# pkuyzy/ESC-GNN

Measured on AMD Instinct MI355X. Metric: graphs/sec + edges-aggregated/sec, NestedGIN_eff h=3 bs=128 @1/2/4/8 GPU, higher is better.
Workload: dtype f32; 1 GPU; count_cycle-shaped random regular graphs (n in 10/15/20/30), target=triangles, NestedGIN_eff h=3 layers=4 hidden=256, bs=128 per GPU (configs[1]); global_batch=128, parallelism=dp1 graph-sharded, rccl_ranks=1, ranks=1

## Files before the change

### esc-gnn_amd/_native.py

```python
import ctypes
import os
from ctypes import c_double, c_int64

from . import _abi

_HERE = os.path.dirname(os.path.abspath(__file__))
LIB_PATH = os.path.join(_HERE, "libescgnn_hip.so")


class NativeLibraryError(ImportError):
    pass


try:
    _ABI = _abi.load()
except OSError as exc:
    raise NativeLibraryError("esc_gnn_amd: cannot read the C header %s the binding is derived from (%s)" % (_abi.HEADER, exc)) from exc


def const(name):
    return _ABI.constants[name]


def struct(name):
    return _ABI.structs[name]


def callback(name):
    return _ABI.callbacks[name]


members = _abi.members
ABI_VERSION = const("ESC_ABI_VERSION")
ESC_ERANGE = const("ESC_ERANGE")
SIGNATURES = {name: args for name, (args, _) in _ABI.functions.items()}
_RET = {name: ret for name, (_, ret) in _ABI.functions.items()}
EXTENSION_HEADER = os.path.join(os.path.dirname(_abi.HEADER), "escgnn_subgraphs.h")
try:
    _EXT = _abi.load(EXTENSION_HEADER)
except OSError as exc:
    raise NativeLibraryError("esc_gnn_amd: cannot read the C header %s the binding is derived from (%s)" % (EXTENSION_HEADER, exc)) from exc
EXTENSION_SIGNATURES = {name: args for name, (args, _) in _EXT.functions.items()}
_RET.update({name: ret for name, (_, ret) in _EXT.functions.items()})
I2GNN_HEADER = os.path.join(os.path.dirname(_abi.HEADER), "escgnn_i2gnn.h")
try:
    _I2 = _abi.load(I2GNN_HEADER)
except OSError as exc:
    raise NativeLibraryError("esc_gnn_amd: cannot read the C header %s the binding is derived from (%s)" % (I2GNN_HEADER, exc)) from exc
I2GNN_SIGNATURES = {name: args for name, (args, _) in _I2.functions.items()}
_RET.update({name: ret for name, (_, ret) in _I2.functions.items()})
GINEPLUS_HEADER = os.path.join(os.path.dirname(_abi.HEADER), "escgnn_gineplus.h")
try:
    _GP = _abi.load(GINEPLUS_HEADER)
except OSError as exc:
    raise NativeLibraryError("esc_gnn_amd: cannot read the C header %s the binding is derived from (%s)" % (GINEPLUS_HEADER, exc)) from exc
GINEPLUS_SIGNATURES = {name: args for name, (args, _) in _GP.functions.items()}
_RET.update({name: ret for name, (_, ret) in _GP.functions.items()})
GPS_HEADER = os.path.join(os.path.dirname(_abi.HEADER), "escgnn_gps.h")
try:
    _GPS = _abi.load(GPS_HEADER)
except OSError as exc:
    raise NativeLibraryError("esc_gnn_amd: cannot read the C header %s the binding is derived from (%s)" % (GPS_HEADER, exc)) from exc
GPS_SIGNATURES = {name: args for name, (args, _) in _GPS.functions.items()}
_RET.update({name: ret for name, (_, ret) in _GPS.functions.items()})
LAPPE_HEADER = os.path.join(os.path.dirname(_abi.HEADER), "escgnn_lappe.h")
try:
    _LAPPE = _abi.load(LAPPE_HEADER)
except OSError as exc:
    raise NativeLibraryError("esc_gnn_amd: cannot read the C header %s the binding is derived from (%s)" % (LAPPE_HEADER, exc)) from exc
LAPPE_SIGNATURES = {name: args for name, (args, _) in _LAPPE.functions.items()}
_RET.update({name: ret for name, (_, ret) in _LAPPE.functions.items()})
RWSE_HEADER = os.path.join(os.path.dirname(_abi.HEADER), "escgnn_rwse.h")
try:
    _RWSE = _abi.load(RWSE_HEADER)
except OSError as exc:
    raise NativeLibraryError("esc_gnn_amd: cannot read the C header %s the binding is derived from (%s)" % (RWSE_HEADER, exc)) from exc
RWSE_SIGNATURES = {name: args for name, (args, _) in _RWSE.functions.items()}
_RET.update({name: ret for name, (_, ret) in _RWSE.functions.items()})
KIND = {name[len("ESC_K_"):].lower(): v for name, v in _ABI.enum.items() if name != "ESC_K_COUNT"}

CollateArgs = struct("esc_collate_args")
BnFuse = struct("esc_bn_fuse")
BnFold = struct("esc_bn_fold")
BnBwdFused = struct("esc_bn_bwd_fused")
BnBwdNext = struct("esc_bn_bwd_next")
SumJob = struct("esc_sum_job")
ReduceJob = struct("esc_reduce_job")

_lib = None


def lib():
    global _lib
    if _lib is not None:
        return _lib
    if not os.path.exists(LIB_PATH):
        raise NativeLibraryError(
            "esc_gnn_amd: %s not found. The HIP hot path has no fallback — build it with "
            "`python -c 'import __graft_entry__ as g; g.build()'` or `make -C esc-gnn_amd/csrc`." % LIB_PATH)
    h = ctypes.CDLL(LIB_PATH)
    for name, args in list(SIGNATURES.items()) + list(EXTENSION_SIGNATURES.items()) + list(I2GNN_SIGNATURES.items()) + list(GINEPLUS_SIGNATURES.items()) + list(GPS_SIGNATURES.items()) + list(LAPPE_SIGNATURES.items()) + list(RWSE_SIGNATURES.items()):
        try:
            fn = getattr(h, name)
        except AttributeError as exc:
            raise NativeLibraryError("esc_gnn_amd: %s lacks symbol %s (stale build?)" % (LIB_PATH, name)) from exc
        fn.argtypes = args
        fn.restype = _RET[name]
    if h.esc_abi_version() != ABI_VERSION:
        raise NativeLibraryError("esc_gnn_amd: ABI version mismatch (library %d, header %d) — rebuild"
                                 % (h.esc_abi_version(), ABI_VERSION))
    _lib = h
    return h


def call(name, *args):
    h = lib()
    rc = getattr(h, name)(*args)
    if rc != 0:
        raise RuntimeError("%s failed (%d): %s" % (name, rc, h.esc_last_error().decode()))


def ptr(t):
    return None if t is None else t.data_ptr()


def stream():
    import torch
    return torch.cuda.current_stream().cuda_stream


def prof_enable(kind, on=True):
    call("esc_prof_enable", KIND[kind], int(on))


def prof_reset(kind):
    call("esc_prof_reset", KIND[kind])


def prof_read(kind):
    n, ms = c_int64(0), c_double(0.0)
    call("esc_prof_read", KIND[kind], ctypes.byref(n), ctypes.byref(ms))
    return n.value, ms.value


def prof_span_arm(kind, launches):
    call("esc_prof_span_arm", KIND[kind], int(launches), stream())


def prof_span_read(kind, cap=1 << 16):
    buf = (c_double * cap)()
    n = lib().esc_prof_span_read(KIND[kind], buf, cap)
    return [buf[i] for i in range(n)]


def prof_read_all(kind, cap=1 << 16):
    buf = (c_double * cap)()
    n = lib().esc_prof_read_all(KIND[kind], buf, cap)
    return [buf[i] for i in range(n)]
```

### esc-gnn_amd/csrc/common.h

```cpp
#pragma once
#include <hip/hip_runtime.h>
#include <hip/hip_ext.h>
#include <stdint.h>
#include <stdio.h>
#include <stdarg.h>

#include "../../include/escgnn_hip.h"

namespace esc {

constexpr int WAVE = 64;

#ifndef ESC_NODE_PRIO
#define ESC_NODE_PRIO 2
#endif
#define ESC_PRIO() __builtin_amdgcn_s_setprio(ESC_NODE_PRIO)

void set_error(const char* fmt, ...);

#define ESC_REQUIRE(cond, ...)                    \
  do {                                            \
    if (!(cond)) {                                \
      esc::set_error(__VA_ARGS__);                \
      return ESC_EINVAL;                          \
    }                                             \
  } while (0)

#define ESC_CHECK_LAUNCH(name)                                              \
  do {                                                                      \
    hipError_t err__ = hipGetLastError();                                   \
    if (err__ != hipSuccess) {                                              \
      esc::set_error("%s: launch failed: %s", name, hipGetErrorString(err__)); \
      return ESC_ELAUNCH;                                                   \
    }                                                                       \
  } while (0)

inline bool aligned16(const void* p) { return (reinterpret_cast<uintptr_t>(p) & 15) == 0; }
inline int64_t cdiv(int64_t a, int64_t b) { return (a + b - 1) / b; }

bool prof_slot(int kind, hipEvent_t* start, hipEvent_t* stop);
unsigned long long* prof_span_next(int kind);
#define ESC_SPAN_WGS 2048
#define ESC_SPAN_WAVES 8192
#define ESC_SPAN_STRIDE (ESC_SPAN_WGS + ESC_SPAN_WAVES)
bool trace_launch();

void arm_launch_event(hipEvent_t ev);
hipEvent_t take_launch_event();
void arm_last_launch_event(hipEvent_t ev);
void next_launch_is_last();
hipEvent_t take_last_launch_event();

template <typename... KArgs, typename... Args>
inline void launch(int kind, void (*kernel)(KArgs...), dim3 grid, dim3 block, size_t lds, hipStream_t s,
                   Args... args) {
  hipEvent_t a = nullptr, b = nullptr;
  hipEvent_t done = take_launch_event();
  if (done != nullptr) {
    hipStreamCaptureStatus cap = hipStreamCaptureStatusNone;
    if (hipStreamIsCapturing(s, &cap) != hipSuccess || cap != hipStreamCaptureStatusNone) { arm_launch_event(done); done = nullptr; }
  }
  if (prof_slot(kind, &a, &b)) {
    hipExtLaunchKernelGGL(kernel, grid, block, (unsigned)lds, s, a, b, 0, static_cast<KArgs>(args)...);
    if (done != nullptr) (void)hipEventRecord(done, s);
  } else if (done != nullptr) {
    hipExtLaunchKernelGGL(kernel, grid, block, (unsigned)lds, s, nullptr, done, 0, static_cast<KArgs>(args)...);
  } else {
    hipLaunchKernelGGL(kernel, grid, block, (unsigned)lds, s, static_cast<KArgs>(args)...);
  }
  if (trace_launch()) {
    const char* name = hipKernelNameRefByPtr(reinterpret_cast<const void*>(kernel), s);
    fprintf(stderr, "[esc] %s grid (%u,%u,%u) block %u lds %zu stream %p ...", name ? name : "?", grid.x, grid.y, grid.z, block.x, lds, (void*)s);
    fflush(stderr);
    const hipError_t e = hipStreamSynchronize(s);
    fprintf(stderr, " %s\n", e == hipSuccess ? "done" : hipGetErrorString(e));
  }
}

struct BnCounters {
  int n = 0;
  int64_t* p[ESC_MAX_BN_COUNTERS] = {};
};
int bag_bwd_classify_counted(const int32_t* c_row, int64_t Z, int64_t H, int64_t rows, float* partials, const BnCounters& cnt,
                             void* stream);

__device__ __forceinline__ int lane_id() { return threadIdx.x & 63; }

__device__ __forceinline__ int uniform(int v) { return __builtin_amdgcn_readfirstlane(v); }

__device__ __forceinline__ float wave_sum(float v) {
#pragma unroll
  for (int o = 32; o > 0; o >>= 1) v += __shfl_xor(v, o, 64);
  return v;
}
__device__ __forceinline__ double wave_sum(double v) {
#pragma unroll
  for (int o = 32; o > 0; o >>= 1) v += __shfl_xor(v, o, 64);
  return v;
}

__device__ __forceinline__ float uniform01(unsigned long long seed, unsigned long long i) {
  unsigned long long z = seed + i * 0x9E3779B97F4A7C15ull;
  z = (z ^ (z >> 30)) * 0xBF58476D1CE4E5B9ull;
  z = (z ^ (z >> 27)) * 0x94D049BB133111EBull;
  z ^= z >> 31;
  return (float)(z >> 40) * (1.0f / 16777216.0f);
}

unsigned* tickets(int n);
int gemm_lds_floor();
void set_gemm_lds_floor(int bytes);
int edge_lds_floor();
int node_lds_floor();
void set_node_lds_floor(int bytes);
void set_edge_lds_floor(int bytes);
int norm_rowblock_cap();
void set_norm_rowblock_cap(int v);
bool bn_bwd_one_launch();
void set_bn_bwd_one_launch(int on);
bool bn_bwd_fold();
void set_bn_bwd_fold(int on);
bool last_block_finalize();
void set_last_block_finalize(int on);
void set_linear_knob(int knob, int value);
struct DualSplit { hipEvent_t dx_done = nullptr, dw_done = nullptr; int dx_lds = 0; };
void request_dual_split(const DualSplit& r);
bool take_dual_split();

__device__ __forceinline__ void store_agent(float2* p, float2 v) {
  const unsigned long long bits = ((unsigned long long)__float_as_uint(v.y) << 32) | __float_as_uint(v.x);
  __hip_atomic_store(reinterpret_cast<unsigned long long*>(p), bits, __ATOMIC_RELAXED, __HIP_MEMORY_SCOPE_AGENT);
}

__device__ __forceinline__ bool grid_last_block(unsigned* counter, unsigned nblocks) {
  __shared__ unsigned s_ticket;
  __builtin_amdgcn_s_waitcnt(0x0F70);
  __syncthreads();
  if (threadIdx.x == 0) s_ticket = __hip_atomic_fetch_add(counter, 1u, __ATOMIC_RELAXED, __HIP_MEMORY_SCOPE_AGENT);
  __syncthreads();
  const bool last = s_ticket == nblocks - 1;
  if (last) {
    __builtin_amdgcn_fence(__ATOMIC_ACQUIRE, "agent");
    if (threadIdx.x == 0) *counter = 0;
  }
  return last;
}

__device__ __forceinline__ void chan_merge(double& n, double& mu, double& m2, double nb, double mub, double m2b) {
  if (nb == 0.0) return;
  const double tot = n + nb;
  const double delta = mub - mu;
  mu += delta * nb / tot;
  m2 += m2b + delta * delta * n * nb / tot;
  n = tot;
}


struct BnFoldDev {
  const float2* partials;
  int P, block_rows, M, C;
  float eps, momentum;
  const float* gamma; const float* beta;
  float* mean; float* invstd; float* scale; float* shift; float* running_mean; float* running_var;
};
__device__ __forceinline__ void bn_fold_column(const BnFoldDev& f, int col, bool writer, float& sc, float& sh) {
  const int full = f.M / f.block_rows;
  double n = 0.0, mu = 0.0, m2 = 0.0;
  if (full > 0) {
    const double pivot = (double)f.partials[col].x;
    double S1 = 0.0, S2 = 0.0, SM = 0.0;
    constexpr int CH = 40;
    for (int p0 = 0; p0 < full; p0 += CH) {
      float2 v[CH];
#pragma unroll
      for (int u = 0; u < CH; ++u) v[u] = f.partials[(size_t)min(p0 + u, full - 1) * f.C + col];
#pragma unroll
      for (int u = 0; u < CH; ++u) {
        if (p0 + u < full) { const double d = (double)v[u].x - pivot; S1 += d; S2 += d * d; SM += (double)v[u].y; }
      }
    }
    n = (double)f.block_rows * full;
    mu = pivot + S1 / full;
    m2 = SM + (double)f.block_rows * (S2 - S1 * S1 / full);
    if (m2 < 0.0) m2 = 0.0;
  }
  if (f.M > f.block_rows * full) {
    const float2 v = f.partials[(size_t)full * f.C + col];
    chan_merge(n, mu, m2, (double)(f.M - f.block_rows * full), (double)v.x, (double)v.y);
  }
  const float is = (float)(1.0 / sqrt(m2 / (double)f.M + (double)f.eps));
  sc = (f.gamma ? f.gamma[col] : 1.f) * is;
  sh = (f.beta ? f.beta[col] : 0.f) - (float)mu * sc;
  if (writer) {
    f.mean[col] = (float)mu;
    f.invstd[col] = is;
    if (f.scale) { f.scale[col] = sc; f.shift[col] = sh; }
    if (f.running_mean) f.running_mean[col] = (1.f - f.momentum) * f.running_mean[col] + f.momentum * (float)mu;
    if (f.running_var) f.running_var[col] = (1.f - f.momentum) * f.running_var[col] + f.momentum * (float)(m2 / (double)(f.M - 1));
  }
}

struct BnbDev {
  const float* x; int ldx;
  const float* mean; const float* invstd; const float* scale; const float* shift;
  const float2* coef;
  int relu;
};
struct BnStatDev {
  float2* partial;
  const float* x; int ldx;
  const float* mean; const float* invstd; const float* scale; const float* shift;
  int relu;
};

__device__ __forceinline__ float bnb_apply(float gv, float xv, float mu, float a, float ms, float mh, float k1, float k2) {
  const float gm = fmaf(xv, ms, mh) > 0.f ? gv : 0.f;
  return a * fmaf(mu - xv, k2, gm - k1);
}
__device__ __forceinline__ float bnb_apply_elu(float gv, float xv, float mu, float a, float ms, float mh, float k1, float k2) {
  const float v = fmaf(xv, ms, mh);
  const float gm = v > 0.f ? gv : gv * expf(v);
  return a * fmaf(mu - xv, k2, gm - k1);
}
__device__ __forceinline__ float bnb_apply_act(float gv, float xv, float mu, float a, float ms, float mh, float k1, float k2, bool elu) {
  return elu ? bnb_apply_elu(gv, xv, mu, a, ms, mh, k1, k2) : bnb_apply(gv, xv, mu, a, ms, mh, k1, k2);
}

}
```

### esc-gnn_amd/csrc/engine.hip

```cpp
#include "common.h"

#include <map>
#include <vector>
#include <cstdlib>

namespace esc {

struct Arena {
  float* base;
  int64_t off;
  float* take(int64_t n) {
    float* p = base ? base + off : nullptr;
    off += (n + 63) & ~63LL;
    return p;
  }
};

struct BnWs { float *mean, *invstd, *scale, *shift, *nglob, *coef; };
struct MlpWs { float *Y0, *Y1; BnWs b0, b1; float* A1 = nullptr; };

struct Layout {
  int64_t N, E, Z, H, L, C0, W;
  float *Zb, *Yz; BnWs zb0, zb1;
  float *A0, *Zemb;
  float* e[ESC_MAX_LAYERS]; float* agg[ESC_MAX_LAYERS]; MlpWs conv[ESC_MAX_LAYERS];
  int64_t ld_e[ESC_MAX_LAYERS];
  float *e_cat, *w_cat;
  MlpWs xemb; float *cat, *Yl; BnWs bl; float *pred, *dpred;
  float *dcat, *dAl, *dT1, *dT2, *dagg, *dZemb, *dAz, *deps_part;
  float* d_e[ESC_MAX_LAYERS];
  float *bn_scratch, *bag_scratch, *slabs;
  float *col_stats;
  float *bst_part;
  float *bn_scratch_e, *col_stats_e;
  float *cat_scale, *cat_shift;
  float *X0, *dX0, *Zcat, *dZcat, *pooled, *dpool, *Al;
  int64_t G, D, Wz;
  int64_t total;
};

static BnWs take_bn(Arena& a, int64_t C) { BnWs w; w.mean = a.take(C); w.invstd = a.take(C); w.scale = a.take(C); w.shift = a.take(C); w.nglob = a.take(16); w.coef = a.take(2 * C); return w; }

static Layout plan_layout(const esc_nested_gin_t* m, int64_t N, int64_t E, int64_t Z, float* base, bool train) {
  Layout y{};
  Arena a{base, 0};
  const int64_t H = m->hidden, L = m->num_layers, C0 = m->in_dim;
  y.N = N; y.E = E; y.Z = Z; y.H = H; y.L = L; y.C0 = C0; y.W = (L + 1) * H;
  y.Zb = a.take(E * H); y.Yz = a.take(E * H); y.zb0 = take_bn(a, H); y.zb1 = take_bn(a, H);
  y.A0 = a.take(E * H); y.Zemb = a.take(E * H);
  const bool batched = L >= 3;
  if (batched) { y.e_cat = a.take(E * (L - 1) * H); y.w_cat = a.take(((L - 1) * H + (L - 1)) * H); }
  for (int l = 0; l < L; ++l) {
    const int64_t C = l == 0 ? C0 : H;
    if (batched && l >= 1) { y.e[l] = base ? y.e_cat + (int64_t)(l - 1) * H : nullptr; y.ld_e[l] = (L - 1) * H; }
    else { y.e[l] = a.take(E * C); y.ld_e[l] = C; }
    y.agg[l] = a.take(N * C);
    y.conv[l].Y0 = a.take(N * H); y.conv[l].Y1 = a.take(N * H);
    y.conv[l].b0 = take_bn(a, H); y.conv[l].b1 = take_bn(a, H);
  }
  y.xemb.Y0 = a.take(N * H); y.xemb.Y1 = a.take(N * H); y.xemb.b0 = take_bn(a, H); y.xemb.b1 = take_bn(a, H);
  y.cat = a.take(N * y.W); y.Yl = a.take(N * H); y.bl = take_bn(a, H);
  y.cat_scale = a.take(y.W); y.cat_shift = a.take(y.W);
  if (base) {
    y.xemb.b1.scale = y.cat_scale; y.xemb.b1.shift = y.cat_shift;
    for (int l = 0; l < L; ++l) { y.conv[l].b1.scale = y.cat_scale + (int64_t)(l + 1) * H; y.conv[l].b1.shift = y.cat_shift + (int64_t)(l + 1) * H; }
  }
  y.pred = a.take(N); y.dpred = a.take(N);
  y.bn_scratch = a.take(esc_bn_scratch(H));
  y.col_stats = a.take(2 * ((E > N ? E : N) / 32 + 1) * H);
  y.bn_scratch_e = a.take(esc_bn_scratch(H));
  y.col_stats_e = a.take(2 * (E / 32 + 1) * H);
  if (train) {
    y.bst_part = a.take(2 * (N / 4 + 2) * H);
    y.dcat = a.take(N * y.W); y.dAl = a.take(N * H); y.dT1 = a.take(N * H); y.dT2 = a.take(N * H);
    y.dagg = a.take(N * H); y.dZemb = a.take(E * H); y.dAz = a.take(E * H);
    for (int l = 0; l < L; ++l) y.d_e[l] = a.take(E * (l == 0 ? C0 : H));
    y.deps_part = a.take(2 * N * (L > 0 ? L : 1));
    y.bag_scratch = a.take(esc_bag_bwd_scratch(Z, H));
    int64_t sl = esc_linear_bwd_weight_scratch(E, H, H) + 64;
    for (int l = 0; l < L; ++l) {
      const int64_t C = l == 0 ? C0 : H;
      sl += esc_linear_bwd_weight_scratch(E, C, H) + esc_linear_bwd_weight_scratch(N, H, H) +
            esc_linear_bwd_weight_scratch(N, H, C) + 3 * 64;
    }
    sl += esc_linear_bwd_weight_scratch(N, H, H) + esc_linear_bwd_weight_scratch(N, H, C0) + 2 * 64;
    sl += esc_linear_bwd_weight_scratch(N, H, y.W) + esc_linear_bwd_weight_scratch(N, 1, H) + 2 * 64;
    sl += esc_linear_bwd_weight_scratch(N, H, 1) + 64;
    y.slabs = a.take(sl);
  }
  y.total = a.off;
  return y;
}

#define ESC_TRY(call)            \
  do {                           \
    int rc__ = (call);           \
    if (rc__ != ESC_OK) return rc__; \
  } while (0)

struct Ctx {
  const esc_nested_gin_t* m;
  const esc_batch_t* b;
  Layout y;
  void* s;
  bool train;
  std::vector<esc_reduce_job>* jobs = nullptr;
  float** slab_cursor = nullptr;
  bool on_edge_stream = false;
  int act = 1;
  const float* l1_target = nullptr;
  int64_t l1_denom = 0;
};

struct LdsFloorGuard {
  explicit LdsFloorGuard(bool on) : on_(on && edge_lds_floor() > 0) { if (on_) set_gemm_lds_floor(edge_lds_floor()); }
  ~LdsFloorGuard() { if (on_) set_gemm_lds_floor(0); }
  bool on_;
};

static constexpr int kNodeLdsFloorBwd = 66 * 1024;
static constexpr int kReadoutDxLds = 84 * 1024;
static_assert(2 * kReadoutDxLds > 160 * 1024 && kReadoutDxLds + kNodeLdsFloorBwd <= 160 * 1024, "one readout dX tile and one node tile per CU");
static int g_readout_one_launch = 0;
struct NodeFloorGuard {
  explicit NodeFloorGuard(int bytes) : on_(bytes > 0) { if (on_) set_node_lds_floor(bytes); }
  ~NodeFloorGuard() { if (on_) set_node_lds_floor(0); }
  bool on_;
};

static int linear_backward(const Ctx& c, const float* dY, int64_t ld_dy, const float* X, int64_t ld_x, const float* sc,
                           const float* sh, const esc_linear_t& lin, int64_t M, float* dX, int64_t ld_dx, int accumulate) {
  const LdsFloorGuard cap(c.on_edge_stream);
  const int64_t N = lin.out_dim, K = lin.in_dim;
  if (c.jobs == nullptr)
    return esc_linear_bwd_both(dY, ld_dy, X, ld_x, sc, sh, lin.w, K, M, N, K, dX, ld_dx, accumulate, lin.dw, K, lin.db,
                               c.y.slabs, c.s);
  float* slabs = *c.slab_cursor;
  *c.slab_cursor += (esc_linear_bwd_weight_scratch(M, N, K) + 63) & ~63LL;
  c.jobs->emplace_back();
  return esc_linear_bwd_both_deferred(dY, ld_dy, X, ld_x, sc, sh, lin.w, K, M, N, K, dX, ld_dx, accumulate, lin.dw, K, lin.db,
                                      slabs, &c.jobs->back(), c.s);
}

static constexpr bool kBnBwdApplyInGemm = true;
static constexpr bool kBnBwdSumsFromDx = true;
static constexpr bool kBnBwdSumsFromAgg = true;
static esc_bn_bwd_fused bn_fused(const float* x, int64_t ld_x, const BnWs& w, int relu) {
  return esc_bn_bwd_fused{x, ld_x, w.mean, w.invstd, w.scale, w.shift, w.coef, relu};
}
static int linear_backward_bn(const Ctx& c, const float* dOut, int64_t ld_dout, const esc_bn_bwd_fused& f, const float* X, int64_t ld_x,
                              const float* sc, const float* sh, const esc_linear_t& lin, int64_t M, float* dX, int64_t ld_dx,
                              int accumulate, const esc_bn_bwd_next* next) {
  const LdsFloorGuard cap(c.on_edge_stream);
  const int64_t N = lin.out_dim, K = lin.in_dim;
  if (c.jobs == nullptr)
    return esc_linear_bwd_both_bn(dOut, ld_dout, &f, X, ld_x, sc, sh, lin.w, K, M, N, K, dX, ld_dx, accumulate, lin.dw, K, lin.db, c.y.slabs,
                                  nullptr, next, c.s);
  float* slabs = *c.slab_cursor;
  *c.slab_cursor += (esc_linear_bwd_weight_scratch(M, N, K) + 63) & ~63LL;
  c.jobs->emplace_back();
  return esc_linear_bwd_both_bn(dOut, ld_dout, &f, X, ld_x, sc, sh, lin.w, K, M, N, K, dX, ld_dx, accumulate, lin.dw, K, lin.db, slabs,
                                &c.jobs->back(), next, c.s);
}

struct EdgeStream {
  hipStream_t stream = nullptr;
  hipEvent_t z_ready = nullptr, joined = nullptr, lin1_fork = nullptr, lin1_rest = nullptr, lin1_dw = nullptr, e_ready[ESC_MAX_LAYERS] = {}, de_ready[ESC_MAX_LAYERS] = {},
             agg_done[ESC_MAX_LAYERS] = {};
  bool ok = false;
};
static int g_use_edge_stream = 1;
static int current_device() {
  int dev = 0;
  (void)hipGetDevice(&dev);
  return dev;
}
static EdgeStream& edge_stream() {
  static thread_local std::map<int, EdgeStream> per_device;
  static thread_local EdgeStream off;
  if (!g_use_edge_stream) return off;
  EdgeStream& es = per_device[current_device()];
  if (!es.ok && es.stream == nullptr) {
    int least = 0, greatest = 0;
    (void)hipDeviceGetStreamPriorityRange(&least, &greatest);
    bool good = hipStreamCreateWithPriority(&es.stream, hipStreamNonBlocking, least) == hipSuccess;
    good = good && hipEventCreateWithFlags(&es.z_ready, hipEventDisableTiming) == hipSuccess;
    good = good && hipEventCreateWithFlags(&es.joined, hipEventDisableTiming) == hipSuccess;
    good = good && hipEventCreateWithFlags(&es.lin1_fork, hipEventDisableTiming) == hipSuccess;
    good = good && hipEventCreateWithFlags(&es.lin1_rest, hipEventDisableTiming) == hipSuccess;
    good = good && hipEventCreateWithFlags(&es.lin1_dw, hipEventDisableTiming) == hipSuccess;
    for (int l = 0; l < ESC_MAX_LAYERS; ++l) {
      good = good && hipEventCreateWithFlags(&es.e_ready[l], hipEventDisableTiming) == hipSuccess;
      good = good && hipEventCreateWithFlags(&es.de_ready[l], hipEventDisableTiming) == hipSuccess;
      good = good && hipEventCreateWithFlags(&es.agg_done[l], hipEventDisableTiming) == hipSuccess;
    }
    es.ok = good;
  }
  return es;
}
static int64_t g_two_stream_min_edges = 12000;
static EdgeStream& edge_stream_for(int64_t edges) {
  static thread_local EdgeStream off;
  return edges >= g_two_stream_min_edges ? edge_stream() : off;
}
static int chain(hipEvent_t ev, hipStream_t src, hipStream_t waiter) {
  if (hipEventRecord(ev, src) != hipSuccess || hipStreamWaitEvent(waiter, ev, 0) != hipSuccess) {
    set_error("esc_engine: stream event failed");
    return ESC_ELAUNCH;
  }
  return ESC_OK;
}

static int g_plain_events = 0;
struct ArmedEvent {
  ArmedEvent(hipEvent_t ev, bool on) : on_(on && !g_plain_events) { if (on_) arm_launch_event(ev); }
  ~ArmedEvent() { if (on_) (void)take_launch_event(); }
  bool on_;
};
struct ArmedLastEvent {
  ArmedLastEvent(hipEvent_t ev, bool on) : on_(on && !g_plain_events) { if (on_) arm_last_launch_event(ev); }
  ~ArmedLastEvent() { if (on_) (void)take_last_launch_event(); }
  bool bound() const { return on_ && take_last_launch_event() == nullptr; }
  bool on_;
};
static int chain_armed(hipEvent_t ev, const ArmedEvent& arm, hipStream_t src, hipStream_t waiter) {
  const bool bound = arm.on_ && take_launch_event() == nullptr;
  if ((!bound && hipEventRecord(ev, src) != hipSuccess) || (waiter != nullptr && hipStreamWaitEvent(waiter, ev, 0) != hipSuccess)) {
    set_error("esc_engine: stream event failed");
    return ESC_ELAUNCH;
  }
  return ESC_OK;
}

static Ctx edge_ctx(const Ctx& c, hipStream_t edge) {
  Ctx x = c;
  x.s = edge;
  x.on_edge_stream = true;
  x.y.bn_scratch = c.y.bn_scratch_e;
  x.y.col_stats = c.y.col_stats_e;
  return x;
}

enum { PH_START = 0, PH_EDGE_FWD_DONE, PH_NODE_FWD_DONE, PH_NODE_BWD_DONE, PH_EDGE_BWD_DONE, PH_END, PH_COUNT };
struct PhaseRing {
  static constexpr int RING = 128;
  hipEvent_t ev[RING][PH_COUNT] = {};
  int steps = 0;
  bool on = getenv("ESC_PHASE_TIMING") != nullptr;
};
static PhaseRing& phases() { static PhaseRing p; return p; }
static void mark(int which, void* stream) {
  PhaseRing& p = phases();
  if (!p.on) return;
  hipEvent_t& e = p.ev[p.steps % PhaseRing::RING][which];
  if (e == nullptr && hipEventCreate(&e) != hipSuccess) { p.on = false; return; }
  (void)hipEventRecord(e, (hipStream_t)stream);
}

static bool fuse_node_act(const Ctx& c) { return c.act == 1 && c.y.H >= 64 && c.y.H % 4 == 0 && c.y.cat_scale != nullptr; }

struct Collective {
  esc_allreduce_fn fn = nullptr; void* user = nullptr;
  int rank = 0, world = 1;
  float *buf_node = nullptr, *buf_edge = nullptr; int64_t cap = 0;
};
static Collective g_coll;
static bool sync_on(const Ctx& c) { return c.train && g_coll.fn != nullptr && g_coll.world > 1; }
static float* sync_buf(const Ctx& c) {
  EdgeStream& es = edge_stream();
  return (es.ok && c.s == (void*)es.stream) ? g_coll.buf_edge : g_coll.buf_node;
}
static int sync_allreduce(const Ctx& c, float* buf, int64_t n) {
  ESC_REQUIRE(buf != nullptr && n <= g_coll.cap, "esc_engine: SyncBN exchange buffer too small (%ld > %ld floats)", (long)n, (long)g_coll.cap);
  const int rc = g_coll.fn(buf, n, c.s, g_coll.user);
  if (rc != 0) { set_error("esc_engine: the collective provider failed (%d)", rc); return ESC_ELAUNCH; }
  return ESC_OK;
}
static int bn_sync_forward(const Ctx& c, int64_t M, const esc_bn_t& bn, const BnWs& w, int64_t C) {
  float* buf = sync_buf(c);
  ESC_TRY(esc_bn_sync_pack(w.mean, w.invstd, M, bn.eps, C, g_coll.rank, g_coll.world, buf, c.s));
  ESC_TRY(sync_allreduce(c, buf, (int64_t)g_coll.world * 3 * C));
  return esc_bn_sync_finalize(buf, g_coll.world, C, bn.eps, bn.momentum, w.mean, w.invstd, bn.running_mean, bn.running_var,
                              bn.gamma, bn.beta, w.scale, w.shift, w.nglob, c.s);
}
static int bn_backward(const Ctx& c, const float* X, int64_t ldx, const float* Y, int64_t ldy, const float* dY, int64_t lddy,
                       int64_t M, const BnWs& w, const esc_bn_t& bn, float* dX, int64_t lddx, float* scratch, int64_t width = 0) {
  const int64_t C = width > 0 ? width : c.y.H;
  if (!sync_on(c))
    return esc_bn_bwd(X, ldx, Y, ldy, dY, lddy, M, C, w.mean, w.invstd, bn.gamma, bn.beta, c.act, dX, lddx, bn.dgamma, bn.dbeta,
                      scratch, c.s);
  float* buf = sync_buf(c);
  ESC_TRY(esc_bn_bwd_sums(X, ldx, Y, ldy, dY, lddy, M, C, w.mean, w.invstd, bn.gamma, bn.beta, c.act, buf, bn.dgamma, bn.dbeta,
                          scratch, c.s));
  ESC_TRY(sync_allreduce(c, buf, 2 * C));
  ESC_TRY(esc_bn_sync_coef(buf, C, w.nglob, c.s));
  return esc_bn_bwd_apply(X, ldx, Y, ldy, dY, lddy, M, C, w.mean, w.invstd, bn.gamma, bn.beta, c.act, buf, dX, lddx, c.s);
}

static int bn_backward_drop(const Ctx& c, const float* X, int64_t ldx, const float* dY, int64_t lddy, int64_t M, const BnWs& w,
                            const esc_bn_t& bn, const uint8_t* mask, float p, int on_output, float* dX, int64_t lddx,
                            float* scratch, int64_t width = 0) {
  const int64_t C = width > 0 ? width : c.y.H;
  if (p <= 0.f) return bn_backward(c, X, ldx, nullptr, 0, dY, lddy, M, w, bn, dX, lddx, scratch, width);
  const bool fused = !sync_on(c) && c.act <= 1 && ldx == C && lddy == C && lddx == C && esc_bn_bwd_dropout_ok(C, ldx, lddy, lddx) &&
                     ((reinterpret_cast<uintptr_t>(X) | reinterpret_cast<uintptr_t>(dY) | reinterpret_cast<uintptr_t>(dX) |
                       reinterpret_cast<uintptr_t>(w.mean) | reinterpret_cast<uintptr_t>(w.invstd) | reinterpret_cast<uintptr_t>(bn.gamma) |
                       reinterpret_cast<uintptr_t>(bn.beta) | reinterpret_cast<uintptr_t>(scratch)) & 15) == 0 &&
                     (reinterpret_cast<uintptr_t>(mask) & 3) == 0;
  if (fused)
    return esc_bn_bwd_dropout(X, ldx, dY, lddy, M, C, w.mean, w.invstd, bn.gamma, bn.beta, c.act, mask, p, on_output, dX, lddx,
                              bn.dgamma, bn.dbeta, scratch, c.s);
  if (!on_output) {
    ESC_TRY(esc_dropout_bwd(dY, lddy, M, C, p, mask, nullptr, 0, dX, lddx, c.s));
    return bn_backward(c, X, ldx, nullptr, 0, dX, lddx, M, w, bn, dX, lddx, scratch, width);
  }
  ESC_TRY(bn_backward(c, X, ldx, nullptr, 0, dY, lddy, M, w, bn, dX, lddx, scratch, width));
  return esc_dropout_bwd(dX, lddx, M, C, p, mask, nullptr, 0, dX, lddx, c.s);
}

static int linear_bn(const Ctx& c, const float* X, int64_t ld_x, const esc_linear_t& lin, const float* sc, const float* sh,
                     int64_t M, float* Y, const esc_bn_t& bn, const BnWs& w, int64_t ld_y = 0) {
  const LdsFloorGuard cap(c.on_edge_stream);
  const int64_t H = lin.out_dim, K = lin.in_dim;
  if (ld_y <= 0) ld_y = H;
  const bool sync = sync_on(c);
  const bool fused = c.train && H > 32 && c.jobs != nullptr;
  if (fused && M > 1 && !sync) {
    esc_bn_fuse f{bn.eps, bn.momentum, w.mean, w.invstd, bn.running_mean, bn.running_var, bn.gamma, bn.beta, w.scale, w.shift};
    return esc_linear_bn_fwd(X, ld_x, lin.w, K, lin.b, sc, sh, M, H, K, Y, ld_y, c.y.col_stats, &f, c.s);
  }
  ESC_TRY(esc_linear_fwd(X, ld_x, lin.w, K, lin.b, sc, sh, M, H, K, Y, ld_y, fused ? c.y.col_stats : nullptr, c.s));
  if (fused) {
    ESC_TRY(esc_bn_stats_from_partials_rows(c.y.col_stats, M, H, esc_linear_stats_block_rows(X, ld_x, lin.w, K, M, H, K), bn.eps,
                                            bn.momentum, w.mean, w.invstd, sync ? nullptr : bn.running_mean,
                                            sync ? nullptr : bn.running_var, bn.gamma, bn.beta, sync ? nullptr : w.scale,
                                            sync ? nullptr : w.shift, c.s));
    return sync ? bn_sync_forward(c, M, bn, w, H) : ESC_OK;
  }
  if (c.train) {
    ESC_TRY(esc_bn_stats(Y, ld_y, M, H, bn.eps, bn.momentum, w.mean, w.invstd, sync ? nullptr : bn.running_mean,
                         sync ? nullptr : bn.running_var, bn.gamma, bn.beta, sync ? nullptr : w.scale, sync ? nullptr : w.shift,
                         c.y.bn_scratch, c.s));
    return sync ? bn_sync_forward(c, M, bn, w, H) : ESC_OK;
  }
  return esc_bn_eval_coef(bn.running_mean, bn.running_var, bn.gamma, bn.beta, bn.eps, H, w.scale, w.shift, c.s);
}

static int bn_coeffs(const Ctx& c, const float* X, int64_t ld, int64_t M, const esc_bn_t& bn, const BnWs& w, int64_t width = 0) {
  const int64_t C = width > 0 ? width : c.y.H;
  if (c.train) {
    const bool sync = sync_on(c);
    ESC_TRY(esc_bn_stats(X, ld, M, C, bn.eps, bn.momentum, w.mean, w.invstd, sync ? nullptr : bn.running_mean,
                         sync ? nullptr : bn.running_var, bn.gamma, bn.beta, sync ? nullptr : w.scale, sync ? nullptr : w.shift,
                         c.y.bn_scratch, c.s));
    return sync ? bn_sync_forward(c, M, bn, w, C) : ESC_OK;
  }
  return esc_bn_eval_coef(bn.running_mean, bn.running_var, bn.gamma, bn.beta, bn.eps, C, w.scale, w.shift, c.s);
}

static int mlp_forward(const Ctx& c, const esc_mlp_t& p, const MlpWs& w, const float* A, int64_t ld_a, int64_t M,
                       float* out, int64_t ld_out, bool pre_out = false) {
  const int64_t H = c.y.H;
  if (pre_out) {
    ESC_TRY(linear_bn(c, A, ld_a, p.lin0, nullptr, nullptr, M, w.Y0, p.bn0, w.b0));
    return linear_bn(c, w.Y0, H, p.lin1, w.b0.scale, w.b0.shift, M, out, p.bn1, w.b1, ld_out);
  }
  ESC_TRY(linear_bn(c, A, ld_a, p.lin0, nullptr, nullptr, M, w.Y0, p.bn0, w.b0));
  if (w.A1) {
    ESC_TRY(esc_affine_act(w.Y0, H, M, H, w.b0.scale, w.b0.shift, c.act, w.A1, H, c.s));
    ESC_TRY(linear_bn(c, w.A1, H, p.lin1, nullptr, nullptr, M, w.Y1, p.bn1, w.b1));
    return esc_affine_act(w.Y1, H, M, H, w.b1.scale, w.b1.shift, c.act, out, ld_out, c.s);
  }
  ESC_TRY(linear_bn(c, w.Y0, H, p.lin1, w.b0.scale, w.b0.shift, M, w.Y1, p.bn1, w.b1));
  return esc_affine_act(w.Y1, H, M, H, w.b1.scale, w.b1.shift, 1, out, ld_out, c.s);
}

struct MlpFuse { bool lin1 = false, lin0 = false; };
static MlpFuse mlp_fuse_plan(const Ctx& c, const esc_mlp_t& p, const MlpWs& w, const float* A, int64_t ld_a, int64_t M, const float* out,
                             int64_t ld_out, const float* dOut, int64_t ld_dout, const float* dA, int64_t ld_da, bool pre_out) {
  const Layout& y = c.y;
  const int64_t H = y.H;
  MlpFuse f;
  if (!(kBnBwdApplyInGemm && c.train && !sync_on(c) && y.bst_part != nullptr && p.lin1.in_dim == H && p.lin1.out_dim == H)) return f;
  if (!(c.act == 1 && w.A1 == nullptr)) return f;
  const esc_bn_bwd_fused f1 = bn_fused(pre_out ? out : w.Y1, pre_out ? ld_out : H, w.b1, c.act), f0 = bn_fused(w.Y0, H, w.b0, c.act);
  const esc_bn_bwd_next n0{y.bst_part, w.Y0, H, w.b0.mean, w.b0.invstd, w.b0.scale, w.b0.shift, c.act};
  const float* slab_probe = c.jobs ? *c.slab_cursor : y.slabs;
  f.lin1 = esc_linear_bwd_both_bn_ok(dOut, ld_dout, &f1, w.Y0, H, p.lin1.w, H, M, H, H, y.dT2, H, slab_probe, &n0) != 0;
  f.lin0 = f.lin1 && esc_linear_bwd_both_bn_ok(y.dT2, H, &f0, A, ld_a, p.lin0.w, p.lin0.in_dim, M, H, p.lin0.in_dim, dA, ld_da, slab_probe, nullptr) != 0;
  return f;
}
static bool mlp_backward_fused(const Ctx& c, const esc_mlp_t& p, const MlpWs& w, const float* A, int64_t ld_a, int64_t M, const float* out,
                               int64_t ld_out, const float* dOut, int64_t ld_dout, const float* dA, int64_t ld_da, bool pre_out) {
  return mlp_fuse_plan(c, p, w, A, ld_a, M, out, ld_out, dOut, ld_dout, dA, ld_da, pre_out).lin1;
}
static int mlp_backward(const Ctx& c, const esc_mlp_t& p, const MlpWs& w, const float* A, int64_t ld_a, int64_t M,
                        const float* out, int64_t ld_out, const float* dOut, int64_t ld_dout, float* dA,
                        int64_t ld_da, bool pre_out = false, int64_t have_slots = 0) {
  const Layout& y = c.y;
  const int64_t H = y.H;
  const MlpFuse fuse = mlp_fuse_plan(c, p, w, A, ld_a, M, out, ld_out, dOut, ld_dout, dA, ld_da, pre_out);
  if (fuse.lin1) {
    const float* x1 = pre_out ? out : w.Y1;
    const int64_t ld_x1 = pre_out ? ld_out : H;
    const esc_bn_bwd_fused f1 = bn_fused(x1, ld_x1, w.b1, c.act), f0 = bn_fused(w.Y0, H, w.b0, c.act);
    esc_bn_bwd_next n0{y.bst_part, w.Y0, H, w.b0.mean, w.b0.invstd, w.b0.scale, w.b0.shift, c.act};
    if (have_slots > 0)
      ESC_TRY(esc_bn_bwd_coef_from_partials(y.bst_part, have_slots, M, H, w.b1.coef, p.bn1.dgamma, p.bn1.dbeta, c.s));
    else
      ESC_TRY(esc_bn_bwd_coef(x1, ld_x1, nullptr, 0, dOut, ld_dout, M, H, w.b1.mean, w.b1.invstd, p.bn1.gamma, p.bn1.beta, c.act, w.b1.coef,
                              p.bn1.dgamma, p.bn1.dbeta, y.bn_scratch, c.s));
    ESC_TRY(linear_backward_bn(c, dOut, ld_dout, f1, w.Y0, H, w.b0.scale, w.b0.shift, p.lin1, M, y.dT2, H, 0, &n0));
    ESC_TRY(esc_bn_bwd_coef_from_partials(y.bst_part, cdiv(M, esc_linear_bwd_bn_block_rows(M, H, H)), M, H, w.b0.coef, p.bn0.dgamma, p.bn0.dbeta, c.s));
    if (fuse.lin0) return linear_backward_bn(c, y.dT2, H, f0, A, ld_a, nullptr, nullptr, p.lin0, M, dA, ld_da, 0, nullptr);
    ESC_TRY(esc_bn_bwd_apply(w.Y0, H, nullptr, 0, y.dT2, H, M, H, w.b0.mean, w.b0.invstd, p.bn0.gamma, p.bn0.beta, c.act, w.b0.coef, y.dT2, H, c.s));
    return linear_backward(c, y.dT2, H, A, ld_a, nullptr, nullptr, p.lin0, M, dA, ld_da, 0);
  }
  if (pre_out) ESC_TRY(bn_backward(c, out, ld_out, nullptr, 0, dOut, ld_dout, M, w.b1, p.bn1, y.dT1, H, y.bn_scratch));
  else         ESC_TRY(bn_backward(c, w.Y1, H, out, ld_out, dOut, ld_dout, M, w.b1, p.bn1, y.dT1, H, y.bn_scratch));
  if (w.A1) {
    ESC_TRY(linear_backward(c, y.dT1, H, w.A1, H, nullptr, nullptr, p.lin1, M, y.dT2, H, 0));
    ESC_TRY(bn_backward(c, w.Y0, H, w.A1, H, y.dT2, H, M, w.b0, p.bn0, y.dT2, H, y.bn_scratch));
    return linear_backward(c, y.dT2, H, A, ld_a, nullptr, nullptr, p.lin0, M, dA, ld_da, 0);
  }
  ESC_TRY(linear_backward(c, y.dT1, H, w.Y0, H, w.b0.scale, w.b0.shift, p.lin1, M, y.dT2, H, 0));
  ESC_TRY(bn_backward(c, w.Y0, H, nullptr, 0, y.dT2, H, M, w.b0, p.bn0, y.dT2, H, y.bn_scratch));
  return linear_backward(c, y.dT2, H, A, ld_a, nullptr, nullptr, p.lin0, M, dA, ld_da, 0);
}

static int forward(const Ctx& c) {
  const esc_nested_gin_t* m = c.m;
  const esc_batch_t* b = c.b;
  const Layout& y = c.y;
  const int64_t N = y.N, E = y.E, H = y.H, L = y.L, W = y.W;
  EdgeStream& es = edge_stream_for(E);
  Ctx ce = c;
  if (es.ok) {
    ESC_TRY(chain(es.z_ready, (hipStream_t)c.s, es.stream));
    ce = edge_ctx(c, es.stream);
  }
  const int64_t bag_block = (c.train && !sync_on(ce)) ? esc_bag_fwd_stats_block_rows(m->z_table, m->z_rows, H, y.Zb, H, E) : 0;
  if (bag_block > 0) {
    ESC_TRY(esc_bag_fwd_rows(m->z_table, m->z_rows, H, b->row_ptr, b->bag_idx, b->bag_val, E, y.Zb, H, 0, ce.y.col_stats, ce.s));
    ESC_TRY(esc_bn_stats_from_partials_rows(ce.y.col_stats, E, H, bag_block, m->zbn0.eps, m->zbn0.momentum, y.zb0.mean, y.zb0.invstd,
                                            m->zbn0.running_mean, m->zbn0.running_var, m->zbn0.gamma, m->zbn0.beta, y.zb0.scale, y.zb0.shift, ce.s));
  } else {
    ESC_TRY(esc_bag_fwd_rows(m->z_table, m->z_rows, H, b->row_ptr, b->bag_idx, b->bag_val, E, y.Zb, H, 0, nullptr, ce.s));
    ESC_TRY(bn_coeffs(ce, y.Zb, H, E, m->zbn0, y.zb0));
  }
  ESC_TRY(esc_affine_act(y.Zb, H, E, H, y.zb0.scale, y.zb0.shift, 1, y.A0, H, ce.s));
  ESC_TRY(linear_bn(ce, y.A0, H, m->zlin, nullptr, nullptr, E, y.Yz, m->zbn1, y.zb1));
  const bool e0_early = y.C0 <= 32 && L >= 1;
  if (e0_early) {
    const LdsFloorGuard cap(ce.on_edge_stream);
    const ArmedEvent arm(es.e_ready[0], es.ok);
    ESC_TRY(esc_linear_fwd(y.Yz, H, m->conv[0].lin.w, H, m->conv[0].lin.b, y.zb1.scale, y.zb1.shift, E, y.C0, H, y.e[0], y.ld_e[0], nullptr, ce.s));
    if (es.ok) ESC_TRY(chain_armed(es.e_ready[0], arm, es.stream, nullptr));
  }
  ESC_TRY(esc_affine_act(y.Yz, H, E, H, y.zb1.scale, y.zb1.shift, 1, y.Zemb, H, ce.s));
  auto edge_term = [&](int l) -> int {
    const LdsFloorGuard cap(ce.on_edge_stream);
    const esc_conv_t& cv = m->conv[l];
    const int64_t C = l == 0 ? y.C0 : H;
    ESC_TRY(esc_linear_fwd(y.Zemb, H, cv.lin.w, H, cv.lin.b, nullptr, nullptr, E, C, H, y.e[l], y.ld_e[l], nullptr, ce.s));
    if (es.ok && hipEventRecord(es.e_ready[l], es.stream) != hipSuccess) { set_error("esc_engine: stream event failed"); return ESC_ELAUNCH; }
    return ESC_OK;
  };
  mark(PH_START, c.s);
  const bool batched = y.e_cat != nullptr;
  if (batched) {
    if (!e0_early) ESC_TRY(edge_term(0));
    esc_table_list tl{};
    tl.count = 2 * ((int)L - 1);
    for (int l = 1; l < (int)L; ++l) {
      tl.rows[l - 1] = (int32_t)H; tl.w[l - 1] = m->conv[l].lin.w;
      tl.rows[(L - 1) + l - 1] = 1; tl.w[(L - 1) + l - 1] = m->conv[l].lin.b;
    }
    ESC_TRY(esc_table_pack(&tl, H, y.w_cat, ce.s));
    {
      const LdsFloorGuard cap(ce.on_edge_stream);
      const ArmedEvent arm(es.e_ready[1], es.ok);
      ESC_TRY(esc_linear_fwd(y.Zemb, H, y.w_cat, H, y.w_cat + (L - 1) * H * H, nullptr, nullptr, E, (L - 1) * H, H, y.e_cat, (L - 1) * H, nullptr, ce.s));
      if (es.ok) ESC_TRY(chain_armed(es.e_ready[1], arm, es.stream, nullptr));
    }
    for (int l = 2; l < (int)L; ++l)
      if (es.ok && hipEventRecord(es.e_ready[l], es.stream) != hipSuccess) { set_error("esc_engine: stream event failed"); return ESC_ELAUNCH; }
  }
  const int ahead = batched ? 0 : (es.ok ? 1 : (int)L);
  for (int l = e0_early ? 1 : 0; l < (int)L && l < ahead; ++l) ESC_TRY(edge_term(l));
  if (c.train) {
    BnCounters cnt;
    cnt.n = (int)m->n_counters;
    for (int i = 0; i < cnt.n; ++i) cnt.p[i] = m->counters[i];
    ESC_TRY(bag_bwd_classify_counted(b->col_row, y.Z, H, E, y.bag_scratch, cnt, c.s));
  }
  ESC_TRY(mlp_forward(c, m->xemb, y.xemb, b->x, y.C0, N, y.cat, W, fuse_node_act(c)));
  for (int l = 0; l < L; ++l) {
    const esc_conv_t& cv = m->conv[l];
    const int64_t C = l == 0 ? y.C0 : H;
    const float* hin = l == 0 ? b->x : y.cat + (int64_t)l * H;
    const int64_t ld_h = l == 0 ? y.C0 : W;
    if (es.ok && !(batched && l >= 2) && hipStreamWaitEvent((hipStream_t)c.s, es.e_ready[l], 0) != hipSuccess) { set_error("esc_engine: stream event failed"); return ESC_ELAUNCH; }
    if (fuse_node_act(c) && l > 0)
      ESC_TRY(esc_gine_aggregate_fwd_affine(hin, ld_h, y.cat_scale + (int64_t)l * H, y.cat_shift + (int64_t)l * H, y.e[l], y.ld_e[l], b->in_ptr,
                                            b->in_edge, b->in_src, cv.eps, N, C, y.agg[l], C, c.s));
    else
      ESC_TRY(esc_gine_aggregate_fwd(hin, ld_h, y.e[l], y.ld_e[l], b->in_ptr, b->in_edge, b->in_src, cv.eps, N, C, y.agg[l], C, c.s));
    if (!batched && es.ok && l + ahead < (int)L) {
      ESC_TRY(chain(es.agg_done[l], (hipStream_t)c.s, es.stream));
      ESC_TRY(edge_term(l + ahead));
    }
    ESC_TRY(mlp_forward(c, cv.nn, y.conv[l], y.agg[l], C, N, y.cat + (int64_t)(l + 1) * H, W, fuse_node_act(c)));
  }
  if (c.train) mark(PH_EDGE_FWD_DONE, ce.s);
  const bool fa = fuse_node_act(c);
  ESC_TRY(linear_bn(c, y.cat, W, m->lin1, fa ? y.cat_scale : nullptr, fa ? y.cat_shift : nullptr, N, y.Yl, m->bn_lin1, y.bl));
  if (c.l1_target != nullptr && esc_linear_fwd_l1_ok(y.Yl, H, m->lin2.w, H, y.bl.scale, y.bl.shift)) {
    const ArmedEvent arm(es.lin1_fork, es.ok);
    ESC_TRY(esc_linear_fwd_l1(y.Yl, H, m->lin2.w, m->lin2.b, y.bl.scale, y.bl.shift, N, H, c.l1_target, c.l1_denom, 1.0f, y.pred, y.dpred, c.s));
    return es.ok ? chain_armed(es.lin1_fork, arm, (hipStream_t)c.s, es.stream) : ESC_OK;
  }
  return esc_linear_fwd(y.Yl, H, m->lin2.w, H, m->lin2.b, y.bl.scale, y.bl.shift, N, 1, H, y.pred, 1, nullptr, c.s);
}

struct Pending {
  bool open = false;
  bool join = false;
  hipStream_t stream = nullptr;
  std::vector<esc_reduce_job> edge_jobs;
};
static Pending& pending() {
  static thread_local Pending p;
  return p;
}
static int finish_pending(Pending& p) {
  if (!p.open) return ESC_OK;
  p.open = false;
  EdgeStream& es = edge_stream();
  if (p.join && hipStreamWaitEvent(p.stream, es.joined, 0) != hipSuccess) { set_error("esc_engine: stream event failed"); return ESC_ELAUNCH; }
  if (!p.edge_jobs.empty()) ESC_TRY(esc_slab_reduce_jobs(p.edge_jobs.data(), (int)p.edge_jobs.size(), p.stream));
  p.edge_jobs.clear();
  mark(PH_END, p.stream);
  if (phases().on) ++phases().steps;
  return ESC_OK;
}

static int backward(const Ctx& c, Pending* defer) {
  EdgeStream& es = edge_stream_for(c.y.E);
  const NodeFloorGuard node_floor(es.ok ? kNodeLdsFloorBwd : 0);
  const esc_nested_gin_t* m = c.m;
  const esc_batch_t* b = c.b;
  const Layout& y = c.y;
  const int64_t N = y.N, E = y.E, H = y.H, L = y.L, W = y.W;
  ESC_TRY(linear_backward(c, y.dpred, 1, y.Yl, H, y.bl.scale, y.bl.shift, m->lin2, N, y.dAl, H, 0));
  const bool split_lin1 = es.ok && c.jobs != nullptr && L >= 1;
  const esc_bn_bwd_fused fl = bn_fused(y.Yl, H, y.bl, 1);
  const bool fa_l = fuse_node_act(c);
  const MlpWs& wl = y.conv[L > 0 ? L - 1 : 0];
  esc_bn_bwd_next nl{y.bst_part, y.cat + L * H, W, wl.b1.mean, wl.b1.invstd, wl.b1.scale, wl.b1.shift, 1};
  auto lin1_ok = [&](int64_t col0, int64_t ncols, const esc_bn_bwd_next* nx) {
    return esc_linear_bwd_both_bn_ok(y.dAl, H, &fl, y.cat + col0, W, m->lin1.w + col0, W, N, H, ncols, y.dcat + col0, W,
                                     c.jobs ? *c.slab_cursor : y.slabs, nx) != 0;
  };
  const bool fuse_l = kBnBwdApplyInGemm && c.act == 1 && !sync_on(c) && y.bst_part != nullptr &&
                      (split_lin1 ? (lin1_ok(0, L * H, nullptr) && lin1_ok(L * H, H, nullptr)) : lin1_ok(0, W, nullptr));
  int64_t last_slots = 0;
  bool k0_split = false;
  bool fork_bound = false;
  if (fuse_l) {
    const ArmedLastEvent arm(es.lin1_fork, split_lin1);
    ESC_TRY(esc_bn_bwd_coef(y.Yl, H, nullptr, 0, y.dAl, H, N, H, y.bl.mean, y.bl.invstd, m->bn_lin1.gamma, m->bn_lin1.beta, 1, y.bl.coef,
                            m->bn_lin1.dgamma, m->bn_lin1.dbeta, y.bn_scratch, c.s));
    fork_bound = arm.bound();
  } else
    ESC_TRY(bn_backward(c, y.Yl, H, nullptr, 0, y.dAl, H, N, y.bl, m->bn_lin1, y.dAl, H, y.bn_scratch));
  if (split_lin1) {
    const int64_t K0 = L * H;
    auto part = [&](void* stream, int64_t col0, int64_t ncols, float* db, const esc_bn_bwd_next* nx) -> int {
      float* slabs = *c.slab_cursor;
      *c.slab_cursor += (esc_linear_bwd_weight_scratch(N, H, ncols) + 63) & ~63LL;
      c.jobs->emplace_back();
      const bool fa = fa_l;
      if (fuse_l)
        return esc_linear_bwd_both_bn(y.dAl, H, &fl, y.cat + col0, W, fa ? y.cat_scale + col0 : nullptr, fa ? y.cat_shift + col0 : nullptr, m->lin1.w + col0, W,
                                      N, H, ncols, y.dcat + col0, W, 0, m->lin1.dw + col0, W, db, slabs, &c.jobs->back(), nx, stream);
      return esc_linear_bwd_both_deferred(y.dAl, H, y.cat + col0, W, fa ? y.cat_scale + col0 : nullptr, fa ? y.cat_shift + col0 : nullptr, m->lin1.w + col0, W, N, H, ncols,
                                          y.dcat + col0, W, 0, m->lin1.dw + col0, W, db, slabs, &c.jobs->back(), stream);
    };
    if ((!fork_bound && hipEventRecord(es.lin1_fork, (hipStream_t)c.s) != hipSuccess) || hipStreamWaitEvent(es.stream, es.lin1_fork, 0) != hipSuccess) {
      set_error("esc_engine: stream event failed");
      return ESC_ELAUNCH;
    }
    {
      const LdsFloorGuard cap(true);
      const bool ask = fuse_l && !g_readout_one_launch && !g_plain_events;
      if (ask) request_dual_split(DualSplit{es.lin1_rest, es.lin1_dw, kReadoutDxLds});
      const int rc = part(es.stream, 0, K0, nullptr, nullptr);
      k0_split = !take_dual_split() && ask;
      ESC_TRY(rc);
    }
    if (!k0_split && hipEventRecord(es.lin1_rest, es.stream) != hipSuccess) { set_error("esc_engine: stream event failed"); return ESC_ELAUNCH; }
    const bool leave = fuse_l && fa_l && kBnBwdSumsFromDx && lin1_ok(K0, H, &nl) &&
                       mlp_backward_fused(c, m->conv[L - 1].nn, y.conv[L - 1], y.agg[L - 1], L == 1 ? y.C0 : H, N, y.cat + L * H, W, y.dcat + L * H, W,
                                          y.dagg, L == 1 ? y.C0 : H, true);
    ESC_TRY(part(c.s, K0, H, m->lin1.db, leave ? &nl : nullptr));
    if (leave) last_slots = cdiv(N, esc_linear_bwd_bn_block_rows(N, H, H));
  } else if (fuse_l) {
    ESC_TRY(linear_backward_bn(c, y.dAl, H, fl, y.cat, W, fa_l ? y.cat_scale : nullptr, fa_l ? y.cat_shift : nullptr, m->lin1, N, y.dcat, W, 0, nullptr));
  } else {
    ESC_TRY(linear_backward(c, y.dAl, H, y.cat, W, fa_l ? y.cat_scale : nullptr, fa_l ? y.cat_shift : nullptr, m->lin1, N, y.dcat, W, 0));
  }
  Ctx ce = es.ok ? edge_ctx(c, es.stream) : c;
  std::vector<esc_reduce_job> edge_jobs;
  edge_jobs.reserve(ESC_MAX_REDUCE_JOBS);
  if (es.ok && c.jobs) ce.jobs = &edge_jobs;
  std::vector<esc_sum_job> eps_jobs;
  int64_t agg_slots = 0;
  for (int l = (int)L - 1; l >= 0; --l) {
    const esc_conv_t& cv = m->conv[l];
    const int64_t C = l == 0 ? y.C0 : H;
    const float* hin = l == 0 ? b->x : y.cat + (int64_t)l * H;
    const int64_t ld_h = l == 0 ? y.C0 : W;
    ESC_TRY(mlp_backward(c, cv.nn, y.conv[l], y.agg[l], C, N, y.cat + (int64_t)(l + 1) * H, W,
                         y.dcat + (int64_t)(l + 1) * H, W, y.dagg, C, fuse_node_act(c), l == (int)L - 1 ? last_slots : agg_slots));
    agg_slots = 0;
    float* dx = l == 0 ? nullptr : y.dcat + (int64_t)l * H;
    if (split_lin1 && l == (int)L - 1 &&
        hipStreamWaitEvent((hipStream_t)c.s, es.lin1_rest, 0) != hipSuccess) { set_error("esc_engine: stream event failed"); return ESC_ELAUNCH; }
    const ArmedEvent arm(es.de_ready[l], es.ok);
    const bool stats_here = fuse_node_act(c) && l > 0 && kBnBwdSumsFromAgg && esc_gine_aggregate_bwd_deps_slots(C) == 1 && C <= 2048 &&
                            mlp_backward_fused(c, m->conv[l - 1].nn, y.conv[l - 1], y.agg[l - 1], l - 1 == 0 ? y.C0 : H, N, y.cat + (int64_t)l * H, W,
                                               y.dcat + (int64_t)l * H, W, y.dagg, l - 1 == 0 ? y.C0 : H, true);
    if (stats_here) {
      ESC_TRY(esc_gine_aggregate_bwd_affine_stats(hin, ld_h, y.cat_scale + (int64_t)l * H, y.cat_shift + (int64_t)l * H, y.conv[l - 1].b1.mean,
                                                  y.conv[l - 1].b1.invstd, y.e[l], y.ld_e[l], y.dagg, C, b->out_ptr, b->out_edge, b->out_dst, cv.eps, N, C,
                                                  y.d_e[l], C, dx, W, 1, y.deps_part + (int64_t)l * 2 * N, y.bst_part, c.s));
      agg_slots = esc_gine_aggregate_bwd_stats_slots(N);
    } else if (fuse_node_act(c) && l > 0)
      ESC_TRY(esc_gine_aggregate_bwd_affine(hin, ld_h, y.cat_scale + (int64_t)l * H, y.cat_shift + (int64_t)l * H, y.e[l], y.ld_e[l], y.dagg, C,
                                            b->out_ptr, b->out_edge, b->out_dst, cv.eps, N, C, y.d_e[l], C, dx, W, 1,
                                            y.deps_part + (int64_t)l * 2 * N, c.s));
    else
      ESC_TRY(esc_gine_aggregate_bwd(hin, ld_h, y.e[l], y.ld_e[l], y.dagg, C, b->out_ptr, b->out_edge, b->out_dst, cv.eps, N, C,
                                     y.d_e[l], C, dx, W, 1, y.deps_part + (int64_t)l * 2 * N, c.s));
    eps_jobs.push_back(esc_sum_job{y.deps_part + (int64_t)l * 2 * N, N * esc_gine_aggregate_bwd_deps_slots(C), cv.deps});
    if (es.ok) ESC_TRY(chain_armed(es.de_ready[l], arm, (hipStream_t)c.s, es.stream));
    const float* zin = y.Zemb;
    if (l == 0 && es.ok && c.jobs) {
      {
        const LdsFloorGuard cap(true);
        ESC_TRY(esc_linear_bwd_input(y.d_e[l], C, cv.lin.w, H, E, C, H, y.dZemb, H, l == (int)L - 1 ? 0 : 1, es.stream));
      }
      float* slabs = *c.slab_cursor;
      *c.slab_cursor += (esc_linear_bwd_weight_scratch(E, C, H) + 63) & ~63LL;
      c.jobs->emplace_back();
      ESC_TRY(esc_linear_bwd_both_deferred(y.d_e[l], C, zin, H, nullptr, nullptr, cv.lin.w, H, E, C, H, nullptr, 0, 0, cv.lin.dw, H, cv.lin.db,
                                           slabs, &c.jobs->back(), c.s));
    } else {
      ESC_TRY(linear_backward(ce, y.d_e[l], C, zin, H, nullptr, nullptr, cv.lin, E, y.dZemb, H, l == (int)L - 1 ? 0 : 1));
    }
    if (es.ok && !edge_jobs.empty() && l > 0) {
      ESC_TRY(esc_slab_reduce_jobs(edge_jobs.data(), (int)edge_jobs.size(), es.stream));
      edge_jobs.clear();
    }
  }
  ESC_TRY(mlp_backward(c, m->xemb, y.xemb, b->x, y.C0, N, y.cat, W, y.dcat, W, nullptr, 0, fuse_node_act(c)));
  Ctx ct = ce;
  ct.on_edge_stream = false;
  ESC_TRY(bn_backward(ce, y.Yz, H, nullptr, 0, y.dZemb, H, E, y.zb1, m->zbn1, y.dZemb, H, ce.y.bn_scratch));
  ESC_TRY(linear_backward(ct, y.dZemb, H, y.A0, H, nullptr, nullptr, m->zlin, E, y.dAz, H, 0));
  ESC_TRY(bn_backward(ce, y.Zb, H, nullptr, 0, y.dAz, H, E, y.zb0, m->zbn0, y.dAz, H, ce.y.bn_scratch));
  ESC_TRY(esc_bag_bwd_table_rows(y.dAz, H, H, b->col_ptr, b->col_row, b->col_val, b->col_col, y.Z, m->z_rows, E,
                                 1, m->dz_table, y.bag_scratch, ce.s));
  mark(PH_NODE_BWD_DONE, c.s);
  mark(PH_EDGE_BWD_DONE, ce.s);
  if (!eps_jobs.empty()) ESC_TRY(esc_reduce_sum_jobs(eps_jobs.data(), (int)eps_jobs.size(), c.s));
  if (k0_split && hipStreamWaitEvent((hipStream_t)c.s, es.lin1_dw, 0) != hipSuccess) { set_error("esc_engine: stream event failed"); return ESC_ELAUNCH; }
  if (c.jobs && !c.jobs->empty()) ESC_TRY(esc_slab_reduce_jobs(c.jobs->data(), (int)c.jobs->size(), c.s));
  if (es.ok) {
    if (hipEventRecord(es.joined, es.stream) != hipSuccess) { set_error("esc_engine: stream event failed"); return ESC_ELAUNCH; }
    Pending local;
    Pending& p = defer ? *defer : local;
    p.open = true; p.join = true; p.stream = (hipStream_t)c.s;
    p.edge_jobs.swap(edge_jobs);
    if (!defer) return finish_pending(p);
  }
  return ESC_OK;
}

static Layout plan_layout_zinc(const esc_zinc_gin_t* m, int64_t N, int64_t E, int64_t Z, int64_t G, float* base, bool train) {
  Layout y{};
  Arena a{base, 0};
  const int64_t H = m->hidden, L = m->num_layers, D = m->edge_emb.dim, C0 = m->node_emb.dim;
  y.N = N; y.E = E; y.Z = Z; y.H = H; y.L = L; y.C0 = C0; y.W = L * H; y.G = G; y.D = D; y.Wz = H + D;
  y.X0 = a.take(N * C0);
  y.Zb = a.take(E * H); y.Yz = a.take(E * H); y.zb0 = take_bn(a, H); y.zb1 = take_bn(a, H);
  y.A0 = a.take(E * H); y.Zcat = a.take(E * y.Wz);
  const int64_t lb = C0 == H ? 0 : 1, nb = L - lb;
  const bool batched = nb >= 2;
  if (batched) { y.e_cat = a.take(E * nb * H); y.w_cat = a.take(nb * H * y.Wz + nb * H); }
  for (int l = 0; l < L; ++l) {
    const int64_t C = l == 0 ? C0 : H;
    if (batched && l >= lb) { y.e[l] = base ? y.e_cat + (int64_t)(l - lb) * H : nullptr; y.ld_e[l] = nb * H; }
    else { y.e[l] = a.take(E * C); y.ld_e[l] = C; }
    y.agg[l] = a.take(N * C);
    y.conv[l].Y0 = a.take(N * H); y.conv[l].Y1 = a.take(N * H); y.conv[l].A1 = a.take(N * H);
    y.conv[l].b0 = take_bn(a, H); y.conv[l].b1 = take_bn(a, H);
  }
  const bool nodes = m->node_readout != 0;
  const int64_t R = nodes ? N : G;
  y.cat = a.take(N * y.W); y.pooled = nodes ? nullptr : a.take(G * y.W); y.Yl = a.take(R * H); y.Al = a.take(R * H);
  y.bl = take_bn(a, H);
  y.pred = a.take(R); y.dpred = a.take(R);
  y.bn_scratch = a.take(esc_bn_scratch(H));
  y.col_stats = a.take(2 * ((E > N ? E : N) / 32 + 1) * H);
  y.bn_scratch_e = a.take(esc_bn_scratch(H));
  y.col_stats_e = a.take(2 * (E / 32 + 1) * H);
  if (train) {
    y.dcat = a.take(N * y.W); y.dpool = nodes ? nullptr : a.take(G * y.W); y.dAl = a.take(R * H);
    y.bst_part = a.take(2 * (N / 4 + E / 64 + 4) * H);
    y.dT1 = a.take(N * H); y.dT2 = a.take(N * H); y.dagg = a.take(N * H); y.dX0 = a.take(N * C0);
    y.dZcat = a.take(E * y.Wz); y.dZemb = a.take(E * H); y.dAz = a.take(E * H);
    for (int l = 0; l < L; ++l) y.d_e[l] = a.take(E * (l == 0 ? C0 : H));
    y.deps_part = a.take(2 * N * (L > 0 ? L : 1));
    y.bag_scratch = a.take(esc_bag_bwd_scratch(Z, H));
    int64_t sl = esc_linear_bwd_weight_scratch(E, H, H) + 64;
    for (int l = 0; l < L; ++l) {
      const int64_t C = l == 0 ? C0 : H;
      sl += esc_linear_bwd_weight_scratch(E, C, y.Wz) + esc_linear_bwd_weight_scratch(N, H, H) +
            esc_linear_bwd_weight_scratch(N, H, C) + 3 * 64;
    }
    sl += esc_linear_bwd_weight_scratch(R, H, y.W) + esc_linear_bwd_weight_scratch(R, 1, H) + 2 * 64;
    y.slabs = a.take(sl);
  }
  y.total = a.off;
  return y;
}

struct ZincCtx {
  const esc_zinc_gin_t* m;
  const esc_mol_batch_t* b;
  Ctx c;
};

static int forward_zinc(const ZincCtx& z) {
  const esc_zinc_gin_t* m = z.m;
  const esc_mol_batch_t* b = z.b;
  const Ctx& c = z.c;
  const Layout& y = c.y;
  const int64_t N = y.N, E = y.E, H = y.H, L = y.L, W = y.W, G = y.G, D = y.D, Wz = y.Wz, C0 = y.C0;
  const int act = c.act;
  EdgeStream& es = edge_stream_for(E);
  Ctx ce = c;
  if (es.ok) {
    ESC_TRY(chain(es.z_ready, (hipStream_t)c.s, es.stream));
    ce = edge_ctx(c, es.stream);
  }
  ESC_TRY(esc_bag_fwd_rows(m->z_table, m->z_rows, H, b->row_ptr, b->bag_idx, b->bag_val, E, y.Zb, H, 0, nullptr, ce.s));
  if (c.train) ESC_TRY(esc_bag_bwd_classify(b->col_row, y.Z, H, E, y.bag_scratch, ce.s));
  ESC_TRY(bn_coeffs(ce, y.Zb, H, E, m->zbn0, y.zb0));
  ESC_TRY(esc_affine_act(y.Zb, H, E, H, y.zb0.scale, y.zb0.shift, act, y.A0, H, ce.s));
  ESC_TRY(linear_bn(ce, y.A0, H, m->zlin, nullptr, nullptr, E, y.Yz, m->zbn1, y.zb1));
  ESC_TRY(esc_affine_act(y.Yz, H, E, H, y.zb1.scale, y.zb1.shift, act, y.Zcat, Wz, ce.s));
  ESC_TRY(esc_embed_fwd(m->edge_emb.w, m->edge_emb.rows, D, b->edge_type, E, y.Zcat + H, Wz, nullptr, ce.s));
  auto edge_term = [&](int l) -> int {
    const LdsFloorGuard cap(ce.on_edge_stream);
    const esc_conv_t& cv = m->conv[l];
    const int64_t C = l == 0 ? C0 : H;
    ESC_TRY(esc_linear_fwd(y.Zcat, Wz, cv.lin.w, Wz, cv.lin.b, nullptr, nullptr, E, C, Wz, y.e[l], y.ld_e[l], nullptr, ce.s));
    if (es.ok && hipEventRecord(es.e_ready[l], es.stream) != hipSuccess) { set_error("esc_zinc: stream event failed"); return ESC_ELAUNCH; }
    return ESC_OK;
  };
  const bool batched = y.e_cat != nullptr;
  if (batched) {
    const int lb = C0 == H ? 0 : 1, nb = (int)L - lb;
    if (lb == 1) ESC_TRY(edge_term(0));
    esc_table_list tw{}, tb{};
    tw.count = nb; tb.count = nb;
    for (int l = lb; l < (int)L; ++l) {
      tw.rows[l - lb] = (int32_t)H; tw.w[l - lb] = m->conv[l].lin.w;
      tb.rows[l - lb] = 1; tb.w[l - lb] = m->conv[l].lin.b;
    }
    ESC_TRY(esc_table_pack(&tw, Wz, y.w_cat, ce.s));
    ESC_TRY(esc_table_pack(&tb, H, y.w_cat + (int64_t)nb * H * Wz, ce.s));
    {
      const LdsFloorGuard cap(ce.on_edge_stream);
      ESC_TRY(esc_linear_fwd(y.Zcat, Wz, y.w_cat, Wz, y.w_cat + (int64_t)nb * H * Wz, nullptr, nullptr, E, nb * H, Wz, y.e_cat, nb * H, nullptr, ce.s));
    }
    for (int l = lb; l < (int)L; ++l)
      if (es.ok && hipEventRecord(es.e_ready[l], es.stream) != hipSuccess) { set_error("esc_zinc: stream event failed"); return ESC_ELAUNCH; }
  }
  const int ahead = batched ? 0 : (es.ok ? 1 : (int)L);
  for (int l = 0; l < (int)L && l < ahead; ++l) ESC_TRY(edge_term(l));
  ESC_TRY(esc_embed_fwd(m->node_emb.w, m->node_emb.rows, C0, b->node_type, N, y.X0, C0, nullptr, c.s));
  for (int l = 0; l < (int)L; ++l) {
    const esc_conv_t& cv = m->conv[l];
    const int64_t C = l == 0 ? C0 : H;
    const float* hin = l == 0 ? y.X0 : y.cat + (int64_t)(l - 1) * H;
    const int64_t ld_h = l == 0 ? C0 : W;
    if (es.ok && hipStreamWaitEvent((hipStream_t)c.s, es.e_ready[l], 0) != hipSuccess) { set_error("esc_zinc: stream event failed"); return ESC_ELAUNCH; }
    ESC_TRY(esc_gine_aggregate_fwd(hin, ld_h, y.e[l], y.ld_e[l], b->in_ptr, b->in_edge, b->in_src, cv.eps, N, C, y.agg[l], C, c.s));
    if (!batched && es.ok && l + ahead < (int)L) {
      ESC_TRY(chain(es.agg_done[l], (hipStream_t)c.s, es.stream));
      ESC_TRY(edge_term(l + ahead));
    }
    ESC_TRY(mlp_forward(c, cv.nn, y.conv[l], y.agg[l], C, N, y.cat + (int64_t)l * H, W));
  }
  const int64_t R = m->node_readout ? N : G;
  const float* rin = y.cat;
  if (!m->node_readout) {
    ESC_TRY(esc_segment_pool_fwd(y.cat, W, b->graph_ptr, G, W, 0, y.pooled, W, c.s));
    rin = y.pooled;
  }
  ESC_TRY(linear_bn(c, rin, W, m->lin1, nullptr, nullptr, R, y.Yl, m->bn_lin1, y.bl));
  ESC_TRY(esc_affine_act(y.Yl, H, R, H, y.bl.scale, y.bl.shift, act, y.Al, H, c.s));
  ESC_TRY(esc_linear_fwd(y.Al, H, m->lin2.w, H, m->lin2.b, nullptr, nullptr, R, 1, H, y.pred, 1, nullptr, c.s));
  if (es.ok) ESC_TRY(chain(es.joined, es.stream, (hipStream_t)c.s));
  return ESC_OK;
}

static int backward_zinc(const ZincCtx& z) {
  const esc_zinc_gin_t* m = z.m;
  const esc_mol_batch_t* b = z.b;
  const Ctx& c = z.c;
  const Layout& y = c.y;
  const int64_t N = y.N, E = y.E, H = y.H, L = y.L, W = y.W, G = y.G, D = y.D, Wz = y.Wz, C0 = y.C0;
  EdgeStream& es = edge_stream_for(E);
  Ctx ce = es.ok ? edge_ctx(c, es.stream) : c;
  std::vector<esc_reduce_job> edge_jobs;
  edge_jobs.reserve(ESC_MAX_REDUCE_JOBS);
  if (es.ok && c.jobs) ce.jobs = &edge_jobs;
  if (es.ok) ESC_TRY(chain(es.z_ready, (hipStream_t)c.s, es.stream));
  const int64_t R = m->node_readout ? N : G;
  ESC_TRY(linear_backward(c, y.dpred, 1, y.Al, H, nullptr, nullptr, m->lin2, R, y.dAl, H, 0));
  ESC_TRY(bn_backward(c, y.Yl, H, y.Al, H, y.dAl, H, R, y.bl, m->bn_lin1, y.dAl, H, y.bn_scratch));
  if (m->node_readout) {
    ESC_TRY(linear_backward(c, y.dAl, H, y.cat, W, nullptr, nullptr, m->lin1, N, y.dcat, W, 0));
  } else {
    ESC_TRY(linear_backward(c, y.dAl, H, y.pooled, W, nullptr, nullptr, m->lin1, G, y.dpool, W, 0));
    ESC_TRY(esc_segment_pool_bwd(y.dpool, W, b->graph_ptr, G, W, 0, y.dcat, W, c.s));
  }
  std::vector<esc_sum_job> eps_jobs;
  for (int l = (int)L - 1; l >= 0; --l) {
    const esc_conv_t& cv = m->conv[l];
    const int64_t C = l == 0 ? C0 : H;
    const float* hin = l == 0 ? y.X0 : y.cat + (int64_t)(l - 1) * H;
    const int64_t ld_h = l == 0 ? C0 : W;
    ESC_TRY(mlp_backward(c, cv.nn, y.conv[l], y.agg[l], C, N, y.cat + (int64_t)l * H, W, y.dcat + (int64_t)l * H, W, y.dagg, C));
    float* dx = l == 0 ? y.dX0 : y.dcat + (int64_t)(l - 1) * H;
    ESC_TRY(esc_gine_aggregate_bwd(hin, ld_h, y.e[l], y.ld_e[l], y.dagg, C, b->out_ptr, b->out_edge, b->out_dst, cv.eps, N, C,
                                   y.d_e[l], C, dx, l == 0 ? C0 : W, l == 0 ? 0 : 1, y.deps_part + (int64_t)l * 2 * N, c.s));
    eps_jobs.push_back(esc_sum_job{y.deps_part + (int64_t)l * 2 * N, N * esc_gine_aggregate_bwd_deps_slots(C), cv.deps});
    if (es.ok) ESC_TRY(chain(es.de_ready[l], (hipStream_t)c.s, es.stream));
    ESC_TRY(linear_backward(ce, y.d_e[l], C, y.Zcat, Wz, nullptr, nullptr, cv.lin, E, y.dZcat, Wz, l == (int)L - 1 ? 0 : 1));
  }
  ESC_TRY(esc_embed_bwd(y.dX0, C0, b->node_type, N, m->node_emb.rows, C0, m->node_emb.dw, c.s));
  ESC_TRY(esc_embed_bwd(y.dZcat + H, Wz, b->edge_type, E, m->edge_emb.rows, D, m->edge_emb.dw, ce.s));
  ESC_TRY(bn_backward(ce, y.Yz, H, y.Zcat, Wz, y.dZcat, Wz, E, y.zb1, m->zbn1, y.dZemb, H, ce.y.bn_scratch));
  ESC_TRY(linear_backward(ce, y.dZemb, H, y.A0, H, nullptr, nullptr, m->zlin, E, y.dAz, H, 0));
  ESC_TRY(bn_backward(ce, y.Zb, H, y.A0, H, y.dAz, H, E, y.zb0, m->zbn0, y.dAz, H, ce.y.bn_scratch));
  ESC_TRY(esc_bag_bwd_table_rows(y.dAz, H, H, b->col_ptr, b->col_row, b->col_val, b->col_col, y.Z, m->z_rows, E, 1,
                                 m->dz_table, y.bag_scratch, ce.s));
  if (es.ok && !edge_jobs.empty()) ESC_TRY(esc_slab_reduce_jobs(edge_jobs.data(), (int)edge_jobs.size(), es.stream));
  if (!eps_jobs.empty()) ESC_TRY(esc_reduce_sum_jobs(eps_jobs.data(), (int)eps_jobs.size(), c.s));
  if (c.jobs && !c.jobs->empty()) ESC_TRY(esc_slab_reduce_jobs(c.jobs->data(), (int)c.jobs->size(), c.s));
  if (es.ok) ESC_TRY(chain(es.joined, es.stream, (hipStream_t)c.s));
  return ESC_OK;
}

static int check_zinc(const esc_zinc_gin_t* m, const esc_mol_batch_t* b, const float* ws, bool train, bool need_y) {
  ESC_REQUIRE(m && b && ws, "esc_zinc: null pointer");
  ESC_REQUIRE(m->num_layers >= 1 && m->num_layers <= ESC_MAX_LAYERS, "esc_zinc: %ld layers unsupported", (long)m->num_layers);
  ESC_REQUIRE(m->hidden > 0 && m->hidden % 4 == 0, "esc_zinc: hidden must be a multiple of 4");
  ESC_REQUIRE(m->node_emb.dim > 0 && m->node_emb.dim % 4 == 0 && m->edge_emb.dim > 0 && m->edge_emb.dim % 4 == 0,
              "esc_zinc: embedding widths must be multiples of 4");
  ESC_REQUIRE(m->conv[0].lin.in_dim == m->hidden + m->edge_emb.dim && m->conv[0].lin.out_dim == m->node_emb.dim,
              "esc_zinc: conv1.lin must map hidden + edge width to the node width");
  ESC_REQUIRE(m->node_readout == 0 || m->node_readout == 1, "esc_zinc: node_readout must be 0 or 1");
  ESC_REQUIRE(b->N >= 2 && b->E >= 2 && b->Z >= 0 && b->G >= (m->node_readout ? 1 : 2),
              "esc_zinc: batch needs >= 2 nodes, edges and %s (BatchNorm statistics)", m->node_readout ? "1 graph" : "graphs");
  ESC_REQUIRE(b->node_type && b->edge_type && b->graph_ptr && b->in_ptr && b->row_ptr &&
              (!train || ((b->y || !need_y) && b->out_ptr && b->col_ptr)), "esc_zinc: null batch arrays");
  ESC_REQUIRE(aligned16(ws), "esc_zinc: workspace must be 16-byte aligned");
  return ESC_OK;
}

static ZincCtx make_zinc(const esc_zinc_gin_t* m, const esc_mol_batch_t* b, float* ws, void* stream, bool train) {
  ZincCtx z{m, b, Ctx{nullptr, nullptr, plan_layout_zinc(m, b->N, b->E, b->Z, b->G, ws, train), stream, train}};
  z.c.act = 2;
  return z;
}

struct OgbLayer {
  float *hin, *e, *agg, *Y0, *hc, *hb;
  BnWs b0, bn;
  unsigned char* mask_h;
  float *tmp, *V0, *VA, *V1, *VB, *vn;
  BnWs vb0, vb1;
  unsigned char* mask_v;
  float* d_e;
};
struct OgbLayout {
  int64_t N, E, Z, G, H, L, T;
  float *Tcat, *dTcat, *h0, *hL;
  float *Zb, *Zd, *A0, *Yz, *Yzd, *Zemb; BnWs zb0, zb1;
  unsigned char *mask_z0, *mask_z1;
  OgbLayer l[ESC_MAX_LAYERS];
  float *h[ESC_MAX_LAYERS + 1];
  float *pooled, *logits, *dlogits;
  float *dpooled, *dHa, *dHb, *dT, *dA1, *dagg, *dZemb, *dYz, *dA0, *dvn_a, *dvn_b, *dG1, *dG2, *dtmp, *poolG;
  float *deps_part, *bag_scratch, *emb_scratch, *emb_scratch_n, *slabs, *bn_scratch, *col_stats, *bn_scratch_e, *col_stats_e;
  float *bst_part;
  int64_t total;
};

static unsigned char* take_bytes(Arena& a, int64_t n) { return reinterpret_cast<unsigned char*>(a.take((n + 3) / 4)); }

static OgbLayout plan_layout_ogb(const esc_ogb_gnn_t* m, int64_t N, int64_t E, int64_t Z, int64_t G, int64_t atom_entries,
                                 int64_t bond_entries, float* base, bool train) {
  OgbLayout y{};
  Arena a{base, 0};
  const int64_t H = m->hidden, L = m->num_layers, T = m->num_tasks, H2 = 2 * H;
  const bool drop = train && m->drop_ratio > 0.f;
  y.N = N; y.E = E; y.Z = Z; y.G = G; y.H = H; y.L = L; y.T = T;
  const int64_t rows_total = m->atom_rows + L * m->bond_rows;
  y.Tcat = a.take(rows_total * H);
  y.h0 = a.take(N * H); y.h[0] = y.h0;
  y.Zb = a.take(E * H); y.Zd = drop ? a.take(E * H) : y.Zb; y.A0 = a.take(E * H);
  y.Yz = a.take(E * H); y.Yzd = drop ? a.take(E * H) : y.Yz; y.Zemb = a.take(E * H);
  y.zb0 = take_bn(a, H); y.zb1 = take_bn(a, H);
  if (drop) { y.mask_z0 = take_bytes(a, E * H); y.mask_z1 = take_bytes(a, E * H); }
  for (int l = 0; l < L; ++l) {
    OgbLayer& q = y.l[l];
    q.vn = a.take(G * H);
    q.hin = a.take(N * H);
    q.e = a.take(E * H);
    q.agg = a.take(N * H);
    q.Y0 = a.take(N * H2); q.hc = a.take(N * H); q.hb = nullptr;
    q.b0 = take_bn(a, H2); q.bn = take_bn(a, H);
    y.h[l + 1] = a.take(N * H);
    if (drop) q.mask_h = take_bytes(a, N * H);
    if (l < L - 1) {
      q.tmp = a.take(G * H); q.V0 = a.take(G * H2); q.VA = a.take(G * H2); q.V1 = a.take(G * H); q.VB = nullptr;
      q.vb0 = take_bn(a, H2); q.vb1 = take_bn(a, H);
      if (drop) q.mask_v = take_bytes(a, G * H);
    }
  }
  y.hL = y.h[L];
  y.pooled = a.take(G * H); y.logits = a.take(G * T); y.dlogits = a.take(G * T);
  y.bn_scratch = a.take(esc_bn_scratch(H2));
  y.col_stats = a.take(2 * ((E > N ? E : N) / 32 + 1) * H2);
  y.bn_scratch_e = a.take(esc_bn_scratch(H2));
  y.col_stats_e = a.take(2 * (E / 32 + 1) * H2);
  if (train) {
    y.dTcat = a.take(rows_total * H);
    y.bst_part = a.take(2 * (N / 64 + 2) * H2);
    y.dpooled = a.take(G * H); y.dHa = a.take(N * H); y.dHb = a.take(N * H); y.dT = a.take(N * H);
    y.dA1 = a.take(N * H2); y.dagg = a.take(N * H);
    y.dZemb = a.take(E * H); y.dYz = a.take(E * H); y.dA0 = a.take(E * H);
    y.dvn_a = a.take(G * H); y.dvn_b = a.take(G * H); y.dG1 = a.take(G * H2); y.dG2 = a.take(G * H); y.dtmp = a.take(G * H);
    y.poolG = a.take(G * H);
    for (int l = 0; l < L; ++l) y.l[l].d_e = a.take(E * H);
    y.deps_part = a.take(2 * N * (L > 0 ? L : 1));
    y.bag_scratch = a.take(esc_bag_bwd_scratch(Z, H));
    const int64_t ent = atom_entries > bond_entries ? atom_entries : bond_entries;
    y.emb_scratch = a.take(esc_bag_bwd_scratch(ent, H));
    y.emb_scratch_n = a.take(esc_bag_bwd_scratch(ent, H));
    int64_t sl = esc_linear_bwd_weight_scratch(E, H, H) + 64;
    for (int l = 0; l < L; ++l) {
      sl += esc_linear_bwd_weight_scratch(E, H, H) + esc_linear_bwd_weight_scratch(N, H2, H) +
            esc_linear_bwd_weight_scratch(N, H, H2) + 3 * 64;
      if (l < L - 1) sl += esc_linear_bwd_weight_scratch(G, H2, H) + esc_linear_bwd_weight_scratch(G, H, H2) + 2 * 64;
    }
    sl += esc_linear_bwd_weight_scratch(G, T, H) + 64;
    y.slabs = a.take(sl);
  }
  y.total = a.off;
  return y;
}

struct OgbCtx {
  const esc_ogb_gnn_t* m;
  const esc_ogb_batch_t* b;
  OgbLayout o;
  Ctx c;
  float p;
};

static uint64_t drop_seed(const OgbCtx& z, int which) { return z.b->seed * 0x2545F4914F6CDD1Dull + (uint64_t)(which + 1) * 0xD1342543DE82EF95ull; }

static int forward_ogb(const OgbCtx& z) {
  const esc_ogb_gnn_t* m = z.m;
  const esc_ogb_batch_t* b = z.b;
  const OgbLayout& y = z.o;
  const Ctx& c = z.c;
  const int64_t N = y.N, E = y.E, H = y.H, L = y.L, G = y.G, T = y.T, H2 = 2 * H;
  const float p = z.p;
  ESC_TRY(esc_table_pack(&m->tables, H, y.Tcat, c.s));
  EdgeStream& es = edge_stream_for(E);
  Ctx ce = c;
  if (es.ok) {
    ESC_TRY(chain(es.z_ready, (hipStream_t)c.s, es.stream));
    ce = edge_ctx(c, es.stream);
  }
  ESC_TRY(esc_bag_fwd_rows(m->z_table, m->z_rows, H, b->row_ptr, b->bag_idx, b->bag_val, E, y.Zb, H, 0, nullptr, ce.s));
  if (c.train) ESC_TRY(esc_bag_bwd_classify(b->col_row, y.Z, H, E, y.bag_scratch, ce.s));
  if (p > 0.f) ESC_TRY(esc_dropout_fwd(y.Zb, H, E, H, p, drop_seed(z, 0), nullptr, 0, y.Zd, H, y.mask_z0, ce.s));
  ESC_TRY(bn_coeffs(ce, y.Zd, H, E, m->zbn0, y.zb0));
  ESC_TRY(esc_affine_act(y.Zd, H, E, H, y.zb0.scale, y.zb0.shift, 1, y.A0, H, ce.s));
  if (p > 0.f) {
    ESC_TRY(esc_linear_fwd(y.A0, H, m->zlin.w, H, m->zlin.b, nullptr, nullptr, E, H, H, y.Yz, H, nullptr, ce.s));
    ESC_TRY(esc_dropout_fwd(y.Yz, H, E, H, p, drop_seed(z, 1), nullptr, 0, y.Yzd, H, y.mask_z1, ce.s));
    ESC_TRY(bn_coeffs(ce, y.Yzd, H, E, m->zbn1, y.zb1));
  } else {
    ESC_TRY(linear_bn(ce, y.A0, H, m->zlin, nullptr, nullptr, E, y.Yz, m->zbn1, y.zb1));
  }
  ESC_TRY(esc_affine_act(y.Yzd, H, E, H, y.zb1.scale, y.zb1.shift, 1, y.Zemb, H, ce.s));
  auto edge_term = [&](int l) -> int {
    const LdsFloorGuard cap(ce.on_edge_stream);
    const esc_ogb_layer_t& q = m->layer[l];
    ESC_TRY(esc_linear_fwd(y.Zemb, H, q.pos.w, H, q.pos.b, nullptr, nullptr, E, H, H, y.l[l].e, H, nullptr, ce.s));
    ESC_TRY(esc_bag_fwd_rows(y.Tcat + q.bond_row0 * H, m->bond_rows, H, b->bonds.row_ptr, b->bonds.idx, b->bonds.ones, E, y.l[l].e, H, 1, nullptr, ce.s));
    if (es.ok && hipEventRecord(es.e_ready[l], es.stream) != hipSuccess) { set_error("esc_ogb: stream event failed"); return ESC_ELAUNCH; }
    return ESC_OK;
  };
  const int ahead = es.ok ? 1 : (int)L;
  for (int l = 0; l < (int)L && l < ahead; ++l) ESC_TRY(edge_term(l));
  ESC_TRY(esc_bag_fwd_rows(y.Tcat, m->atom_rows, H, b->atoms.row_ptr, b->atoms.idx, b->atoms.ones, N, y.h0, H, 0, nullptr, c.s));
  ESC_TRY(esc_embed_fwd(m->vn_w, 1, H, b->zero_idx, G, y.l[0].vn, H, nullptr, c.s));
  for (int l = 0; l < (int)L; ++l) {
    const esc_ogb_layer_t& q = m->layer[l];
    const OgbLayer& w = y.l[l];
    ESC_TRY(esc_segment_broadcast_add(y.h[l], H, w.vn, H, b->graph_ptr, G, N, H, w.hin, H, c.s));
    if (es.ok && hipStreamWaitEvent((hipStream_t)c.s, es.e_ready[l], 0) != hipSuccess) { set_error("esc_ogb: stream event failed"); return ESC_ELAUNCH; }
    ESC_TRY(esc_gine_aggregate_fwd(w.hin, H, w.e, H, b->in_ptr, b->in_edge, b->in_src, q.eps, N, H, w.agg, H, c.s));
    if (es.ok && l + ahead < (int)L) {
      ESC_TRY(chain(es.agg_done[l], (hipStream_t)c.s, es.stream));
      ESC_TRY(edge_term(l + ahead));
    }
    ESC_TRY(linear_bn(c, w.agg, H, q.lin0, nullptr, nullptr, N, w.Y0, q.bn0, w.b0));
    ESC_TRY(linear_bn(c, w.Y0, H2, q.lin1, w.b0.scale, w.b0.shift, N, w.hc, q.bn, w.bn));
    ESC_TRY(esc_affine_act_dropout_fwd(w.hc, H, N, H, w.bn.scale, w.bn.shift, l == (int)L - 1 ? 0 : 1, p, drop_seed(z, 2 + 2 * l),
                                       m->residual ? w.hin : nullptr, H, y.h[l + 1], H, w.mask_h, c.s));
    if (l < (int)L - 1) {
      ESC_TRY(esc_segment_pool_fwd(w.hin, H, b->graph_ptr, G, H, 0, w.tmp, H, c.s));
      ESC_TRY(esc_dropout_fwd(w.tmp, H, G, H, 0.f, 0, w.vn, H, w.tmp, H, nullptr, c.s));
      ESC_TRY(linear_bn(c, w.tmp, H, q.vlin0, nullptr, nullptr, G, w.V0, q.vbn0, w.vb0));
      ESC_TRY(esc_affine_act(w.V0, H2, G, H2, w.vb0.scale, w.vb0.shift, 1, w.VA, H2, c.s));
      ESC_TRY(linear_bn(c, w.VA, H2, q.vlin1, nullptr, nullptr, G, w.V1, q.vbn1, w.vb1));
      ESC_TRY(esc_affine_act_dropout_fwd(w.V1, H, G, H, w.vb1.scale, w.vb1.shift, 1, p, drop_seed(z, 3 + 2 * l),
                                         m->residual ? w.vn : nullptr, H, y.l[l + 1].vn, H, w.mask_v, c.s));
    }
  }
  ESC_TRY(esc_segment_pool_fwd(y.hL, H, b->graph_ptr, G, H, m->mean_pool, y.pooled, H, c.s));
  ESC_TRY(esc_linear_fwd(y.pooled, H, m->head.w, H, m->head.b, nullptr, nullptr, G, T, H, y.logits, T, nullptr, c.s));
  if (es.ok) ESC_TRY(chain(es.joined, es.stream, (hipStream_t)c.s));
  return ESC_OK;
}

static int backward_ogb(const OgbCtx& z) {
  const esc_ogb_gnn_t* m = z.m;
  const esc_ogb_batch_t* b = z.b;
  const OgbLayout& y = z.o;
  const Ctx& c = z.c;
  Ctx c0 = c; c0.act = 0;
  const int64_t N = y.N, E = y.E, H = y.H, L = y.L, G = y.G, T = y.T, H2 = 2 * H;
  const float p = z.p;
  ESC_TRY(linear_backward(c, y.dlogits, T, y.pooled, H, nullptr, nullptr, m->head, G, y.dpooled, H, 0));
  float* dH = y.dHa;
  float* dHin = y.dHb;
  ESC_TRY(esc_segment_pool_bwd(y.dpooled, H, b->graph_ptr, G, H, m->mean_pool, dH, H, c.s));
  float* dvn_next = nullptr;
  float* dvn_cur = y.dvn_a;
  std::vector<esc_sum_job> eps_jobs;
  EdgeStream& es = edge_stream_for(E);
  Ctx ce = es.ok ? edge_ctx(c, es.stream) : c;
  std::vector<esc_reduce_job> edge_jobs;
  edge_jobs.reserve(ESC_MAX_REDUCE_JOBS);
  if (es.ok && c.jobs) ce.jobs = &edge_jobs;
  if (es.ok) ESC_TRY(chain(es.z_ready, (hipStream_t)c.s, es.stream));
  for (int l = (int)L - 1; l >= 0; --l) {
    const esc_ogb_layer_t& q = m->layer[l];
    const OgbLayer& w = y.l[l];
    const bool last = l == (int)L - 1;
    ESC_TRY(bn_backward_drop(last ? c0 : c, w.hc, H, dH, H, N, w.bn, q.bn, w.mask_h, p, 0, y.dT, H, y.bn_scratch));
    bool hidden_done = false;
    if (kBnBwdSumsFromDx && !sync_on(c) && y.bst_part != nullptr) {
      const esc_bn_bwd_next n0{y.bst_part, w.Y0, H2, w.b0.mean, w.b0.invstd, w.b0.scale, w.b0.shift, 1};
      const float* slab_probe = c.jobs ? *c.slab_cursor : c.y.slabs;
      if (esc_linear_bwd_both_bn_ok(y.dT, H, nullptr, w.Y0, H2, q.lin1.w, H2, N, H, H2, y.dA1, H2, slab_probe, &n0)) {
        float* slabs = c.y.slabs;
        esc_reduce_job* job = nullptr;
        if (c.jobs) {
          slabs = *c.slab_cursor;
          *c.slab_cursor += (esc_linear_bwd_weight_scratch(N, H, H2) + 63) & ~63LL;
          c.jobs->emplace_back();
          job = &c.jobs->back();
        }
        ESC_TRY(esc_linear_bwd_both_bn(y.dT, H, nullptr, w.Y0, H2, w.b0.scale, w.b0.shift, q.lin1.w, H2, N, H, H2, y.dA1, H2, 0, q.lin1.dw, H2,
                                       q.lin1.db, slabs, job, &n0, c.s));
        ESC_TRY(esc_bn_bwd_coef_from_partials(y.bst_part, cdiv(N, esc_linear_bwd_bn_block_rows(N, H, H2)), N, H2, w.b0.coef, q.bn0.dgamma,
                                              q.bn0.dbeta, c.s));
        ESC_TRY(esc_bn_bwd_apply(w.Y0, H2, nullptr, 0, y.dA1, H2, N, H2, w.b0.mean, w.b0.invstd, q.bn0.gamma, q.bn0.beta, 1, w.b0.coef, y.dA1, H2, c.s));
        hidden_done = true;
      }
    }
    if (!hidden_done) {
      ESC_TRY(linear_backward(c, y.dT, H, w.Y0, H2, w.b0.scale, w.b0.shift, q.lin1, N, y.dA1, H2, 0));
      ESC_TRY(bn_backward(c, w.Y0, H2, nullptr, 0, y.dA1, H2, N, w.b0, q.bn0, y.dA1, H2, y.bn_scratch, H2));
    }
    ESC_TRY(linear_backward(c, y.dA1, H2, w.agg, H, nullptr, nullptr, q.lin0, N, y.dagg, H, 0));
    bool have_dhin = false;
    if (!last) {
      ESC_TRY(bn_backward_drop(c, w.V1, H, dvn_next, H, G, w.vb1, q.vbn1, w.mask_v, p, 0, y.dG2, H, y.bn_scratch));
      ESC_TRY(linear_backward(c, y.dG2, H, w.VA, H2, nullptr, nullptr, q.vlin1, G, y.dG1, H2, 0));
      ESC_TRY(bn_backward(c, w.V0, H2, nullptr, 0, y.dG1, H2, G, w.vb0, q.vbn0, y.dG1, H2, y.bn_scratch, H2));
      ESC_TRY(linear_backward(c, y.dG1, H2, w.tmp, H, nullptr, nullptr, q.vlin0, G, y.dtmp, H, 0));
      ESC_TRY(esc_dropout_bwd(y.dtmp, H, G, H, 0.f, nullptr, m->residual ? dvn_next : nullptr, H, dvn_cur, H, c.s));
      ESC_TRY(esc_segment_broadcast_add(m->residual ? dH : nullptr, H, y.dtmp, H, b->graph_ptr, G, N, H, dHin, H, c.s));
      have_dhin = true;
    } else if (m->residual) {
      float* t = dH; dH = dHin; dHin = t;
      have_dhin = true;
    }
    ESC_TRY(esc_gine_aggregate_bwd(w.hin, H, w.e, H, y.dagg, H, b->out_ptr, b->out_edge, b->out_dst, q.eps, N, H, w.d_e, H,
                                   dHin, H, have_dhin ? 1 : 0, y.deps_part + (int64_t)l * 2 * N, c.s));
    eps_jobs.push_back(esc_sum_job{y.deps_part + (int64_t)l * 2 * N, N * esc_gine_aggregate_bwd_deps_slots(H), q.deps});
    if (es.ok) ESC_TRY(chain(es.de_ready[l], (hipStream_t)c.s, es.stream));
    const bool bonds_on_node = l == 0 && es.ok;
    ESC_TRY(esc_bag_bwd_table(w.d_e, H, H, b->bonds.col_ptr, b->bonds.c_row, b->bonds.ones, b->bonds.c_col, b->bonds.n_entries,
                              m->bond_rows, y.dTcat + q.bond_row0 * H, bonds_on_node ? y.emb_scratch_n : y.emb_scratch,
                              bonds_on_node ? c.s : ce.s));
    ESC_TRY(linear_backward(ce, w.d_e, H, y.Zemb, H, nullptr, nullptr, q.pos, E, y.dZemb, H, last ? 0 : 1));
    ESC_TRY(esc_segment_pool_fwd(dHin, H, b->graph_ptr, G, H, 0, y.poolG, H, c.s));
    ESC_TRY(esc_dropout_bwd(y.poolG, H, G, H, 0.f, nullptr, last ? nullptr : dvn_cur, H, dvn_cur, H, c.s));
    dvn_next = dvn_cur;
    dvn_cur = dvn_cur == y.dvn_a ? y.dvn_b : y.dvn_a;
    { float* t = dH; dH = dHin; dHin = t; }
  }
  ESC_TRY(esc_bag_bwd_table(dH, H, H, b->atoms.col_ptr, b->atoms.c_row, b->atoms.ones, b->atoms.c_col, b->atoms.n_entries,
                            m->atom_rows, y.dTcat, y.emb_scratch_n, c.s));
  ESC_TRY(esc_embed_bwd(dvn_next, H, b->zero_idx, G, 1, H, m->vn_dw, c.s));
  ESC_TRY(bn_backward_drop(ce, y.Yzd, H, y.dZemb, H, E, y.zb1, m->zbn1, y.mask_z1, p, 1, y.dYz, H, ce.y.bn_scratch));
  ESC_TRY(linear_backward(ce, y.dYz, H, y.A0, H, nullptr, nullptr, m->zlin, E, y.dA0, H, 0));
  ESC_TRY(bn_backward_drop(ce, y.Zd, H, y.dA0, H, E, y.zb0, m->zbn0, y.mask_z0, p, 1, y.dA0, H, ce.y.bn_scratch));
  ESC_TRY(esc_bag_bwd_table_rows(y.dA0, H, H, b->col_ptr, b->col_row, b->col_val, b->col_col, y.Z, m->z_rows, E, 1,
                                 m->dz_table, y.bag_scratch, ce.s));
  if (es.ok && !edge_jobs.empty()) ESC_TRY(esc_slab_reduce_jobs(edge_jobs.data(), (int)edge_jobs.size(), es.stream));
  if (!eps_jobs.empty()) ESC_TRY(esc_reduce_sum_jobs(eps_jobs.data(), (int)eps_jobs.size(), c.s));
  if (c.jobs && !c.jobs->empty()) ESC_TRY(esc_slab_reduce_jobs(c.jobs->data(), (int)c.jobs->size(), c.s));
  if (es.ok) ESC_TRY(chain(es.joined, es.stream, (hipStream_t)c.s));
  return esc_table_unpack_grad(&m->tables, H, y.dTcat, c.s);
}

static int check_ogb(const esc_ogb_gnn_t* m, const esc_ogb_batch_t* b, const float* ws, bool train, bool need_y) {
  ESC_REQUIRE(m && b && ws, "esc_ogb: null pointer");
  ESC_REQUIRE(m->num_layers >= 1 && m->num_layers <= ESC_MAX_LAYERS, "esc_ogb: %ld layers unsupported", (long)m->num_layers);
  ESC_REQUIRE(m->hidden > 0 && m->hidden % 4 == 0 && m->num_tasks >= 1, "esc_ogb: hidden must be a multiple of 4");
  ESC_REQUIRE(m->drop_ratio >= 0.f && m->drop_ratio < 1.f, "esc_ogb: drop_ratio %g outside [0,1)", (double)m->drop_ratio);
  ESC_REQUIRE(m->tables.count > 0 && m->tables.count <= ESC_MAX_TABLES && m->atom_rows > 0 && m->bond_rows > 0 && m->vn_w,
              "esc_ogb: encoder tables missing");
  ESC_REQUIRE(b->N >= 2 && b->E >= 2 && b->Z >= 0 && b->G >= 2, "esc_ogb: batch needs >= 2 nodes, edges and graphs (BatchNorm statistics)");
  ESC_REQUIRE(b->graph_ptr && b->zero_idx && b->in_ptr && b->row_ptr && b->atoms.row_ptr && b->atoms.idx && b->atoms.ones &&
              b->bonds.row_ptr && b->bonds.idx && b->bonds.ones, "esc_ogb: null batch arrays");
  ESC_REQUIRE(!train || ((b->y || !need_y) && b->out_ptr && b->col_ptr && b->atoms.col_ptr && b->atoms.c_row && b->atoms.c_col &&
                         b->bonds.col_ptr && b->bonds.c_row && b->bonds.c_col && m->vn_dw), "esc_ogb: null training arrays");
  ESC_REQUIRE(aligned16(ws), "esc_ogb: workspace must be 16-byte aligned");
  return ESC_OK;
}

static OgbCtx make_ogb(const esc_ogb_gnn_t* m, const esc_ogb_batch_t* b, float* ws, void* stream, bool train) {
  OgbCtx z{m, b, plan_layout_ogb(m, b->N, b->E, b->Z, b->G, b->atoms.n_entries, b->bonds.n_entries, ws, train),
           Ctx{nullptr, nullptr, Layout{}, stream, train}, train ? m->drop_ratio : 0.f};
  z.c.y.H = m->hidden; z.c.y.N = b->N; z.c.y.E = b->E;
  z.c.y.col_stats = z.o.col_stats; z.c.y.bn_scratch = z.o.bn_scratch; z.c.y.slabs = z.o.slabs;
  z.c.y.col_stats_e = z.o.col_stats_e; z.c.y.bn_scratch_e = z.o.bn_scratch_e;
  z.c.act = 1;
  return z;
}

static int check(const esc_nested_gin_t* m, const esc_batch_t* b, const float* ws, bool train, bool need_y = true) {
  ESC_REQUIRE(m && b && ws, "esc_engine: null pointer");
  ESC_REQUIRE(m->num_layers >= 1 && m->num_layers <= ESC_MAX_LAYERS, "esc_engine: %ld layers unsupported", (long)m->num_layers);
  ESC_REQUIRE(m->hidden > 0 && m->hidden % 4 == 0 && m->in_dim > 0, "esc_engine: hidden must be a multiple of 4");
  ESC_REQUIRE(b->N >= 2 && b->E >= 2 && b->Z >= 0, "esc_engine: batch needs >= 2 nodes and edges (BatchNorm statistics)");
  ESC_REQUIRE(b->x && b->in_ptr && b->row_ptr && (!train || ((b->y || !need_y) && b->out_ptr && b->col_ptr)), "esc_engine: null batch arrays");
  ESC_REQUIRE(aligned16(ws), "esc_engine: workspace must be 16-byte aligned");
  ESC_REQUIRE(m->n_counters >= 0 && m->n_counters <= ESC_MAX_BN_COUNTERS, "esc_engine: bad BatchNorm counter list");
  for (int64_t i = 0; i < m->n_counters; ++i) ESC_REQUIRE(m->counters[i] != nullptr, "esc_engine: null BatchNorm counter");
  return ESC_OK;
}

static int copy_floats(float* dst, const float* src, int64_t n, void* stream, const char* what) {
  if (hipMemcpyAsync(dst, src, sizeof(float) * (size_t)n, hipMemcpyDeviceToDevice, (hipStream_t)stream) != hipSuccess) {
    set_error("%s: copy failed", what);
    return ESC_ELAUNCH;
  }
  return ESC_OK;
}

struct JobList {
  std::vector<esc_reduce_job> jobs;
  float* cursor = nullptr;
};

static void arm_jobs(Ctx& c, JobList& l, float* slabs, int64_t budget, bool always = false) {
  if (!always) l.jobs.reserve(ESC_MAX_REDUCE_JOBS);
  l.cursor = slabs;
  if (always || budget <= ESC_MAX_REDUCE_JOBS) { c.jobs = &l.jobs; c.slab_cursor = &l.cursor; }
}

}

using namespace esc;

extern "C" {

int esc_engine_set_two_stream_min_edges(int64_t edges) {
  g_two_stream_min_edges = edges < 0 ? 0 : edges;
  return ESC_OK;
}

int esc_engine_set_side_stream(int on) {
  g_use_edge_stream = (on & 2) != 0;
  g_plain_events = (on & 64) != 0;
  g_readout_one_launch = (on & 128) != 0;
  return ESC_OK;
}

int esc_engine_phase_times(double* out, int skip) {
  PhaseRing& p = phases();
  for (int i = 0; i < 6; ++i) out[i] = 0.0;
  if (!p.on || p.steps < 2) return 0;
  const int first = p.steps > PhaseRing::RING ? p.steps - PhaseRing::RING + 1 : 0;
  int n = 0;
  for (int sidx = first + skip; sidx < p.steps; ++sidx) {
    hipEvent_t* e = p.ev[sidx % PhaseRing::RING];
    bool ok = true;
    for (int k = 0; k < PH_COUNT; ++k) ok = ok && e[k] != nullptr;
    if (!ok) continue;
    float t[6] = {};
    if (hipEventElapsedTime(&t[0], e[PH_START], e[PH_EDGE_FWD_DONE]) != hipSuccess) continue;
    (void)hipEventElapsedTime(&t[1], e[PH_START], e[PH_NODE_FWD_DONE]);
    (void)hipEventElapsedTime(&t[2], e[PH_NODE_FWD_DONE], e[PH_NODE_BWD_DONE]);
    if (hipEventElapsedTime(&t[3], e[PH_NODE_BWD_DONE], e[PH_EDGE_BWD_DONE]) != hipSuccess) {
      (void)hipEventElapsedTime(&t[3], e[PH_EDGE_BWD_DONE], e[PH_NODE_BWD_DONE]); t[3] = -t[3];
    }
    (void)hipEventElapsedTime(&t[4], e[PH_START], e[PH_END]);
    if (sidx + 1 < p.steps) (void)hipEventElapsedTime(&t[5], e[PH_END], p.ev[(sidx + 1) % PhaseRing::RING][PH_START]);
    for (int i = 0; i < 6; ++i) out[i] += t[i];
    ++n;
  }
  for (int i = 0; i < 6; ++i) out[i] /= n > 0 ? n : 1;
  return n;
}

int esc_engine_set_collective(esc_allreduce_fn fn, void* user, int rank, int world, float* buf_node, float* buf_edge,
                              int64_t cap) {
  ESC_REQUIRE(fn == nullptr || (world >= 1 && rank >= 0 && rank < world && buf_node && buf_edge && cap > 0),
              "esc_engine_set_collective: bad argument");
  g_coll = Collective{fn, user, rank, world < 1 ? 1 : world, buf_node, buf_edge, cap};
  return ESC_OK;
}

int64_t esc_engine_workspace_floats(const esc_nested_gin_t* m, int64_t N, int64_t E, int64_t Z) {
  if (!m || N < 0 || E < 0 || Z < 0) return -1;
  return plan_layout(m, N, E, Z, nullptr, true).total;
}

static int train_step_impl(const esc_nested_gin_t* m, const esc_batch_t* b, float* workspace,
                           int64_t loss_denom, float* loss, float* pred, void* stream, Pending* defer);

int esc_engine_train_step(const esc_nested_gin_t* m, const esc_batch_t* b, float* workspace,
                          int64_t loss_denom, float* loss, float* pred, void* stream) {
  ESC_TRY(finish_pending(pending()));
  return train_step_impl(m, b, workspace, loss_denom, loss, pred, stream, nullptr);
}

int esc_engine_train_step_begin(const esc_nested_gin_t* m, const esc_batch_t* b, float* workspace,
                                int64_t loss_denom, float* loss, float* pred, void* stream) {
  ESC_TRY(finish_pending(pending()));
  return train_step_impl(m, b, workspace, loss_denom, loss, pred, stream, &pending());
}

int esc_engine_train_step_end(void) { return finish_pending(pending()); }

static int train_step_impl(const esc_nested_gin_t* m, const esc_batch_t* b, float* workspace,
                           int64_t loss_denom, float* loss, float* pred, void* stream, Pending* defer) {
  int rc = check(m, b, workspace, true);
  if (rc) return rc;
  ESC_REQUIRE(loss, "esc_engine_train_step: null loss pointer");
  Ctx c{m, b, plan_layout(m, b->N, b->E, b->Z, workspace, true), stream, true};
  JobList jobs;
  arm_jobs(c, jobs, c.y.slabs, 3 * m->num_layers + 7);
  const int64_t denom = loss_denom > 0 ? loss_denom : b->N;
  EdgeStream& es = edge_stream_for(b->E);
  const bool head_l1 = es.ok && m->hidden <= 1024 &&
                       esc_linear_fwd_l1_ok(c.y.Yl, m->hidden, m->lin2.w, m->hidden, c.y.bl.scale, c.y.bl.shift) != 0;
  if (head_l1) { c.l1_target = b->y; c.l1_denom = denom; }
  ESC_TRY(forward(c));
  if (head_l1) {
    ESC_TRY(esc_l1_loss(c.y.pred, b->y, b->N, denom, 1.0f, loss, nullptr, es.stream));
  } else {
    ESC_TRY(esc_l1_loss(c.y.pred, b->y, b->N, denom, 1.0f, loss, c.y.dpred, stream));
  }
  mark(PH_NODE_FWD_DONE, stream);
  if (pred) ESC_TRY(copy_floats(pred, c.y.pred, b->N, stream, "esc_engine_train_step"));
  return backward(c, defer);
}

int esc_engine_forward_train(const esc_nested_gin_t* m, const esc_batch_t* b, float* workspace, float* pred,
                             void* stream) {
  ESC_TRY(finish_pending(pending()));
  int rc = check(m, b, workspace, true, false);
  if (rc) return rc;
  ESC_REQUIRE(pred, "esc_engine_forward_train: null output");
  Ctx c{m, b, plan_layout(m, b->N, b->E, b->Z, workspace, true), stream, true};
  JobList jobs;
  arm_jobs(c, jobs, c.y.slabs, 0, true);
  ESC_TRY(forward(c));
  return copy_floats(pred, c.y.pred, b->N, stream, "esc_engine_forward_train");
}

int esc_engine_backward(const esc_nested_gin_t* m, const esc_batch_t* b, float* workspace, const float* dpred,
                        void* stream) {
  ESC_TRY(finish_pending(pending()));
  int rc = check(m, b, workspace, true, false);
  if (rc) return rc;
  ESC_REQUIRE(dpred, "esc_engine_backward: null gradient");
  Ctx c{m, b, plan_layout(m, b->N, b->E, b->Z, workspace, true), stream, true};
  JobList jobs;
  arm_jobs(c, jobs, c.y.slabs, 3 * m->num_layers + 7);
  ESC_TRY(copy_floats(c.y.dpred, dpred, b->N, stream, "esc_engine_backward"));
  return backward(c, nullptr);
}

int esc_engine_predict(const esc_nested_gin_t* m, const esc_batch_t* b, float* workspace, float* pred,
                       void* stream) {
  ESC_TRY(finish_pending(pending()));
  int rc = check(m, b, workspace, false);
  if (rc) return rc;
  ESC_REQUIRE(pred, "esc_engine_predict: null output");
  Ctx c{m, b, plan_layout(m, b->N, b->E, b->Z, workspace, false), stream, false};
  ESC_TRY(forward(c));
  return copy_floats(pred, c.y.pred, b->N, stream, "esc_engine_predict");
}

int64_t esc_zinc_workspace_floats(const esc_zinc_gin_t* m, int64_t N, int64_t E, int64_t Z, int64_t G) {
  if (!m || N < 0 || E < 0 || Z < 0 || G < 0) return -1;
  return plan_layout_zinc(m, N, E, Z, G, nullptr, true).total + 64;
}

static int64_t zinc_rows(const esc_zinc_gin_t* m, const esc_mol_batch_t* b) { return m->node_readout ? b->N : b->G; }

int esc_zinc_train_step(const esc_zinc_gin_t* m, const esc_mol_batch_t* b, float* workspace, int64_t loss_denom,
                        float* loss, float* pred, void* stream) {
  ESC_TRY(finish_pending(pending()));
  int rc = check_zinc(m, b, workspace, true, true);
  if (rc) return rc;
  ESC_REQUIRE(loss, "esc_zinc_train_step: null loss pointer");
  ZincCtx z = make_zinc(m, b, workspace, stream, true);
  JobList jobs;
  arm_jobs(z.c, jobs, z.c.y.slabs, 3 * m->num_layers + 3);
  const int64_t R = zinc_rows(m, b);
  ESC_TRY(forward_zinc(z));
  ESC_TRY(esc_l1_loss(z.c.y.pred, b->y, R, loss_denom > 0 ? loss_denom : R, 1.0f, loss, z.c.y.dpred, stream));
  if (pred) ESC_TRY(copy_floats(pred, z.c.y.pred, R, stream, "esc_zinc_train_step"));
  return backward_zinc(z);
}

int esc_zinc_forward_train(const esc_zinc_gin_t* m, const esc_mol_batch_t* b, float* workspace, float* pred, void* stream) {
  ESC_TRY(finish_pending(pending()));
  int rc = check_zinc(m, b, workspace, true, false);
  if (rc) return rc;
  ESC_REQUIRE(pred, "esc_zinc_forward_train: null output");
  ZincCtx z = make_zinc(m, b, workspace, stream, true);
  JobList jobs;
  arm_jobs(z.c, jobs, z.c.y.slabs, 0, true);
  ESC_TRY(forward_zinc(z));
  return copy_floats(pred, z.c.y.pred, zinc_rows(m, b), stream, "esc_zinc_forward_train");
}

int esc_zinc_backward(const esc_zinc_gin_t* m, const esc_mol_batch_t* b, float* workspace, const float* dpred, void* stream) {
  ESC_TRY(finish_pending(pending()));
  int rc = check_zinc(m, b, workspace, true, false);
  if (rc) return rc;
  ESC_REQUIRE(dpred, "esc_zinc_backward: null gradient");
  ZincCtx z = make_zinc(m, b, workspace, stream, true);
  JobList jobs;
  arm_jobs(z.c, jobs, z.c.y.slabs, 3 * m->num_layers + 3);
  ESC_TRY(copy_floats(z.c.y.dpred, dpred, zinc_rows(m, b), stream, "esc_zinc_backward"));
  return backward_zinc(z);
}

int esc_zinc_predict(const esc_zinc_gin_t* m, const esc_mol_batch_t* b, float* workspace, float* pred, void* stream) {
  ESC_TRY(finish_pending(pending()));
  int rc = check_zinc(m, b, workspace, false, false);
  if (rc) return rc;
  ESC_REQUIRE(pred, "esc_zinc_predict: null output");
  ZincCtx z = make_zinc(m, b, workspace, stream, false);
  ESC_TRY(forward_zinc(z));
  return copy_floats(pred, z.c.y.pred, zinc_rows(m, b), stream, "esc_zinc_predict");
}

int64_t esc_ogb_workspace_floats(const esc_ogb_gnn_t* m, int64_t N, int64_t E, int64_t Z, int64_t G, int64_t atom_entries,
                                 int64_t bond_entries) {
  if (!m || N < 0 || E < 0 || Z < 0 || G < 0 || atom_entries < 0 || bond_entries < 0) return -1;
  return plan_layout_ogb(m, N, E, Z, G, atom_entries, bond_entries, nullptr, true).total + 64;
}

int esc_ogb_train_step(const esc_ogb_gnn_t* m, const esc_ogb_batch_t* b, float* workspace, int64_t loss_denom, float* loss,
                       float* logits, void* stream) {
  ESC_TRY(finish_pending(pending()));
  int rc = check_ogb(m, b, workspace, true, true);
  if (rc) return rc;
  ESC_REQUIRE(loss, "esc_ogb_train_step: null loss pointer");
  OgbCtx z = make_ogb(m, b, workspace, stream, true);
  JobList jobs;
  arm_jobs(z.c, jobs, z.o.slabs, 5 * m->num_layers + 2);
  ESC_TRY(forward_ogb(z));
  ESC_TRY(esc_bce_logits_loss(z.o.logits, b->y, b->G * m->num_tasks, loss_denom, loss, z.o.dlogits, stream));
  if (logits) ESC_TRY(copy_floats(logits, z.o.logits, b->G * m->num_tasks, stream, "esc_ogb_train_step"));
  return backward_ogb(z);
}

int esc_ogb_forward_train(const esc_ogb_gnn_t* m, const esc_ogb_batch_t* b, float* workspace, float* logits, void* stream) {
  ESC_TRY(finish_pending(pending()));
  int rc = check_ogb(m, b, workspace, true, false);
  if (rc) return rc;
  ESC_REQUIRE(logits, "esc_ogb_forward_train: null output");
  OgbCtx z = make_ogb(m, b, workspace, stream, true);
  JobList jobs;
  arm_jobs(z.c, jobs, z.o.slabs, 0, true);
  ESC_TRY(forward_ogb(z));
  return copy_floats(logits, z.o.logits, b->G * m->num_tasks, stream, "esc_ogb_forward_train");
}

int esc_ogb_backward(const esc_ogb_gnn_t* m, const esc_ogb_batch_t* b, float* workspace, const float* dlogits, void* stream) {
  ESC_TRY(finish_pending(pending()));
  int rc = check_ogb(m, b, workspace, true, false);
  if (rc) return rc;
  ESC_REQUIRE(dlogits, "esc_ogb_backward: null gradient");
  OgbCtx z = make_ogb(m, b, workspace, stream, true);
  JobList jobs;
  arm_jobs(z.c, jobs, z.o.slabs, 5 * m->num_layers + 2);
  ESC_TRY(copy_floats(z.o.dlogits, dlogits, b->G * m->num_tasks, stream, "esc_ogb_backward"));
  return backward_ogb(z);
}

int esc_ogb_predict(const esc_ogb_gnn_t* m, const esc_ogb_batch_t* b, float* workspace, float* logits, void* stream) {
  ESC_TRY(finish_pending(pending()));
  int rc = check_ogb(m, b, workspace, false, false);
  if (rc) return rc;
  ESC_REQUIRE(logits, "esc_ogb_predict: null output");
  OgbCtx z = make_ogb(m, b, workspace, stream, false);
  ESC_TRY(forward_ogb(z));
  return copy_floats(logits, z.o.logits, b->G * m->num_tasks, stream, "esc_ogb_predict");
}

}
```

### esc-gnn_amd/csrc/optim.hip

```cpp
#include "common.h"

namespace esc {

__global__ __launch_bounds__(1024) void l1_loss_kernel(const float* __restrict__ pred, const float* __restrict__ y,
                                                       int64_t M, double denom, float grad_scale,
                                                       float* __restrict__ loss, float* __restrict__ dpred) {
  ESC_PRIO();
  __shared__ double sh[16];
  double acc = 0.0;
  const float gs = (float)((double)grad_scale / denom);
  for (int64_t i = threadIdx.x; i < M; i += blockDim.x) {
    const float d = pred[i] - y[i];
    acc += (double)fabsf(d);
    if (dpred) dpred[i] = d > 0.f ? gs : (d < 0.f ? -gs : 0.f);
  }
  acc = wave_sum(acc);
  if ((threadIdx.x & 63) == 0) sh[threadIdx.x >> 6] = acc;
  __syncthreads();
  if (threadIdx.x == 0) {
    double t = 0.0;
    for (int w = 0; w < 16; ++w) t += sh[w];
    loss[0] = (float)(t / denom);
  }
}

__global__ __launch_bounds__(1024) void bce_logits_kernel(const float* __restrict__ pred, const float* __restrict__ y,
                                                          int64_t M, double denom_in, float* __restrict__ loss,
                                                          float* __restrict__ dpred) {
  ESC_PRIO();
  __shared__ double sh[16];
  __shared__ double shc[16];
  double acc = 0.0, cnt = 0.0;
  for (int64_t i = threadIdx.x; i < M; i += blockDim.x) {
    const float t = y[i], x = pred[i];
    if (t == t) {
      acc += (double)(fmaxf(x, 0.f) - x * t + log1pf(expf(-fabsf(x))));
      cnt += 1.0;
    }
  }
  acc = wave_sum(acc);
  cnt = wave_sum(cnt);
  if ((threadIdx.x & 63) == 0) { sh[threadIdx.x >> 6] = acc; shc[threadIdx.x >> 6] = cnt; }
  __syncthreads();
  double t = 0.0, c = 0.0;
  for (int w = 0; w < 16; ++w) { t += sh[w]; c += shc[w]; }
  const double denom = denom_in > 0.0 ? denom_in : c;
  if (threadIdx.x == 0) loss[0] = denom > 0.0 ? (float)(t / denom) : 0.f;
  if (dpred) {
    const float inv = denom > 0.0 ? (float)(1.0 / denom) : 0.f;
    for (int64_t i = threadIdx.x; i < M; i += blockDim.x) {
      const float tt = y[i], x = pred[i];
      const float sg = 1.f / (1.f + expf(-x));
      dpred[i] = (tt == tt) ? (sg - tt) * inv : 0.f;
    }
  }
}

__global__ __launch_bounds__(256) void adam_kernel(float* __restrict__ p, const float* __restrict__ g,
                                                   float* __restrict__ m, float* __restrict__ v, int64_t n,
                                                   float one_minus_b1, float b2, float one_minus_b2,
                                                   float bc2_sqrt, float eps, float neg_step,
                                                   const float* __restrict__ grad_denom) {
  ESC_PRIO();
  const float den = grad_denom ? grad_denom[0] : 1.f;
  for (int64_t i = (int64_t)blockIdx.x * blockDim.x + threadIdx.x; i < n; i += (int64_t)gridDim.x * blockDim.x) {
    const float gi = grad_denom ? g[i] / den : g[i];
    const float mi = m[i] + one_minus_b1 * (gi - m[i]);
    const float vi = v[i] * b2 + one_minus_b2 * gi * gi;
    m[i] = mi;
    v[i] = vi;
    const float denom = sqrtf(vi) / bc2_sqrt + eps;
    p[i] = p[i] + neg_step * (mi / denom);
  }
}

}

using namespace esc;

extern "C" {

int esc_l1_loss(const float* pred, const float* y, int64_t M, int64_t denom, float grad_scale, float* loss,
                float* dpred, void* stream) {
  ESC_REQUIRE(pred && y && loss, "esc_l1_loss: null pointer");
  ESC_REQUIRE(M > 0 && denom > 0, "esc_l1_loss: empty batch");
  esc::launch(-1, l1_loss_kernel, dim3(1), dim3(1024), 0, (hipStream_t)stream, pred, y, M, (double)denom, grad_scale, loss, dpred);
  ESC_CHECK_LAUNCH("esc_l1_loss");
  return ESC_OK;
}

int esc_bce_logits_loss(const float* pred, const float* y, int64_t M, int64_t denom, float* loss, float* dpred,
                        void* stream) {
  ESC_REQUIRE(pred && y && loss, "esc_bce_logits_loss: null pointer");
  ESC_REQUIRE(M > 0, "esc_bce_logits_loss: empty batch");
  esc::launch(-1, bce_logits_kernel, dim3(1), dim3(1024), 0, (hipStream_t)stream, pred, y, M, (double)denom, loss, dpred);
  ESC_CHECK_LAUNCH("esc_bce_logits_loss");
  return ESC_OK;
}

int esc_adam_step(float* param, const float* grad, float* exp_avg, float* exp_avg_sq, int64_t n,
                  double lr, double beta1, double beta2, double eps, int64_t step, void* stream) {
  return esc_adam_step_scaled(param, grad, exp_avg, exp_avg_sq, n, lr, beta1, beta2, eps, step, nullptr, stream);
}

int esc_adam_step_scaled(float* param, const float* grad, float* exp_avg, float* exp_avg_sq, int64_t n,
                         double lr, double beta1, double beta2, double eps, int64_t step,
                         const float* grad_denom, void* stream) {
  ESC_REQUIRE(param && grad && exp_avg && exp_avg_sq, "esc_adam_step: null pointer");
  ESC_REQUIRE(n >= 0 && step >= 1, "esc_adam_step: bad n/step");
  if (n == 0) return ESC_OK;
  const double bc1 = 1.0 - pow(beta1, (double)step);
  const double bc2 = 1.0 - pow(beta2, (double)step);
  const unsigned blocks = (unsigned)(cdiv(n, 256) < 2048 ? cdiv(n, 256) : 2048);
  esc::launch(-1, adam_kernel, dim3(blocks), dim3(256), 0, (hipStream_t)stream, param, grad, exp_avg, exp_avg_sq, n,
                     (float)(1.0 - beta1), (float)beta2, (float)(1.0 - beta2), (float)sqrt(bc2), (float)eps,
                     (float)(-lr / bc1), grad_denom);
  ESC_CHECK_LAUNCH("esc_adam_step");
  return ESC_OK;
}

}
```

### esc-gnn_amd/engine.py

```python
import collections
import ctypes
import functools
from ctypes import c_void_p

import torch

from . import _native as nv
from .nested import Z_TABLE_ROWS
from .plan import plan_of

MAX_LAYERS, MAX_BN_COUNTERS, MAX_TABLES = (nv.const(n) for n in ("ESC_MAX_LAYERS", "ESC_MAX_BN_COUNTERS", "ESC_MAX_TABLES"))

_Linear, _BN, _MLP, _Conv = (nv.struct(n) for n in ("esc_linear_t", "esc_bn_t", "esc_mlp_t", "esc_conv_t"))
_Model, _Batch = nv.struct("esc_nested_gin_t"), nv.struct("esc_batch_t")
_Embed, _ZincModel, _MolBatch = nv.struct("esc_embed_t"), nv.struct("esc_zinc_gin_t"), nv.struct("esc_mol_batch_t")
_TableList, _OgbLayer, _OgbModel = nv.struct("esc_table_list"), nv.struct("esc_ogb_layer_t"), nv.struct("esc_ogb_gnn_t")
_BagPlan, _OgbBatch = nv.struct("esc_bag_plan_t"), nv.struct("esc_ogb_batch_t")


def _names(cls):
    return [m[0] for m in nv.members(cls)]


_PLAN_FIELDS = tuple(_names(_Batch)[_names(_Batch).index("in_ptr"):])
assert all(set(_PLAN_FIELDS) <= set(_names(b)) for b in (_MolBatch, _OgbBatch)), "batch structs without the plan's index arrays"


def _bind_plan(b, plan):
    for f in _PLAN_FIELDS:
        setattr(b, f, getattr(plan, f).data_ptr())


def _f32c(t):
    return t if (t.dtype == torch.float32 and t.is_contiguous()) else t.float().contiguous()


def _grad_ptr(p):
    if p.grad is None:
        p.grad = torch.zeros_like(p.data)
    return p.grad.data_ptr()


def _lin(mod, gp=_grad_ptr):
    s = _Linear()
    s.w, s.dw = mod.weight.data_ptr(), gp(mod.weight)
    s.b, s.db = (mod.bias.data_ptr(), gp(mod.bias)) if mod.bias is not None else (None, None)
    s.in_dim, s.out_dim = mod.in_features, mod.out_features
    return s


def _bn(mod, gp=_grad_ptr):
    s = _BN()
    s.gamma, s.beta = mod.weight.data_ptr(), mod.bias.data_ptr()
    s.dgamma, s.dbeta = gp(mod.weight), gp(mod.bias)
    s.running_mean, s.running_var = mod.running_mean.data_ptr(), mod.running_var.data_ptr()
    s.eps, s.momentum = mod.eps, mod.momentum
    return s


def _mlp(seq, gp=_grad_ptr):
    s = _MLP()
    s.lin0, s.bn0, s.lin1, s.bn1 = _lin(seq[0], gp), _bn(seq[2], gp), _lin(seq[4], gp), _bn(seq[6], gp)
    return s


def describe(m, gp=_grad_ptr):
    d = _Model()
    convs = [m.conv1] + list(m.convs)
    if len(convs) > MAX_LAYERS:
        raise ValueError("at most %d layers" % MAX_LAYERS)
    d.num_layers, d.hidden = len(convs), m.lin2.in_features
    d.in_dim, d.z_rows = m.x_embedding[0].in_features, m.z_initial.num_embeddings
    d.z_table, d.dz_table = m.z_initial.weight.data_ptr(), gp(m.z_initial.weight)
    d.zbn0, d.zlin, d.zbn1 = _bn(m.z_embedding[1], gp), _lin(m.z_embedding[3], gp), _bn(m.z_embedding[5], gp)
    d.xemb = _mlp(m.x_embedding, gp)
    for i, cv in enumerate(convs):
        c = _Conv()
        c.eps, c.deps = cv.eps.data_ptr(), gp(cv.eps)
        c.nn, c.lin = _mlp(cv.nn, gp), _lin(cv.lin, gp)
        d.conv[i] = c
    d.lin1, d.bn_lin1, d.lin2 = _lin(m.lin1, gp), _bn(m.bn_lin1, gp), _lin(m.lin2, gp)
    counters = _bn_counters(m)
    if len(counters) > MAX_BN_COUNTERS:
        raise ValueError("at most %d BatchNorm step counters" % MAX_BN_COUNTERS)
    d.n_counters = len(counters)
    for i, t in enumerate(counters):
        if t.dtype != torch.int64 or t.device != m.lin1.weight.device:
            raise RuntimeError("step engine: num_batches_tracked must be an int64 tensor on the model's device")
        d.counters[i] = t.data_ptr()
    return d


def _bn_counters(m):
    return [mod.num_batches_tracked for mod in m.modules()
            if isinstance(mod, torch.nn.BatchNorm1d) and mod.num_batches_tracked is not None]


def _bns(m, cache=None):
    if cache is None:
        cache = m.__dict__.get("_esc_node_cache")
        if cache is not None and not cache.valid():
            cache = None
    if cache is not None:
        return cache.bns
    return [mod for mod in m.modules() if hasattr(mod, "sync_group")]


def _sync_groups(m, cache=None):
    return [mod.sync_group for mod in _bns(m, cache) if mod.sync_group is not False]


def engine_supports(m, cache=None):
    if m.graph_pred or m.dropout != 0 or not m.use_cycle or m.lin1.weight.device.type != "cuda":
        return False
    if m.lin2.out_features != 1 or m.lin2.in_features % 4 != 0:
        return False
    return _one_sync_group(m, cache)


def _one_sync_group(m, cache=None):
    bns = _bns(m, cache)
    groups = [mod.sync_group for mod in bns if mod.sync_group is not False]
    return not groups or (len(groups) == len(bns) and all(g is groups[0] for g in groups))


def _bn_width(m, cache=None):
    mods = _bns(m, cache)
    return max([mod.num_features for mod in mods if isinstance(mod, torch.nn.BatchNorm1d)] or [1])


def _arm_collective(model, device, cache=None):
    groups = _sync_groups(model, cache)
    if not groups:
        return
    if not _one_sync_group(model, cache):
        raise NotImplementedError("step engine: all BatchNorm layers must share one sync group")
    width = _bn_width(model, cache)
    if _collective.get("group", False) is not groups[0] or _collective.get("width", 0) < width:
        install_collective(width, device, groups[0])


_ALLREDUCE_T = nv.callback("esc_allreduce_fn")
_collective = {}


def install_collective(hidden, device, group=None):
    import torch.distributed as dist
    if not (dist.is_available() and dist.is_initialized()) or dist.get_world_size(group) <= 1:
        nv.call("esc_engine_set_collective", None, None, 0, 1, None, None, 0)
        _collective.clear()
        return False
    world, rank = dist.get_world_size(group), dist.get_rank(group)
    cap = world * 3 * hidden
    bufs = [torch.zeros(cap, dtype=torch.float32, device=device) for _ in range(2)]
    by_ptr = {b.data_ptr(): b for b in bufs}

    def allreduce(buf, n, stream, user):
        try:
            t = by_ptr[buf][:n]
            cur = torch.cuda.current_stream(device)
            if stream is None or stream == cur.cuda_stream:
                dist.all_reduce(t, op=dist.ReduceOp.SUM, group=group)
            else:
                with torch.cuda.stream(torch.cuda.ExternalStream(stream, device=device)):
                    dist.all_reduce(t, op=dist.ReduceOp.SUM, group=group)
            return 0
        except Exception as exc:
            print("esc_gnn_amd: collective provider failed: %r" % (exc,))
            return 1

    cb = _ALLREDUCE_T(allreduce)
    nv.call("esc_engine_set_collective", ctypes.cast(cb, c_void_p), None, rank, world, bufs[0].data_ptr(), bufs[1].data_ptr(), cap)
    _collective.update(cb=cb, bufs=bufs, group=group, world=world, width=hidden)
    return True


class _AddressGuard(object):

    def _sentinels(self):
        ps = self._guard_params
        first, last = ps[0], ps[-1]
        g0, g1 = first.grad, last.grad
        bufs = self._guard_buffers
        return (first.data_ptr(), last.data_ptr(), g0.data_ptr() if g0 is not None else 0,
                g1.data_ptr() if g1 is not None else 0, bufs[0].data_ptr() if bufs else 0)

    def _guard_arm(self):
        self._guard_params = list(self.model.parameters())
        self._guard_buffers = [b for b in self.model.buffers() if b.is_floating_point()]
        self._guard_sig = self._sentinels()

    def _guard_check(self):
        if self._sentinels() != self._guard_sig:
            self.refresh()

    def _mark_bucket_written(self):
        bucket = _bucket_of(self._guard_params[0])
        if bucket is not None:
            bucket._clean_version = None


def _bucket_of(param):
    from .parallel import _BUCKETS
    g = param.grad
    base = getattr(g, "_base", None) if g is not None else None
    return _BUCKETS.get(base.data_ptr()) if base is not None else None


def _count_batch(model, data, need_y):
    dev = model.lin1.weight.device
    if data.x.device != dev:
        data.to(dev)
    plan = plan_of(data)
    if plan.in_ptr.device != dev:
        raise RuntimeError("StepEngine: batch plan lives on %s, model on %s" % (plan.in_ptr.device, dev))
    b = _Batch()
    b.N, b.E, b.Z = plan.num_nodes, plan.num_edges, plan.nnz
    x = data.x if data.x.is_contiguous() else data.x.contiguous()
    b.x = x.data_ptr()
    y = None
    if need_y:
        y = _f32c(data.y.reshape(-1))
        if y.numel() != plan.num_nodes:
            raise ValueError("StepEngine: expected one target per node")
        b.y = y.data_ptr()
    _bind_plan(b, plan)
    return b, (x, y, plan)


def _embed(mod, gp=_grad_ptr):
    s = _Embed()
    s.w, s.dw = mod.weight.data_ptr(), gp(mod.weight)
    s.rows, s.dim = mod.num_embeddings, mod.embedding_dim
    return s


def describe_zinc(m, gp=_grad_ptr):
    d = _ZincModel()
    convs = [m.conv1] + list(m.convs)
    if len(convs) > MAX_LAYERS:
        raise ValueError("at most %d layers" % MAX_LAYERS)
    d.num_layers, d.hidden, d.z_rows = len(convs), m.lin2.in_features, m.z_initial.num_embeddings
    d.z_table, d.dz_table = m.z_initial.weight.data_ptr(), gp(m.z_initial.weight)
    d.zbn0, d.zlin, d.zbn1 = _bn(m.z_embedding[1], gp), _lin(m.z_embedding[3], gp), _bn(m.z_embedding[5], gp)
    d.node_emb, d.edge_emb = _embed(m.node_type_embedding, gp), _embed(m.edge_type_embedding, gp)
    for i, cv in enumerate(convs):
        c = _Conv()
        c.eps, c.deps = cv.eps.data_ptr(), gp(cv.eps)
        c.nn, c.lin = _mlp(cv.nn, gp), _lin(cv.lin, gp)
        d.conv[i] = c
    d.lin1, d.bn_lin1, d.lin2 = _lin(m.lin1, gp), _bn(m.bn_lin1, gp), _lin(m.lin2, gp)
    d.node_readout = int(bool(getattr(m, "node_readout", False)))
    return d


def _zinc_rows(m, b):
    return b.N if getattr(m, "node_readout", False) else b.G


def zinc_engine_supports(m, data=None):
    from .zinc_models import NestedGIN_eff
    if not isinstance(m, NestedGIN_eff):
        return False
    if m.dropout != 0 or m.lin1.weight.device.type != "cuda" or m.lin2.out_features != 1 or not _one_sync_group(m):
        return False
    if data is not None:
        if "edge_pos" in data or "pos_batch" not in data or data.edge_index.size(1) < 2 or data["edge_attr"] is None:
            return False
    return True


def zinc_engine_ready(m, data):
    if not zinc_engine_supports(m, data):
        return False
    from .plan import graph_ptr_of
    plan = plan_of(data, Z_TABLE_ROWS)
    if getattr(m, "node_readout", False):
        return plan.num_nodes >= 2
    return graph_ptr_of(data, plan)[1] >= 2


def _zinc_batch(model, data, need_y, y=None):
    from .plan import graph_ptr_of
    dev = model.lin1.weight.device
    if data.edge_index.device != dev:
        data.to(dev)
    plan = plan_of(data, Z_TABLE_ROWS)
    gptr, G = graph_ptr_of(data, plan)
    b = _MolBatch()
    b.N, b.E, b.Z, b.G = plan.num_nodes, plan.num_edges, plan.nnz, G
    nt = data.x.reshape(-1)
    et = data.edge_attr.reshape(-1)
    nt = nt if (nt.dtype == torch.int64 and nt.is_contiguous()) else nt.to(torch.int64).contiguous()
    et = et if (et.dtype == torch.int64 and et.is_contiguous()) else et.to(torch.int64).contiguous()
    if nt.numel() != b.N or et.numel() != b.E:
        raise ValueError("ZINC engine: expected one type id per node and per edge")
    rng, sig = data.__dict__.get("_esc_int_ranges") or ({}, {})
    for key, src, ids, rows in (("x", data.x, nt, model.node_type_embedding.num_embeddings),
                                ("edge_attr", data.edge_attr, et, model.edge_type_embedding.num_embeddings)):
        r = rng.get(key) if sig.get(key) == (src.data_ptr(), src._version) else None
        if r is not None and min(r[0]) >= 0 and max(r[1]) < rows:
            continue
        seen = getattr(src, "_esc_zinc_checked", None)
        if seen == (src._version, rows):
            continue
        if ids.numel() and (int(ids.min()) < 0 or int(ids.max()) >= rows):
            raise IndexError("ZINC engine: %s holds a type id outside the %d-row embedding table" % (key, rows))
        src._esc_zinc_checked = (src._version, rows)
    b.node_type, b.edge_type, b.graph_ptr = nt.data_ptr(), et.data_ptr(), gptr.data_ptr()
    if need_y:
        y = _f32c((data.y if y is None else y).reshape(-1))
        if y.numel() != _zinc_rows(model, b):
            raise ValueError("ZINC engine: expected one target per %s" % ("node" if getattr(model, "node_readout", False) else "graph"))
        if y.device != dev:
            y = y.to(dev)
        b.y = y.data_ptr()
    _bind_plan(b, plan)
    return b, (nt, et, y, plan, gptr)


def ogb_engine_supports(m, data=None):
    from .ogb_mol_gnn import AtomEncoder, BondEncoder
    g = m.gnn_node
    if g.JK != "last" or not g.virtual_node or g.skip_node_encoder or m.graph_pooling not in ("sum", "mean") or not _one_sync_group(m):
        return False
    if m.graph_pred_linear.weight.device.type != "cuda" or m.emb_dim % 4 != 0 or not isinstance(g.node_encoder, AtomEncoder):
        return False
    if not all(isinstance(cv.edge_encoder, BondEncoder) for cv in g.convs):
        return False
    if data is not None:
        if "edge_pos" in data or "pos_batch" not in data or data.edge_index.size(1) < 2 or data["edge_attr"] is None:
            return False
        if data.x.dim() != 2 or data.x.size(1) != 9 or data.edge_attr.dim() != 2 or data.edge_attr.size(1) != 3:
            return False
    return True


def describe_ogb(m, gp=_grad_ptr):
    g = m.gnn_node
    L = g.num_layer
    if L > MAX_LAYERS:
        raise ValueError("at most %d layers" % MAX_LAYERS)
    d = _OgbModel()
    d.num_layers, d.hidden, d.z_rows, d.num_tasks = L, m.emb_dim, g.z_initial.num_embeddings, m.num_tasks
    d.residual, d.mean_pool, d.drop_ratio = int(bool(g.residual)), int(m.graph_pooling == "mean"), float(g.drop_ratio)
    d.z_table, d.dz_table = g.z_initial.weight.data_ptr(), gp(g.z_initial.weight)
    d.zbn0, d.zlin, d.zbn1 = _bn(g.z_embedding[1], gp), _lin(g.z_embedding[3], gp), _bn(g.z_embedding[5], gp)
    tabs = list(g.node_encoder.atom_embedding_list)
    d.atom_rows = sum(t.num_embeddings for t in tabs)
    bond_rows = sum(t.num_embeddings for t in g.convs[0].edge_encoder.bond_embedding_list)
    d.bond_rows = bond_rows
    for l, cv in enumerate(g.convs):
        tabs += list(cv.edge_encoder.bond_embedding_list)
    if len(tabs) > MAX_TABLES:
        raise ValueError("too many embedding tables for the OGB engine")
    d.tables.count = len(tabs)
    for j, t in enumerate(tabs):
        d.tables.rows[j], d.tables.w[j], d.tables.dw[j] = t.num_embeddings, t.weight.data_ptr(), gp(t.weight)
    d.vn_w, d.vn_dw = g.virtualnode_embedding.weight.data_ptr(), gp(g.virtualnode_embedding.weight)
    for l, cv in enumerate(g.convs):
        q = _OgbLayer()
        q.eps, q.deps = cv.eps.data_ptr(), gp(cv.eps)
        q.pos = _lin(cv.edge_encoder_pos, gp)
        q.lin0, q.bn0, q.lin1 = _lin(cv.mlp[0], gp), _bn(cv.mlp[1], gp), _lin(cv.mlp[3], gp)
        q.bn = _bn(g.batch_norms[l], gp)
        if l < L - 1:
            v = g.mlp_virtualnode_list[l]
            q.vlin0, q.vbn0, q.vlin1, q.vbn1 = _lin(v[0], gp), _bn(v[1], gp), _lin(v[3], gp), _bn(v[4], gp)
        q.bond_row0 = d.atom_rows + l * bond_rows
        d.layer[l] = q
    d.head = _lin(m.graph_pred_linear, gp)
    return d


def _bag_plan(plan):
    b = _BagPlan()
    b.n_entries = plan["entries"]
    b.row_ptr, b.idx, b.ones = plan["row_ptr"].data_ptr(), plan["idx32"].data_ptr(), plan["ones"].data_ptr()
    b.col_ptr, b.c_row, b.c_col = plan["col_ptr"].data_ptr(), plan["c_row"].data_ptr(), plan["c_col"].data_ptr()
    return b


_zero_idx = {}


def _ogb_batch(model, data, need_y, seed=0):
    from .ogb_mol_gnn import ATOM_FEATURE_DIMS, BOND_FEATURE_DIMS
    from .ops import embed_plan
    from .plan import graph_ptr_of
    dev = model.graph_pred_linear.weight.device
    if data.edge_index.device != dev:
        data.to(dev)
    plan = plan_of(data, Z_TABLE_ROWS)
    gptr, G = graph_ptr_of(data, plan)
    rng, sig = data.__dict__.get("_esc_int_ranges") or ({}, {})

    def known(key):
        t = data[key]
        return rng.get(key) if sig.get(key) == (t.data_ptr(), t._version) else None
    pa = embed_plan(data.x, ATOM_FEATURE_DIMS, known("x"))
    pb = embed_plan(data.edge_attr, BOND_FEATURE_DIMS, known("edge_attr"))
    b = _OgbBatch()
    b.N, b.E, b.Z, b.G = plan.num_nodes, plan.num_edges, plan.nnz, G
    if data.x.size(0) != b.N or data.edge_attr.size(0) != b.E:
        raise ValueError("OGB engine: expected one feature row per node and per edge")
    b.atoms, b.bonds = _bag_plan(pa), _bag_plan(pb)
    zero = _zero_idx.get(dev)
    if zero is None or zero.numel() < G:
        zero = _zero_idx[dev] = torch.zeros(max(G, 1024), dtype=torch.int64, device=dev)
    b.graph_ptr, b.zero_idx, b.seed = gptr.data_ptr(), zero.data_ptr(), int(seed) & ((1 << 64) - 1)
    y = None
    if need_y:
        y = _f32c(data.y.reshape(G, -1))
        if y.size(1) != model.num_tasks:
            raise ValueError("OGB engine: expected [num_graphs, num_tasks] targets")
        b.y = y.data_ptr()
    _bind_plan(b, plan)
    return b, (y, plan, gptr, pa, pb, zero)


def ogb_engine_ready(m, data):
    if not ogb_engine_supports(m, data):
        return False
    from .plan import graph_ptr_of
    return graph_ptr_of(data, plan_of(data, Z_TABLE_ROWS))[1] >= 2


def _drop_seed(model):
    n = model.__dict__.get("_esc_drop_step", 0)
    model.__dict__["_esc_drop_step"] = n + 1
    return (torch.initial_seed() * 0x9E3779B97F4A7C15 + n) & ((1 << 64) - 1)


_Family = collections.namedtuple("_Family", "prefix describe struct device batch sizes pred_shape py_counters dropout")

COUNTING = _Family("esc_engine_", describe, _Model, lambda m: m.lin1.weight.device, _count_batch,
                   lambda b: (b.N, b.E, b.Z), lambda m, b: (b.N, 1), py_counters=False, dropout=False)
ZINC = _Family("esc_zinc_", describe_zinc, _ZincModel, lambda m: m.lin1.weight.device, _zinc_batch,
               lambda b: (b.N, b.E, b.Z, b.G), lambda m, b: (_zinc_rows(m, b), 1), py_counters=True, dropout=False)
OGB = _Family("esc_ogb_", describe_ogb, _OgbModel, lambda m: m.graph_pred_linear.weight.device, _ogb_batch,
              lambda b: (b.N, b.E, b.Z, b.G, b.atoms.n_entries, b.bonds.n_entries), lambda m, b: (b.G, m.num_tasks),
              py_counters=True, dropout=True)


def _training_args(family, model):
    return {"seed": _drop_seed(model)} if family.dropout else {}


def _workspace_floats(family, desc, b):
    return getattr(nv.lib(), family.prefix + "workspace_floats")(ctypes.byref(desc), *family.sizes(b))


class _NodeCache(object):

    MARK = 0x5E5C00000000

    def __init__(self, model, family):
        import numpy as np
        self.family = family
        self.params = list(model.parameters())
        self.buffers = [b for b in model.buffers() if b.is_floating_point()]
        self.counters = _bn_counters(model)
        self.key = tuple(t.data_ptr() for t in self.params + self.buffers + self.counters)
        self.bns = [m for m in model.modules() if hasattr(m, "sync_group")]
        with torch.enable_grad():
            p0 = self.params[0]
            self.acc0 = p0.view_as(p0).grad_fn.next_functions[0][0] if p0.requires_grad else None
        index = {id(p): i for i, p in enumerate(self.params)}
        self.template = family.describe(model, lambda p: self.MARK + index[id(p)])
        words = np.frombuffer(self.template, dtype=np.uint64)
        hits = np.nonzero((words >= self.MARK) & (words < self.MARK + len(self.params)))[0]
        self.slots = hits
        self.slot_param = (words[hits] - self.MARK).astype(np.int64)
        offs, total = [], 0
        for p in self.params:
            offs.append(total)
            total += -(-p.numel() // 16) * 16
        self.offsets, self.total = offs, total
        self.byte_offsets = np.asarray(offs, dtype=np.uint64)[self.slot_param] * np.uint64(4)

    def valid(self):
        return self.key == tuple(t.data_ptr() for t in self.params + self.buffers + self.counters)

    def descriptor(self, grad_base):
        import numpy as np
        d = self.family.struct.from_buffer_copy(self.template)
        np.frombuffer(d, dtype=np.uint64)[self.slots] = np.uint64(grad_base) + self.byte_offsets
        return d

    def descriptor_at(self, addresses):
        import numpy as np
        d = self.family.struct.from_buffer_copy(self.template)
        np.frombuffer(d, dtype=np.uint64)[self.slots] = np.asarray(addresses, dtype=np.uint64)[self.slot_param]
        return d

    def owning_bucket(self):
        bucket = _bucket_of(self.params[0])
        if bucket is None or not bucket.engine_direct:
            return None
        for p in self.params:
            if not p.requires_grad or p._backward_hooks or getattr(p, "_post_accumulate_grad_hooks", None):
                return None
        return bucket

    def direct_bucket(self):
        bucket = self.owning_bucket()
        return bucket.direct_grad_addresses(self.params) if bucket is not None else None

    def node_inputs(self):
        return (self.params[0],) if self.owning_bucket() is not None else tuple(self.params)


def _under_autograd_grad(cache):
    if cache.acc0 is None:
        return False
    try:
        torch._C._will_engine_execute_node(cache.acc0)
        return False
    except RuntimeError as exc:
        return "autograd.grad" in str(exc)
    except Exception:
        return False


def _node_backward(ctx, dpred, entry):
    cache = ctx.cache
    if ctx.ws is None:
        raise RuntimeError("esc_gnn_amd: this engine node's workspace was released by its first backward; a second "
                           "backward through the same forward (retain_graph=True) needs the per-op path")
    g = _f32c(dpred.reshape(-1))
    slim = ctx.n_in < len(cache.params)
    none = (None, None, None) + (None,) * ctx.n_in

    def run(desc):
        nv.call(entry, ctypes.byref(desc), ctypes.byref(ctx.b), ctx.ws.data_ptr(), g.data_ptr(), nv.stream())
        ctx.ws = ctx.keep = None

    if _under_autograd_grad(cache):
        flat = torch.empty(cache.total, dtype=torch.float32, device=dpred.device)
        run(cache.descriptor(flat.data_ptr()))
        grads = tuple(flat[o:o + p.numel()].view(p.shape) if p.requires_grad else None
                      for p, o in zip(cache.params[:ctx.n_in], cache.offsets[:ctx.n_in]))
        return (None, None, None) + grads

    bucket = cache.owning_bucket()
    direct = bucket.direct_grad_addresses(cache.params) if bucket is not None else None
    if direct is not None:
        run(cache.descriptor_at(direct))
        return none
    if slim:
        offs = bucket.grad_offsets(cache.params) if bucket is not None else None
        if offs is not None:
            tmp = torch.zeros_like(bucket.flat_grad)
            run(cache.descriptor_at([tmp.data_ptr() + 4 * o for o in offs]))
            bucket.flat_grad.add_(tmp)
            return none
        flat = torch.zeros(cache.total, dtype=torch.float32, device=dpred.device)
        run(cache.descriptor(flat.data_ptr()))
        for p, o in zip(cache.params, cache.offsets):
            gp = flat[o:o + p.numel()].view(p.shape)
            if p.grad is None:
                p.grad = gp
            else:
                p.grad.add_(gp)
        return none
    flat = torch.empty(cache.total, dtype=torch.float32, device=dpred.device)
    run(cache.descriptor(flat.data_ptr()))
    grads = tuple(flat[o:o + p.numel()].view(p.shape) if p.requires_grad else None
                  for p, o in zip(cache.params, cache.offsets))
    return (None, None, None) + grads


def _node_cache(model, family):
    c = model.__dict__.get("_esc_node_cache")
    if c is None or not c.valid():
        c = model.__dict__["_esc_node_cache"] = _NodeCache(model, family)
    return c


def _private_workspace(family, desc, b, dev):
    return torch.empty(int(_workspace_floats(family, desc, b)), dtype=torch.float32, device=dev)


class _EngineNode(torch.autograd.Function):

    @staticmethod
    def forward(ctx, model, data, cache, *params):
        fam = cache.family
        dev = fam.device(model)
        b, keep = fam.batch(model, data, False, **_training_args(fam, model))
        desc = cache.descriptor(0)
        ws = _private_workspace(fam, desc, b, dev)
        pred = torch.empty(fam.pred_shape(model, b), dtype=torch.float32, device=dev)
        nv.call(fam.prefix + "forward_train", ctypes.byref(desc), ctypes.byref(b), ws.data_ptr(), pred.data_ptr(), nv.stream())
        if fam.py_counters and cache.counters:
            torch._foreach_add_(cache.counters, 1)
        ctx.cache, ctx.b, ctx.keep, ctx.ws, ctx.n_in = cache, b, keep, ws, len(params)
        return pred

    @staticmethod
    @torch.autograd.function.once_differentiable
    def backward(ctx, dpred):
        return _node_backward(ctx, dpred, ctx.cache.family.prefix + "backward")


def _engine_forward(family, model, data, cache=None):
    cache = cache if cache is not None else _node_cache(model, family)
    _arm_collective(model, family.device(model), cache)
    return _EngineNode.apply(model, data, cache, *cache.node_inputs())


@torch.no_grad()
def _predict(family, model, data, desc, workspace):
    b, keep = family.batch(model, data, False)
    ws = workspace(b)
    pred = torch.empty(family.pred_shape(model, b), dtype=torch.float32, device=ws.device)
    nv.call(family.prefix + "predict", ctypes.byref(desc), ctypes.byref(b), ws.data_ptr(), pred.data_ptr(), nv.stream())
    return pred


def _engine_predict(family, model, data):
    desc = _node_cache(model, family).descriptor(0)
    return _predict(family, model, data, desc, lambda b: _private_workspace(family, desc, b, family.device(model)))


engine_forward, engine_predict = functools.partial(_engine_forward, COUNTING), functools.partial(_engine_predict, COUNTING)
zinc_engine_forward, zinc_engine_predict = functools.partial(_engine_forward, ZINC), functools.partial(_engine_predict, ZINC)
ogb_engine_forward, ogb_engine_predict = functools.partial(_engine_forward, OGB), functools.partial(_engine_predict, OGB)


class _FamilyEngine(_AddressGuard):
    family = None

    def __init__(self, model):
        self.model = model
        self._ws = None
        _arm_collective(model, self.family.device(model))
        self.refresh()

    def refresh(self):
        fam, m = self.family, self.model
        self._desc = fam.describe(m)
        self._dev = fam.device(m)
        self._counters = _bn_counters(m) if fam.py_counters else []
        self._open = None
        self._guard_arm()

    def _workspace(self, b):
        need = _workspace_floats(self.family, self._desc, b)
        if self._ws is None or self._ws.numel() < need:
            self._ws = torch.empty(int(need * 1.25), dtype=torch.float32, device=self._dev)
        return self._ws

    def prepare(self, data):
        self.family.batch(self.model, data, False)
        return data

    def _step(self, entry, data, loss_denom, return_pred, **target):
        fam, m = self.family, self.model
        self._guard_check()
        b, keep = fam.batch(m, data, True, **target, **_training_args(fam, m))
        ws = self._workspace(b)
        loss = torch.empty(1, dtype=torch.float32, device=self._dev)
        pred = torch.empty(fam.pred_shape(m, b), dtype=torch.float32, device=self._dev) if return_pred else None
        nv.call(fam.prefix + entry, ctypes.byref(self._desc), ctypes.byref(b), ws.data_ptr(), int(loss_denom or 0),
                loss.data_ptr(), nv.ptr(pred), nv.stream())
        self._mark_bucket_written()
        if self._counters:
            torch._foreach_add_(self._counters, 1)
        self._open = (keep, ws) if entry.endswith("_begin") else None
        return (loss.view(()), pred) if return_pred else loss.view(())

    def train_step(self, data, loss_denom=None, return_pred=False):
        return self._step("train_step", data, loss_denom, return_pred)

    def predict(self, data):
        self._guard_check()
        return _predict(self.family, self.model, data, self._desc, self._workspace)


class StepEngine(_FamilyEngine):
    family = COUNTING

    def __init__(self, model):
        if model.graph_pred or model.dropout != 0 or not model.use_cycle:
            raise NotImplementedError("StepEngine covers the run_graphcount configuration "
                                      "(graph_pred=False, dropout=0, use_cycle=True); use model(batch) otherwise")
        if model.lin1.weight.device.type != "cuda":
            raise RuntimeError("StepEngine runs on the HIP device only; there is no CPU fallback")
        super().__init__(model)

    def begin_step(self, data, loss_denom=None, return_pred=False):
        return self._step("train_step_begin", data, loss_denom, return_pred)

    def end_step(self):
        nv.call("esc_engine_train_step_end")
        self._open = None


class ZincStepEngine(_FamilyEngine):
    family = ZINC

    def __init__(self, model):
        if not zinc_engine_supports(model):
            raise NotImplementedError("ZincStepEngine covers dropout 0, lin2 -> 1 output, BatchNorm on one sync group, on the HIP device")
        super().__init__(model)

    def train_step(self, data, loss_denom=None, return_pred=False, y=None):
        return self._step("train_step", data, loss_denom, return_pred, y=y)


class OgbStepEngine(_FamilyEngine):
    family = OGB

    def __init__(self, model):
        if not ogb_engine_supports(model):
            raise NotImplementedError("OgbStepEngine covers ogbg-mol* gin_eff with a virtual node, JK=last, sum/mean pooling")
        super().__init__(model)
```

### esc-gnn_amd/optim.py

```python
import math

import torch

from . import _native as nv
from .parallel import FlatBucket


class FlatAdam(FlatBucket):
    def __init__(self, params, lr=1e-3, betas=(0.9, 0.999), eps=1e-8, late=None, weight_decay=0.0):
        params = [p for p in params]
        if params and params[0].device.type != "cuda":
            raise RuntimeError("FlatAdam runs on the HIP device only; there is no CPU fallback")
        super().__init__(params, late=late)
        self.exp_avg = torch.zeros_like(self.flat_param)
        self.exp_avg_sq = torch.zeros_like(self.flat_param)
        self.param_groups = [dict(lr=lr, betas=betas, eps=eps, params=self.params)]
        if weight_decay:
            self.param_groups[0]["weight_decay"] = weight_decay
        self.step_count = 0

    def step(self, grad_denom=None):
        g = self.param_groups[0]
        self.step_count += 1
        if g.get("weight_decay"):
            self.flat_param.mul_(1.0 - float(g["lr"]) * float(g["weight_decay"]))
        nv.call("esc_adam_step_scaled", nv.ptr(self.flat_param), nv.ptr(self.flat_grad), nv.ptr(self.exp_avg),
                nv.ptr(self.exp_avg_sq), self.flat_param.numel(), float(g["lr"]), float(g["betas"][0]),
                float(g["betas"][1]), float(g["eps"]), self.step_count, nv.ptr(grad_denom), nv.stream())

    def clip_scale(self, max_norm):
        norm = torch.linalg.vector_norm(self.flat_grad)
        return ((norm + 1e-6) / float(max_norm)).clamp_(min=1.0).reshape(1)

    def state_dict(self):
        return dict(step=self.step_count, exp_avg=self.exp_avg, exp_avg_sq=self.exp_avg_sq,
                    param_groups=[{k: v for k, v in g.items() if k != "params"} for g in self.param_groups])

    def load_state_dict(self, sd):
        self.step_count = int(sd["step"])
        self.exp_avg.copy_(sd["exp_avg"])
        self.exp_avg_sq.copy_(sd["exp_avg_sq"])
        for g, s in zip(self.param_groups, sd["param_groups"]):
            g.update(s)


class ReduceLROnPlateau(object):

    def __init__(self, optimizer, mode="min", factor=0.1, patience=10, min_lr=0.0, threshold=1e-4):
        assert mode == "min"
        self.optimizer, self.factor, self.patience, self.min_lr, self.threshold = optimizer, factor, patience, min_lr, threshold
        self.best, self.num_bad = float("inf"), 0

    def step(self, metric):
        m = float(metric)
        if m < self.best * (1.0 - self.threshold):
            self.best, self.num_bad = m, 0
        else:
            self.num_bad += 1
        if self.num_bad > self.patience:
            for g in self.optimizer.param_groups:
                new = max(g["lr"] * self.factor, self.min_lr)
                if g["lr"] - new > 1e-8:
                    g["lr"] = new
            self.num_bad = 0


class CosineWithWarmup(object):

    def __init__(self, optimizer, num_warmup_epochs, max_epoch):
        self.optimizer, self.num_warmup_epochs, self.max_epoch = optimizer, int(num_warmup_epochs), int(max_epoch)
        self.base_lrs = [g["lr"] for g in optimizer.param_groups]
        self.last_epoch = -1
        self.step()

    def factor(self, epoch):
        if epoch < self.num_warmup_epochs:
            return max(1e-6, float(epoch) / float(max(1, self.num_warmup_epochs)))
        progress = float(epoch - self.num_warmup_epochs) / float(max(1, self.max_epoch - self.num_warmup_epochs))
        return max(0.0, 0.5 * (1.0 + math.cos(math.pi * 0.5 * 2.0 * progress)))

    def step(self, metric=None):
        self.last_epoch += 1
        for g, base in zip(self.optimizer.param_groups, self.base_lrs):
            g["lr"] = base * self.factor(self.last_epoch)
```

### esc-gnn_amd/store.py

```python
import ctypes

import numpy as np
import torch

from . import _native as nv
from .batch import Batch
from .plan import BatchPlan, plan_key, _sig

N_COLS = 1800


def _stable_group(key, n_keys):
    perm = torch.sort(key, stable=True)[1]
    ptr = torch.zeros(n_keys + 1, dtype=torch.int64, device=key.device)
    ptr[1:] = torch.cumsum(torch.bincount(key, minlength=n_keys), 0)
    return ptr, perm


class DeviceGraphStore(object):
    def __init__(self, data_list, device):
        if len(data_list) == 0:
            raise ValueError("DeviceGraphStore: empty dataset")
        dev = torch.device(device)
        if dev.type != "cuda":
            raise RuntimeError("DeviceGraphStore lives in HBM; there is no CPU fallback")
        self.device = dev
        G = len(data_list)
        n = torch.tensor([d.x.size(0) for d in data_list], dtype=torch.int64)
        e = torch.tensor([d.edge_index.size(1) for d in data_list], dtype=torch.int64)
        z = torch.tensor([d.pos_enc.numel() for d in data_list], dtype=torch.int64)
        ys = [d.y.reshape(d.y.size(0), -1) if d.y.dim() > 0 else d.y.reshape(1, 1) for d in data_list]
        yr = torch.tensor([t.size(0) for t in ys], dtype=torch.int64)

        def ptr(c):
            p = torch.zeros(G + 1, dtype=torch.int64)
            p[1:] = torch.cumsum(c, 0)
            return p
        self.h_node_ptr, self.h_edge_ptr, self.h_nnz_ptr, self.h_y_ptr = ptr(n), ptr(e), ptr(z), ptr(yr)
        self.node_ptr, self.edge_ptr = self.h_node_ptr.to(dev), self.h_edge_ptr.to(dev)
        self.nnz_ptr, self.y_ptr = self.h_nnz_ptr.to(dev), self.h_y_ptr.to(dev)
        self.num_graphs = G
        self.x_is_int = not data_list[0].x.is_floating_point()
        self.x_was_1d = data_list[0].x.dim() == 1
        self.geo_dim, self.names, self.node_type_range = None, None, None
        if data_list[0]["pos"] is not None and data_list[0]["node_type"] is not None:
            self.geo_dim = int(data_list[0].x.reshape(data_list[0].x.size(0), -1).size(1))
            nt = torch.cat([d.node_type.reshape(-1) for d in data_list])
            if nt.numel() and (int(nt.min()) < -(1 << 24) or int(nt.max()) > (1 << 24)):
                raise ValueError("DeviceGraphStore: node_type does not survive the fp32 packing")
            self.node_type_range = (int(nt.min()), int(nt.max())) if nt.numel() else (0, 0)
            self.x_all = torch.cat([torch.cat([d.x.reshape(d.x.size(0), -1).float(), d.pos.reshape(-1, 3).float(),
                                               d.node_type.reshape(-1, 1).float()], dim=1) for d in data_list]).contiguous().to(dev)
            if data_list[0]["name"] is not None:
                self.names = [d.name for d in data_list]
        else:
            self.x_all = torch.cat([d.x.reshape(d.x.size(0), -1).float() for d in data_list]).contiguous().to(dev)
        ea = [d.edge_attr for d in data_list]
        self.edge_attr_all = None if any(a is None for a in ea) else torch.cat(ea, dim=0).contiguous().to(dev)
        self._compute_int_ranges()
        self.y_all = torch.cat(ys).float().contiguous().to(dev)
        self.x_dim, self.y_dim = self.x_all.size(1), self.y_all.size(1)
        self.y_is_vector = all(d.y.dim() <= 1 for d in data_list)
        ei = torch.cat([d.edge_index for d in data_list], dim=1).to(torch.int64)
        self.esrc_all, self.edst_all = ei[0].contiguous().to(dev), ei[1].contiguous().to(dev)
        self.pos_enc_all = torch.cat([d.pos_enc for d in data_list]).to(torch.int64).to(dev)
        self.pos_index_all = torch.cat([d.pos_index for d in data_list]).to(torch.int64).to(dev)
        self.pos_batch_all = torch.cat([d.pos_batch for d in data_list]).to(torch.int64).to(dev)
        if int(self.pos_index_all.max()) >= N_COLS or int(self.pos_index_all.min()) < 0:
            raise IndexError("pos_index outside the %d-row z_initial table" % N_COLS)

        Nn, Ee, Zz = int(self.h_node_ptr[-1]), int(self.h_edge_ptr[-1]), int(self.h_nnz_ptr[-1])
        gid_e = torch.repeat_interleave(torch.arange(G, device=dev), e.to(dev))
        node_off_e = self.node_ptr[gid_e]
        self.in_ptr_all, self.in_edge_all = _stable_group(self.edst_all + node_off_e, Nn)
        self.out_ptr_all, self.out_edge_all = _stable_group(self.esrc_all + node_off_e, Nn)
        gid_z = torch.repeat_interleave(torch.arange(G, device=dev), z.to(dev))
        edge_glob = self.pos_batch_all + self.edge_ptr[gid_z]
        if Zz and not bool((edge_glob[1:] >= edge_glob[:-1]).all()):
            raise ValueError("pos_batch must be non-decreasing inside every graph")
        self.row_ptr_all = torch.zeros(Ee + 1, dtype=torch.int64, device=dev)
        self.row_ptr_all[1:] = torch.cumsum(torch.bincount(edge_glob, minlength=Ee), 0)
        gc_key = gid_z * N_COLS + self.pos_index_all
        gc_ptr, self.c_perm_all = _stable_group(gc_key, G * N_COLS)
        self.c_rank_all = (torch.arange(Zz, device=dev) - gc_ptr[gc_key[self.c_perm_all]]).to(torch.int32)
        self.col_cnt_all = (gc_ptr[1:] - gc_ptr[:-1]).to(torch.int32).view(G, N_COLS).contiguous()
        self._build_views()

    _VIEWS = ("in_ptr32", "out_ptr32", "in_edge32", "in_src32", "out_edge32", "out_dst32", "row_ptr32",
              "c_col32", "c_row32", "c_val32")
    _NARROW = (("esrc32", "esrc_all"), ("edst32", "edst_all"), ("pos_enc32", "pos_enc_all"),
               ("pos_index32", "pos_index_all"), ("pos_batch32", "pos_batch_all"))

    def _build_views(self):
        dev, G = self.device, self.num_graphs

        def low32(t):
            return (((t & 0xFFFFFFFF) ^ 0x80000000) - 0x80000000).to(torch.int32).contiguous()

        def per(hptr):
            return torch.repeat_interleave(torch.arange(G, device=dev), (hptr[1:] - hptr[:-1]).to(dev))
        gid_n, gid_e = per(self.h_node_ptr), per(self.h_edge_ptr)
        e0_n, e0_e, z0_e = self.edge_ptr[gid_n], self.edge_ptr[gid_e], self.nnz_ptr[gid_e]
        self.in_ptr32, self.out_ptr32 = low32(self.in_ptr_all[:-1] - e0_n), low32(self.out_ptr_all[:-1] - e0_n)
        self.in_edge32, self.out_edge32 = low32(self.in_edge_all - e0_e), low32(self.out_edge_all - e0_e)
        self.in_src32, self.out_dst32 = low32(self.esrc_all[self.in_edge_all]), low32(self.edst_all[self.out_edge_all])
        self.row_ptr32 = low32(self.row_ptr_all[:-1] - z0_e)
        perm = self.c_perm_all
        self.c_col32, self.c_row32 = low32(self.pos_index_all[perm]), low32(self.pos_batch_all[perm])
        self.c_val32 = low32(self.pos_enc_all[perm])
        for name, src in self._NARROW:
            t = getattr(self, src)
            fits = t.numel() == 0 or (int(t.min()) >= -2 ** 31 and int(t.max()) < 2 ** 31)
            setattr(self, name, t.to(torch.int32).contiguous() if fits else None)
        self.__dict__.pop("_args_tpl", None)

    def _compute_int_ranges(self):
        self.int_ranges = {}
        if self.x_is_int and self.x_all.numel():
            xi = self.x_all.long()
            self.int_ranges["x"] = (xi.min(0)[0].tolist(), xi.max(0)[0].tolist())
        ea = self.edge_attr_all
        if ea is not None and not ea.is_floating_point() and ea.numel():
            ea2 = ea.reshape(ea.size(0), -1)
            self.int_ranges["edge_attr"] = (ea2.min(0)[0].tolist(), ea2.max(0)[0].tolist())

    def __len__(self):
        return self.num_graphs

    _HOST = ("h_node_ptr", "h_edge_ptr", "h_nnz_ptr", "h_y_ptr")
    _META = ("num_graphs", "x_dim", "y_dim", "y_is_vector", "x_is_int", "x_was_1d", "geo_dim", "names", "node_type_range")

    def save(self, path):
        blob = {k: (v.cpu() if torch.is_tensor(v) else v) for k, v in self.__dict__.items()
                if torch.is_tensor(v) or k in self._META}
        torch.save(blob, path)

    def to_data_slices(self):
        x = self.x_all.cpu()
        x = (x.long().view(-1) if self.x_was_1d else x.long()) if self.x_is_int else x
        geo = getattr(self, "geo_dim", None)
        packed, x = x, (x[:, :geo].contiguous() if geo is not None else x)
        y = self.y_all.cpu()
        data = dict(x=x, edge_index=torch.stack([self.esrc_all, self.edst_all]).cpu(),
                    y=y.view(-1) if (self.y_is_vector and self.y_dim == 1) else y,
                    pos_enc=self.pos_enc_all.cpu(), pos_index=self.pos_index_all.cpu(), pos_batch=self.pos_batch_all.cpu())
        slices = dict(x=self.h_node_ptr.clone(), edge_index=self.h_edge_ptr.clone(), y=self.h_y_ptr.clone(),
                      pos_enc=self.h_nnz_ptr.clone(), pos_index=self.h_nnz_ptr.clone(), pos_batch=self.h_nnz_ptr.clone())
        if self.edge_attr_all is not None:
            data["edge_attr"], slices["edge_attr"] = self.edge_attr_all.cpu(), self.h_edge_ptr.clone()
        if geo is not None:
            data["pos"], slices["pos"] = packed[:, geo:geo + 3].contiguous(), self.h_node_ptr.clone()
            data["node_type"], slices["node_type"] = packed[:, geo + 3].long(), self.h_node_ptr.clone()
        return data, slices

    @classmethod
    def from_data_slices(cls, data, slices, device):
        from .data import Data
        get = (lambda k: data[k] if k in data else None) if isinstance(data, dict) else (lambda k: getattr(data, k, None))
        keys = [k for k in ("x", "edge_index", "edge_attr", "y", "pos_enc", "pos_index", "pos_batch") if get(k) is not None]
        if "pos" in slices and "node_type" in slices and get("pos") is not None and get("node_type") is not None:
            keys += ["pos", "node_type"]
        for k in ("x", "edge_index", "y", "pos_enc", "pos_index", "pos_batch"):
            if k not in keys or k not in slices:
                raise KeyError("from_data_slices: key %r missing from data / slices" % k)
        G = int(slices["x"].numel()) - 1
        graphs = []
        for g in range(G):
            kw = {}
            for k in keys:
                t, a, b = get(k), int(slices[k][g]), int(slices[k][g + 1])
                kw[k] = t[:, a:b] if k == "edge_index" else t[a:b]
            graphs.append(Data(**kw))
        return cls(graphs, device)

    @classmethod
    def load(cls, path, device):
        dev = torch.device(device)
        if dev.type != "cuda":
            raise RuntimeError("DeviceGraphStore lives in HBM; there is no CPU fallback")
        blob = torch.load(path, map_location="cpu", weights_only=True)
        self = cls.__new__(cls)
        self.device = dev
        self.edge_attr_all = None
        self.geo_dim, self.names, self.node_type_range = None, None, None
        for k, v in blob.items():
            setattr(self, k, v if (k in cls._HOST or k in cls._META) else v.to(dev))
        self._compute_int_ranges()
        if all(k in blob for k in cls._VIEWS):
            for name, _ in cls._NARROW:
                self.__dict__.setdefault(name, None)
        else:
            self._build_views()
        return self

    def nbytes(self):
        return sum(v.numel() * v.element_size() for v in self.__dict__.values() if torch.is_tensor(v) and v.is_cuda)

    def collate(self, graph_ids):
        if torch.is_tensor(graph_ids) and graph_ids.is_cuda:
            ids_h = graph_ids.to(torch.int64).reshape(-1).cpu()
        else:
            ids_h = torch.as_tensor(graph_ids, dtype=torch.int64).reshape(-1)
        B = ids_h.numel()
        if B == 0:
            raise ValueError("collate: empty batch")
        if int(ids_h.min()) < 0 or int(ids_h.max()) >= self.num_graphs:
            raise IndexError("collate: graph id out of range")
        ptrs = self.__dict__.get("_np_ptrs")
        if ptrs is None:
            ptrs = np.stack([t.numpy() for t in (self.h_node_ptr, self.h_edge_ptr, self.h_nnz_ptr, self.h_y_ptr)])
            self.__dict__["_np_ptrs"] = ptrs
        stage = torch.empty(13 * B + 4, dtype=torch.int64, pin_memory=True)
        st = stage.numpy()
        idn = ids_h.numpy()
        st[:B] = idn
        start, count = st[B:5 * B].reshape(4, B), st[5 * B:9 * B].reshape(4, B)
        offs_np = st[9 * B:].reshape(4, B + 1)
        np.take(ptrs, idn, axis=1, out=start)
        np.subtract(ptrs[:, idn + 1], start, out=count)
        offs_np[:, 0] = 0
        np.cumsum(count, axis=1, out=offs_np[:, 1:])
        N, E, Z, Y = (int(v) for v in offs_np[:, B])
        stage_d = stage.to(self.device, non_blocking=True)
        ids_d, offs_d = stage_d[:B], stage_d[9 * B:].view(4, B + 1)
        offs = stage[9 * B:].view(4, B + 1)
        dev, i64, i32, f32 = self.device, torch.int64, torch.int32, torch.float32
        x = torch.empty((N, self.x_dim), dtype=i64 if self.x_is_int else f32, device=dev)
        ea_all = self.edge_attr_all
        ea_row = 1
        for d_ in (ea_all.shape[1:] if ea_all is not None else ()):
            ea_row *= int(d_)
        ea_fused = ea_all is not None and ea_all.is_contiguous() and ea_row > 0 and (ea_all.element_size() * ea_row) % 4 == 0
        edge_attr = torch.empty((E,) + tuple(ea_all.shape[1:]), dtype=ea_all.dtype, device=dev) if ea_fused else None
        graph_ptr = torch.empty(B + 1, dtype=i32, device=dev)
        y = torch.empty((Y, self.y_dim), dtype=f32, device=dev)
        edge_index = torch.empty((2, E), dtype=i64, device=dev)
        batch = torch.empty(N, dtype=i64, device=dev)
        pos_enc = torch.empty(Z, dtype=i64, device=dev)
        pos_index = torch.empty(Z, dtype=i64, device=dev)
        pos_batch = torch.empty(Z, dtype=i64, device=dev)
        sizes = [N + 1, E, E, N + 1, E, E, E + 1, Z, Z, Z, Z, Z, N_COLS + 1, N_COLS, B * N_COLS]
        slab = torch.empty(sum(sizes), dtype=i32, device=dev)
        parts, o = [], 0
        for s_ in sizes:
            parts.append(slab[o:o + s_])
            o += s_
        (in_ptr, in_edge, in_src, out_ptr, out_edge, out_dst, row_ptr, bag_idx, bag_val, col_row, col_val, col_col,
         col_ptr, col_total, col_prefix) = parts
        s = nv.stream()
        nv.call("esc_collate_cols", nv.ptr(self.col_cnt_all), N_COLS, nv.ptr(ids_d), B, nv.ptr(col_prefix),
                nv.ptr(col_total), s)
        tpl = self.__dict__.get("_args_tpl")
        if tpl is None:
            t0 = nv.CollateArgs()
            t0.x_dim, t0.y_dim, t0.n_cols = self.x_dim, self.y_dim, N_COLS
            for name in ("x_all", "y_all", "esrc_all", "edst_all", "pos_enc_all", "pos_index_all", "pos_batch_all",
                         "c_rank_all") + self._VIEWS + tuple(n for n, _ in self._NARROW):
                setattr(t0, name, nv.ptr(getattr(self, name)))
            tpl = bytes(t0)
            self.__dict__["_args_tpl"] = tpl
        a = nv.CollateArgs.from_buffer_copy(tpl)
        a.B, a.N, a.E, a.Z = B, N, E, Z
        a.stage, a.col_total, a.col_prefix = stage_d.data_ptr(), col_total.data_ptr(), col_prefix.data_ptr()
        a.x, a.y, a.edge_index, a.batch = x.data_ptr(), y.data_ptr(), edge_index.data_ptr(), batch.data_ptr()
        a.pos_enc, a.pos_index, a.pos_batch = pos_enc.data_ptr(), pos_index.data_ptr(), pos_batch.data_ptr()
        base32 = slab.data_ptr()
        o = 0
        for name, s_ in zip(("in_ptr", "in_edge", "in_src", "out_ptr", "out_edge", "out_dst", "row_ptr", "bag_idx", "bag_val",
                             "col_row", "col_val", "col_col", "col_ptr"), sizes):
            setattr(a, name, base32 + 4 * o)
            o += s_
        if self.x_is_int:
            a.x, a.x_long = None, x.data_ptr()
        if ea_fused:
            a.edge_attr_all, a.edge_attr = ea_all.data_ptr(), edge_attr.data_ptr()
            a.ea_words = ea_all.element_size() * ea_row // 4
        a.graph_ptr = graph_ptr.data_ptr()
        nv.call("esc_collate_fill", ctypes.byref(a), s)
        out = Batch()
        if self.x_is_int:
            x = x.view(-1) if self.x_was_1d else x
        geo = getattr(self, "geo_dim", None)
        if geo is not None:
            packed, x = x, x[:, :geo]
            out.pos = packed[:, geo:geo + 3]
            out.node_type = packed[:, geo + 3].long()
            out.node_type._esc_known_range = (self.node_type_range, out.node_type._version)
            if self.names is not None:
                out.name = [self.names[i] for i in ids_h.tolist()]
        out.x, out.edge_index = x, edge_index
        if ea_fused:
            out.edge_attr = edge_attr
        elif self.edge_attr_all is not None:
            cnt = (offs_d[1, 1:] - offs_d[1, :-1])
            src0 = self.edge_ptr[ids_d]
            gather = torch.arange(E, device=dev) + torch.repeat_interleave(src0 - offs_d[1, :-1], cnt, output_size=E)
            out.edge_attr = self.edge_attr_all[gather]
        out.y = y.view(-1) if (self.y_is_vector and self.y_dim == 1) else y
        out.pos_enc, out.pos_index, out.pos_batch, out.batch = pos_enc, pos_index, pos_batch, batch
        plan = BatchPlan(in_ptr=in_ptr, in_edge=in_edge, in_src=in_src, out_ptr=out_ptr, out_edge=out_edge,
                         out_dst=out_dst, row_ptr=row_ptr, bag_idx=bag_idx, bag_val=bag_val, col_ptr=col_ptr,
                         col_row=col_row, col_val=col_val, col_col=col_col, num_nodes=N, num_edges=E, nnz=Z,
                         n_cols=N_COLS)
        plan._keepalive = (slab, stage_d)
        plan.graph_ptr, plan.num_graphs = graph_ptr, B
        plan._batch_sig = _sig(batch)
        object.__setattr__(out, "_num_graphs", B)
        batch._esc_seg = {(batch._version, None): plan.graph_ptr, (batch._version, B): plan.graph_ptr}
        sig = {k: (out[k].data_ptr(), out[k]._version) for k in ("x", "edge_attr") if out[k] is not None}
        object.__setattr__(out, "_esc_int_ranges", (getattr(self, "int_ranges", None) or {}, sig))
        for k, rng in (getattr(self, "int_ranges", None) or {}).items():
            if out[k] is not None:
                out[k]._esc_known_range = (rng, out[k]._version)
        plan._key = plan_key(out, N_COLS)
        object.__setattr__(out, "_esc_plan", plan)
        has_attr = self.edge_attr_all is not None

        def lazy_slices():
            node, edge, nnz, yy = (offs[r].tolist() for r in range(4))
            zero = [0] * B
            slices = dict(x=node, edge_index=edge, y=yy, pos_enc=nnz, pos_index=nnz, pos_batch=nnz)
            shifts = dict(x=zero, edge_index=node[:-1], y=zero, pos_enc=zero, pos_index=zero, pos_batch=edge[:-1])
            if has_attr:
                slices["edge_attr"], shifts["edge_attr"] = edge, zero
            if geo is not None:
                slices["pos"], shifts["pos"], slices["node_type"], shifts["node_type"] = node, zero, node, zero
                if self.names is not None:
                    slices["name"], shifts["name"] = list(range(B + 1)), zero
            return slices, shifts
        object.__setattr__(out, "_lazy_slices", lazy_slices)
        return out


class DeviceLoader(object):

    def __init__(self, store, batch_size=1, shuffle=False, generator=None):
        self.store, self.batch_size, self.shuffle, self.generator = store, batch_size, shuffle, generator

    def __len__(self):
        return (len(self.store) + self.batch_size - 1) // self.batch_size

    def __iter__(self):
        G = len(self.store)
        order = torch.randperm(G, generator=self.generator) if self.shuffle else torch.arange(G)
        for i in range(0, G, self.batch_size):
            yield self.store.collate(order[i:i + self.batch_size])
```

Baseline: 135,500 graphs/s.

## Split Adam step across streams and overlap next forward's bag gather with late update

Adds a "seam" between optimizer and the next training step. The Adam update is split into an early slice on the caller stream and a late slice (containing the z_table) on the edge stream. The next step's forward can then start its bag gather before waiting on z_ready, and the edge-side reduce jobs are moved onto the edge stream before the join. The aim is to remove serialization between the optimizer tail and the next forward. In exchange it adds complex version/stamp bookkeeping, which risks ordering bugs if the guards miss a write to the z_table.

```diff
diff --git a/esc-gnn_amd/_native.py b/esc-gnn_amd/_native.py
--- a/esc-gnn_amd/_native.py
+++ b/esc-gnn_amd/_native.py
@@ -77,6 +77,13 @@
     raise NativeLibraryError("esc_gnn_amd: cannot read the C header %s the binding is derived from (%s)" % (RWSE_HEADER, exc)) from exc
 RWSE_SIGNATURES = {name: args for name, (args, _) in _RWSE.functions.items()}
 _RET.update({name: ret for name, (_, ret) in _RWSE.functions.items()})
+STEP_HEADER = os.path.join(os.path.dirname(_abi.HEADER), "escgnn_step.h")
+try:
+    _STEP = _abi.load(STEP_HEADER)
+except OSError as exc:
+    raise NativeLibraryError("esc_gnn_amd: cannot read the C header %s the binding is derived from (%s)" % (STEP_HEADER, exc)) from exc
+STEP_SIGNATURES = {name: args for name, (args, _) in _STEP.functions.items()}
+_RET.update({name: ret for name, (_, ret) in _STEP.functions.items()})
 KIND = {name[len("ESC_K_"):].lower(): v for name, v in _ABI.enum.items() if name != "ESC_K_COUNT"}
 
 CollateArgs = struct("esc_collate_args")
@@ -99,7 +106,7 @@
             "esc_gnn_amd: %s not found. The HIP hot path has no fallback — build it with "
             "`python -c 'import __graft_entry__ as g; g.build()'` or `make -C esc-gnn_amd/csrc`." % LIB_PATH)
     h = ctypes.CDLL(LIB_PATH)
-    for name, args in list(SIGNATURES.items()) + list(EXTENSION_SIGNATURES.items()) + list(I2GNN_SIGNATURES.items()) + list(GINEPLUS_SIGNATURES.items()) + list(GPS_SIGNATURES.items()) + list(LAPPE_SIGNATURES.items()) + list(RWSE_SIGNATURES.items()):
+    for name, args in list(SIGNATURES.items()) + list(EXTENSION_SIGNATURES.items()) + list(I2GNN_SIGNATURES.items()) + list(GINEPLUS_SIGNATURES.items()) + list(GPS_SIGNATURES.items()) + list(LAPPE_SIGNATURES.items()) + list(RWSE_SIGNATURES.items()) + list(STEP_SIGNATURES.items()):
         try:
             fn = getattr(h, name)
         except AttributeError as exc:
diff --git a/esc-gnn_amd/csrc/common.h b/esc-gnn_amd/csrc/common.h
--- a/esc-gnn_amd/csrc/common.h
+++ b/esc-gnn_amd/csrc/common.h
@@ -50,6 +50,10 @@
 void arm_last_launch_event(hipEvent_t ev);
 void next_launch_is_last();
 hipEvent_t take_last_launch_event();
+
+int adam_launch(float* param, const float* grad, float* exp_avg, float* exp_avg_sq, int64_t n, double lr, double beta1, double beta2,
+                double eps, int64_t step, const float* grad_denom, void* stream);
+void seam_reset();
 
 template <typename... KArgs, typename... Args>
 inline void launch(int kind, void (*kernel)(KArgs...), dim3 grid, dim3 block, size_t lds, hipStream_t s,
diff --git a/esc-gnn_amd/csrc/engine.hip b/esc-gnn_amd/csrc/engine.hip
--- a/esc-gnn_amd/csrc/engine.hip
+++ b/esc-gnn_amd/csrc/engine.hip
@@ -1,4 +1,5 @@
 #include "common.h"
+#include "../../include/escgnn_step.h"
 
 #include <map>
 #include <vector>
@@ -110,6 +111,7 @@
   int act = 1;
   const float* l1_target = nullptr;
   int64_t l1_denom = 0;
+  bool fast_seam = false;
 };
 
 struct LdsFloorGuard {
@@ -167,6 +169,7 @@
   hipStream_t stream = nullptr;
   hipEvent_t z_ready = nullptr, joined = nullptr, lin1_fork = nullptr, lin1_rest = nullptr, lin1_dw = nullptr, e_ready[ESC_MAX_LAYERS] = {}, de_ready[ESC_MAX_LAYERS] = {},
              agg_done[ESC_MAX_LAYERS] = {};
+  hipEvent_t caller_done = nullptr, late_done = nullptr;
   bool ok = false;
 };
 static int g_use_edge_stream = 1;
@@ -189,6 +192,8 @@
     good = good && hipEventCreateWithFlags(&es.lin1_fork, hipEventDisableTiming) == hipSuccess;
     good = good && hipEventCreateWithFlags(&es.lin1_rest, hipEventDisableTiming) == hipSuccess;
     good = good && hipEventCreateWithFlags(&es.lin1_dw, hipEventDisableTiming) == hipSuccess;
+    good = good && hipEventCreateWithFlags(&es.caller_done, hipEventDisableTiming) == hipSuccess;
+    good = good && hipEventCreateWithFlags(&es.late_done, hipEventDisableTiming) == hipSuccess;
     for (int l = 0; l < ESC_MAX_LAYERS; ++l) {
       good = good && hipEventCreateWithFlags(&es.e_ready[l], hipEventDisableTiming) == hipSuccess;
       good = good && hipEventCreateWithFlags(&es.de_ready[l], hipEventDisableTiming) == hipSuccess;
@@ -436,16 +441,18 @@
   EdgeStream& es = edge_stream_for(E);
   Ctx ce = c;
   if (es.ok) {
-    ESC_TRY(chain(es.z_ready, (hipStream_t)c.s, es.stream));
+    if (!c.fast_seam) ESC_TRY(chain(es.z_ready, (hipStream_t)c.s, es.stream));
     ce = edge_ctx(c, es.stream);
   }
   const int64_t bag_block = (c.train && !sync_on(ce)) ? esc_bag_fwd_stats_block_rows(m->z_table, m->z_rows, H, y.Zb, H, E) : 0;
   if (bag_block > 0) {
     ESC_TRY(esc_bag_fwd_rows(m->z_table, m->z_rows, H, b->row_ptr, b->bag_idx, b->bag_val, E, y.Zb, H, 0, ce.y.col_stats, ce.s));
+    if (c.fast_seam) ESC_TRY(chain(es.z_ready, (hipStream_t)c.s, es.stream));
     ESC_TRY(esc_bn_stats_from_partials_rows(ce.y.col_stats, E, H, bag_block, m->zbn0.eps, m->zbn0.momentum, y.zb0.mean, y.zb0.invstd,
                                             m->zbn0.running_mean, m->zbn0.running_var, m->zbn0.gamma, m->zbn0.beta, y.zb0.scale, y.zb0.shift, ce.s));
   } else {
     ESC_TRY(esc_bag_fwd_rows(m->z_table, m->z_rows, H, b->row_ptr, b->bag_idx, b->bag_val, E, y.Zb, H, 0, nullptr, ce.s));
+    if (c.fast_seam) ESC_TRY(chain(es.z_ready, (hipStream_t)c.s, es.stream));
     ESC_TRY(bn_coeffs(ce, y.Zb, H, E, m->zbn0, y.zb0));
   }
   ESC_TRY(esc_affine_act(y.Zb, H, E, H, y.zb0.scale, y.zb0.shift, 1, y.A0, H, ce.s));
@@ -526,23 +533,56 @@
 struct Pending {
   bool open = false;
   bool join = false;
+  bool halves = false;
   hipStream_t stream = nullptr;
+  const float* workspace = nullptr;
+  const float *z_table = nullptr, *dz_table = nullptr;
   std::vector<esc_reduce_job> edge_jobs;
 };
 static Pending& pending() {
   static thread_local Pending p;
   return p;
 }
+
+static int g_legacy_seam = 0;
+struct Seam {
+  int stage = 0;
+  bool claimed = false;
+  hipStream_t stream = nullptr;
+  const float* workspace = nullptr;
+  const float *z_table = nullptr, *dz_table = nullptr;
+  const float *late_lo = nullptr, *late_hi = nullptr;
+  int64_t taken = 0, split_steps = 0;
+};
+static Seam& seam() {
+  static thread_local Seam s;
+  return s;
+}
+void seam_reset() { seam().stage = 0; seam().claimed = false; }
+
 static int finish_pending(Pending& p) {
   if (!p.open) return ESC_OK;
   p.open = false;
   EdgeStream& es = edge_stream();
+  const bool edge_reduced = p.join && p.edge_jobs.empty();
+  if (p.join && p.halves && !g_legacy_seam && hipEventRecord(es.caller_done, p.stream) != hipSuccess) { set_error("esc_engine: stream event failed"); return ESC_ELAUNCH; }
   if (p.join && hipStreamWaitEvent(p.stream, es.joined, 0) != hipSuccess) { set_error("esc_engine: stream event failed"); return ESC_ELAUNCH; }
   if (!p.edge_jobs.empty()) ESC_TRY(esc_slab_reduce_jobs(p.edge_jobs.data(), (int)p.edge_jobs.size(), p.stream));
   p.edge_jobs.clear();
   mark(PH_END, p.stream);
   if (phases().on) ++phases().steps;
-  return ESC_OK;
+  Seam& sm = seam();
+  seam_reset();
+  if (p.halves && edge_reduced && !g_legacy_seam) {
+    sm.stage = 1;
+    sm.stream = p.stream; sm.workspace = p.workspace; sm.z_table = p.z_table; sm.dz_table = p.dz_table;
+  }
+  return ESC_OK;
+}
+static int enter_engine() {
+  const int rc = finish_pending(pending());
+  seam_reset();
+  return rc;
 }
 
 static int backward(const Ctx& c, Pending* defer) {
@@ -678,10 +718,16 @@
   if (k0_split && hipStreamWaitEvent((hipStream_t)c.s, es.lin1_dw, 0) != hipSuccess) { set_error("esc_engine: stream event failed"); return ESC_ELAUNCH; }
   if (c.jobs && !c.jobs->empty()) ESC_TRY(esc_slab_reduce_jobs(c.jobs->data(), (int)c.jobs->size(), c.s));
   if (es.ok) {
-    if (hipEventRecord(es.joined, es.stream) != hipSuccess) { set_error("esc_engine: stream event failed"); return ESC_ELAUNCH; }
+    if (!g_legacy_seam) {
+      const ArmedEvent arm(es.joined, !edge_jobs.empty());
+      if (!edge_jobs.empty()) ESC_TRY(esc_slab_reduce_jobs(edge_jobs.data(), (int)edge_jobs.size(), es.stream));
+      edge_jobs.clear();
+      ESC_TRY(chain_armed(es.joined, arm, es.stream, nullptr));
+    } else if (hipEventRecord(es.joined, es.stream) != hipSuccess) { set_error("esc_engine: stream event failed"); return ESC_ELAUNCH; }
     Pending local;
     Pending& p = defer ? *defer : local;
-    p.open = true; p.join = true; p.stream = (hipStream_t)c.s;
+    p.open = true; p.join = true; p.halves = defer != nullptr; p.stream = (hipStream_t)c.s;
+    p.workspace = nullptr; p.z_table = m->z_table; p.dz_table = m->dz_table;
     p.edge_jobs.swap(edge_jobs);
     if (!defer) return finish_pending(p);
   }
@@ -1225,8 +1271,49 @@
   g_use_edge_stream = (on & 2) != 0;
   g_plain_events = (on & 64) != 0;
   g_readout_one_launch = (on & 128) != 0;
-  return ESC_OK;
-}
+  g_legacy_seam = (on & 256) != 0;
+  seam_reset();
+  return ESC_OK;
+}
+
+int esc_engine_adam_step(float* param, const float* grad, float* exp_avg, float* exp_avg_sq, int64_t n, int64_t n_early,
+                         double lr, double beta1, double beta2, double eps, int64_t step, void* stream) {
+  ESC_REQUIRE(param && grad && exp_avg && exp_avg_sq, "esc_engine_adam_step: null pointer");
+  ESC_REQUIRE(n >= 0 && n_early >= 0 && n_early <= n && step >= 1, "esc_engine_adam_step: bad n/n_early/step");
+  Seam& sm = seam();
+  const bool split = sm.stage == 1 && !g_legacy_seam && sm.stream == (hipStream_t)stream && n_early < n &&
+                     sm.z_table >= param + n_early && sm.z_table < param + n && sm.dz_table >= grad + n_early && sm.dz_table < grad + n;
+  seam_reset();
+  if (!split) return adam_launch(param, grad, exp_avg, exp_avg_sq, n, lr, beta1, beta2, eps, step, nullptr, stream);
+  EdgeStream& es = edge_stream();
+  if (!es.ok) return adam_launch(param, grad, exp_avg, exp_avg_sq, n, lr, beta1, beta2, eps, step, nullptr, stream);
+  if (hipStreamWaitEvent(es.stream, es.caller_done, 0) != hipSuccess) { set_error("esc_engine: stream event failed"); return ESC_ELAUNCH; }
+  {
+    const ArmedEvent arm(es.late_done, true);
+    ESC_TRY(adam_launch(param + n_early, grad + n_early, exp_avg + n_early, exp_avg_sq + n_early, n - n_early, lr, beta1, beta2, eps, step,
+                        nullptr, es.stream));
+    ESC_TRY(chain_armed(es.late_done, arm, es.stream, nullptr));
+  }
+  ESC_TRY(adam_launch(param, grad, exp_avg, exp_avg_sq, n_early, lr, beta1, beta2, eps, step, nullptr, stream));
+  if (hipStreamWaitEvent((hipStream_t)stream, es.late_done, 0) != hipSuccess) { set_error("esc_engine: stream event failed"); return ESC_ELAUNCH; }
+  sm.stage = 2;
+  sm.late_lo = param + n_early; sm.late_hi = param + n;
+  ++sm.split_steps;
+  return ESC_OK;
+}
+
+int esc_engine_claim_fast_seam(void) {
+  Seam& sm = seam();
+  sm.claimed = sm.stage == 2;
+  return ESC_OK;
+}
+
+int esc_engine_drop_fast_seam(void) {
+  seam_reset();
+  return ESC_OK;
+}
+
+int64_t esc_engine_seam_count(int which) { return which == 0 ? seam().taken : which == 1 ? seam().split_steps : -1; }
 
 int esc_engine_phase_times(double* out, int skip) {
   PhaseRing& p = phases();
@@ -1273,7 +1360,7 @@
 
 int esc_engine_train_step(const esc_nested_gin_t* m, const esc_batch_t* b, float* workspace,
                           int64_t loss_denom, float* loss, float* pred, void* stream) {
-  ESC_TRY(finish_pending(pending()));
+  ESC_TRY(enter_engine());
   return train_step_impl(m, b, workspace, loss_denom, loss, pred, stream, nullptr);
 }
 
@@ -1283,10 +1370,14 @@
   return train_step_impl(m, b, workspace, loss_denom, loss, pred, stream, &pending());
 }
 
+
 int esc_engine_train_step_end(void) { return finish_pending(pending()); }
 
 static int train_step_impl(const esc_nested_gin_t* m, const esc_batch_t* b, float* workspace,
                            int64_t loss_denom, float* loss, float* pred, void* stream, Pending* defer) {
+  Seam& sm = seam();
+  const bool seam_offered = defer != nullptr && sm.stage == 2 && sm.claimed && !g_legacy_seam;
+  seam_reset();
   int rc = check(m, b, workspace, true);
   if (rc) return rc;
   ESC_REQUIRE(loss, "esc_engine_train_step: null loss pointer");
@@ -1298,6 +1389,9 @@
   const bool head_l1 = es.ok && m->hidden <= 1024 &&
                        esc_linear_fwd_l1_ok(c.y.Yl, m->hidden, m->lin2.w, m->hidden, c.y.bl.scale, c.y.bl.shift) != 0;
   if (head_l1) { c.l1_target = b->y; c.l1_denom = denom; }
+  c.fast_seam = seam_offered && es.ok && !sync_on(c) && sm.stream == (hipStream_t)stream && sm.workspace == workspace &&
+                m->z_table >= sm.late_lo && m->z_table < sm.late_hi;
+  if (c.fast_seam) ++sm.taken;
   ESC_TRY(forward(c));
   if (head_l1) {
     ESC_TRY(esc_l1_loss(c.y.pred, b->y, b->N, denom, 1.0f, loss, nullptr, es.stream));
@@ -1306,12 +1400,14 @@
   }
   mark(PH_NODE_FWD_DONE, stream);
   if (pred) ESC_TRY(copy_floats(pred, c.y.pred, b->N, stream, "esc_engine_train_step"));
-  return backward(c, defer);
+  rc = backward(c, defer);
+  if (defer != nullptr) defer->workspace = workspace;
+  return rc;
 }
 
 int esc_engine_forward_train(const esc_nested_gin_t* m, const esc_batch_t* b, float* workspace, float* pred,
                              void* stream) {
-  ESC_TRY(finish_pending(pending()));
+  ESC_TRY(enter_engine());
   int rc = check(m, b, workspace, true, false);
   if (rc) return rc;
   ESC_REQUIRE(pred, "esc_engine_forward_train: null output");
@@ -1324,7 +1420,7 @@
 
 int esc_engine_backward(const esc_nested_gin_t* m, const esc_batch_t* b, float* workspace, const float* dpred,
                         void* stream) {
-  ESC_TRY(finish_pending(pending()));
+  ESC_TRY(enter_engine());
   int rc = check(m, b, workspace, true, false);
   if (rc) return rc;
   ESC_REQUIRE(dpred, "esc_engine_backward: null gradient");
@@ -1337,7 +1433,7 @@
 
 int esc_engine_predict(const esc_nested_gin_t* m, const esc_batch_t* b, float* workspace, float* pred,
                        void* stream) {
-  ESC_TRY(finish_pending(pending()));
+  ESC_TRY(enter_engine());
   int rc = check(m, b, workspace, false);
   if (rc) return rc;
   ESC_REQUIRE(pred, "esc_engine_predict: null output");
@@ -1355,7 +1451,7 @@
 
 int esc_zinc_train_step(const esc_zinc_gin_t* m, const esc_mol_batch_t* b, float* workspace, int64_t loss_denom,
                         float* loss, float* pred, void* stream) {
-  ESC_TRY(finish_pending(pending()));
+  ESC_TRY(enter_engine());
   int rc = check_zinc(m, b, workspace, true, true);
   if (rc) return rc;
   ESC_REQUIRE(loss, "esc_zinc_train_step: null loss pointer");
@@ -1370,7 +1466,7 @@
 }
 
 int esc_zinc_forward_train(const esc_zinc_gin_t* m, const esc_mol_batch_t* b, float* workspace, float* pred, void* stream) {
-  ESC_TRY(finish_pending(pending()));
+  ESC_TRY(enter_engine());
   int rc = check_zinc(m, b, workspace, true, false);
   if (rc) return rc;
   ESC_REQUIRE(pred, "esc_zinc_forward_train: null output");
@@ -1382,7 +1478,7 @@
 }
 
 int esc_zinc_backward(const esc_zinc_gin_t* m, const esc_mol_batch_t* b, float* workspace, const float* dpred, void* stream) {
-  ESC_TRY(finish_pending(pending()));
+  ESC_TRY(enter_engine());
   int rc = check_zinc(m, b, workspace, true, false);
   if (rc) return rc;
   ESC_REQUIRE(dpred, "esc_zinc_backward: null gradient");
@@ -1394,7 +1490,7 @@
 }
 
 int esc_zinc_predict(const esc_zinc_gin_t* m, const esc_mol_batch_t* b, float* workspace, float* pred, void* stream) {
-  ESC_TRY(finish_pending(pending()));
+  ESC_TRY(enter_engine());
   int rc = check_zinc(m, b, workspace, false, false);
   if (rc) return rc;
   ESC_REQUIRE(pred, "esc_zinc_predict: null output");
@@ -1411,7 +1507,7 @@
 
 int esc_ogb_train_step(const esc_ogb_gnn_t* m, const esc_ogb_batch_t* b, float* workspace, int64_t loss_denom, float* loss,
                        float* logits, void* stream) {
-  ESC_TRY(finish_pending(pending()));
+  ESC_TRY(enter_engine());
   int rc = check_ogb(m, b, workspace, true, true);
   if (rc) return rc;
   ESC_REQUIRE(loss, "esc_ogb_train_step: null loss pointer");
@@ -1425,7 +1521,7 @@
 }
 
 int esc_ogb_forward_train(const esc_ogb_gnn_t* m, const esc_ogb_batch_t* b, float* workspace, float* logits, void* stream) {
-  ESC_TRY(finish_pending(pending()));
+  ESC_TRY(enter_engine());
   int rc = check_ogb(m, b, workspace, true, false);
   if (rc) return rc;
   ESC_REQUIRE(logits, "esc_ogb_forward_train: null output");
@@ -1437,7 +1533,7 @@
 }
 
 int esc_ogb_backward(const esc_ogb_gnn_t* m, const esc_ogb_batch_t* b, float* workspace, const float* dlogits, void* stream) {
-  ESC_TRY(finish_pending(pending()));
+  ESC_TRY(enter_engine());
   int rc = check_ogb(m, b, workspace, true, false);
   if (rc) return rc;
   ESC_REQUIRE(dlogits, "esc_ogb_backward: null gradient");
@@ -1449,7 +1545,7 @@
 }
 
 int esc_ogb_predict(const esc_ogb_gnn_t* m, const esc_ogb_batch_t* b, float* workspace, float* logits, void* stream) {
-  ESC_TRY(finish_pending(pending()));
+  ESC_TRY(enter_engine());
   int rc = check_ogb(m, b, workspace, false, false);
   if (rc) return rc;
   ESC_REQUIRE(logits, "esc_ogb_predict: null output");
diff --git a/esc-gnn_amd/csrc/optim.hip b/esc-gnn_amd/csrc/optim.hip
--- a/esc-gnn_amd/csrc/optim.hip
+++ b/esc-gnn_amd/csrc/optim.hip
@@ -74,6 +74,21 @@
   }
 }
 
+int adam_launch(float* param, const float* grad, float* exp_avg, float* exp_avg_sq, int64_t n, double lr, double beta1, double beta2,
+                double eps, int64_t step, const float* grad_denom, void* stream) {
+  ESC_REQUIRE(param && grad && exp_avg && exp_avg_sq, "esc_adam_step: null pointer");
+  ESC_REQUIRE(n >= 0 && step >= 1, "esc_adam_step: bad n/step");
+  if (n == 0) return ESC_OK;
+  const double bc1 = 1.0 - pow(beta1, (double)step);
+  const double bc2 = 1.0 - pow(beta2, (double)step);
+  const unsigned blocks = (unsigned)(cdiv(n, 256) < 2048 ? cdiv(n, 256) : 2048);
+  esc::launch(-1, adam_kernel, dim3(blocks), dim3(256), 0, (hipStream_t)stream, param, grad, exp_avg, exp_avg_sq, n,
+                     (float)(1.0 - beta1), (float)beta2, (float)(1.0 - beta2), (float)sqrt(bc2), (float)eps,
+                     (float)(-lr / bc1), grad_denom);
+  ESC_CHECK_LAUNCH("esc_adam_step");
+  return ESC_OK;
+}
+
 }
 
 using namespace esc;
@@ -106,17 +121,8 @@
 int esc_adam_step_scaled(float* param, const float* grad, float* exp_avg, float* exp_avg_sq, int64_t n,
                          double lr, double beta1, double beta2, double eps, int64_t step,
                          const float* grad_denom, void* stream) {
-  ESC_REQUIRE(param && grad && exp_avg && exp_avg_sq, "esc_adam_step: null pointer");
-  ESC_REQUIRE(n >= 0 && step >= 1, "esc_adam_step: bad n/step");
-  if (n == 0) return ESC_OK;
-  const double bc1 = 1.0 - pow(beta1, (double)step);
-  const double bc2 = 1.0 - pow(beta2, (double)step);
-  const unsigned blocks = (unsigned)(cdiv(n, 256) < 2048 ? cdiv(n, 256) : 2048);
-  esc::launch(-1, adam_kernel, dim3(blocks), dim3(256), 0, (hipStream_t)stream, param, grad, exp_avg, exp_avg_sq, n,
-                     (float)(1.0 - beta1), (float)beta2, (float)(1.0 - beta2), (float)sqrt(bc2), (float)eps,
-                     (float)(-lr / bc1), grad_denom);
-  ESC_CHECK_LAUNCH("esc_adam_step");
-  return ESC_OK;
+  esc::seam_reset();
+  return esc::adam_launch(param, grad, exp_avg, exp_avg_sq, n, lr, beta1, beta2, eps, step, grad_denom, stream);
 }
 
 }
diff --git a/esc-gnn_amd/engine.py b/esc-gnn_amd/engine.py
--- a/esc-gnn_amd/engine.py
+++ b/esc-gnn_amd/engine.py
@@ -644,6 +644,7 @@
         self._dev = fam.device(m)
         self._counters = _bn_counters(m) if fam.py_counters else []
         self._open = None
+        self._seam_mark = None
         self._guard_arm()
 
     def _workspace(self, b):
@@ -663,6 +664,8 @@
         ws = self._workspace(b)
         loss = torch.empty(1, dtype=torch.float32, device=self._dev)
         pred = torch.empty(fam.pred_shape(m, b), dtype=torch.float32, device=self._dev) if return_pred else None
+        if entry.endswith("_begin") and self._claims_fast_seam(keep):
+            nv.call("esc_engine_claim_fast_seam")
         nv.call(fam.prefix + entry, ctypes.byref(self._desc), ctypes.byref(b), ws.data_ptr(), int(loss_denom or 0),
                 loss.data_ptr(), nv.ptr(pred), nv.stream())
         self._mark_bucket_written()
@@ -694,8 +697,28 @@
         return self._step("train_step_begin", data, loss_denom, return_pred)
 
     def end_step(self):
+        from .store import collate_seq
         nv.call("esc_engine_train_step_end")
         self._open = None
+        self._seam_mark = collate_seq()
+        bucket = _bucket_of(self._guard_params[0])
+        if hasattr(bucket, "write_versions"):
+            bucket._seam_versions = bucket.write_versions()
+
+    def _claims_fast_seam(self, keep):
+        x, y, plan = keep
+        stamp, mark = getattr(plan, "_collate_stamp", None), getattr(self, "_seam_mark", None)
+        if stamp is None or mark is None:
+            return False
+        bucket = _bucket_of(self._guard_params[0])
+        if not hasattr(bucket, "write_versions") or bucket._seam_versions != bucket.write_versions():
+            return False
+        seq, sig_x, sig_y, stream = stamp
+        return (seq <= mark and stream == nv.stream() and sig_x[0] == x.data_ptr() and sig_x[2] == x._version and
+                sig_y[0] == y.data_ptr() and sig_y[2] == y._version)
+
+    def drop_fast_seam(self):
+        nv.call("esc_engine_drop_fast_seam")
 
 
 class ZincStepEngine(_FamilyEngine):
diff --git a/esc-gnn_amd/optim.py b/esc-gnn_amd/optim.py
--- a/esc-gnn_amd/optim.py
+++ b/esc-gnn_amd/optim.py
@@ -4,6 +4,11 @@
 
 from . import _native as nv
 from .parallel import FlatBucket
+
+
+def _several_ranks():
+    import torch.distributed as dist
+    return dist.is_available() and dist.is_initialized() and dist.get_world_size() > 1
 
 
 class FlatAdam(FlatBucket):
@@ -18,12 +23,23 @@
         if weight_decay:
             self.param_groups[0]["weight_decay"] = weight_decay
         self.step_count = 0
+        self._seam_versions = None
+
+    def write_versions(self):
+        return (self._grad_store._version, self.flat_param._version, self.exp_avg._version, self.exp_avg_sq._version,
+                tuple(p._version for p in self.params))
 
     def step(self, grad_denom=None):
         g = self.param_groups[0]
         self.step_count += 1
         if g.get("weight_decay"):
             self.flat_param.mul_(1.0 - float(g["lr"]) * float(g["weight_decay"]))
+        elif (grad_denom is None and self.early_numel < self.numel and self._seam_versions is not None and
+              self._seam_versions == self.write_versions() and not _several_ranks()):
+            nv.call("esc_engine_adam_step", nv.ptr(self.flat_param), nv.ptr(self.flat_grad), nv.ptr(self.exp_avg),
+                    nv.ptr(self.exp_avg_sq), self.flat_param.numel(), self.early_numel, float(g["lr"]), float(g["betas"][0]),
+                    float(g["betas"][1]), float(g["eps"]), self.step_count, nv.stream())
+            return
         nv.call("esc_adam_step_scaled", nv.ptr(self.flat_param), nv.ptr(self.flat_grad), nv.ptr(self.exp_avg),
                 nv.ptr(self.exp_avg_sq), self.flat_param.numel(), float(g["lr"]), float(g["betas"][0]),
                 float(g["betas"][1]), float(g["eps"]), self.step_count, nv.ptr(grad_denom), nv.stream())
diff --git a/esc-gnn_amd/store.py b/esc-gnn_amd/store.py
--- a/esc-gnn_amd/store.py
+++ b/esc-gnn_amd/store.py
@@ -8,6 +8,12 @@
 from .plan import BatchPlan, plan_key, _sig
 
 N_COLS = 1800
+
+_collate_seq = [0]
+
+
+def collate_seq():
+    return _collate_seq[0]
 
 
 def _stable_group(key, n_keys):
@@ -314,6 +320,8 @@
                 out[k]._esc_known_range = (rng, out[k]._version)
         plan._key = plan_key(out, N_COLS)
         object.__setattr__(out, "_esc_plan", plan)
+        _collate_seq[0] += 1
+        plan._collate_stamp = (_collate_seq[0], _sig(out.x), _sig(out.y), s)
         has_attr = self.edge_attr_all is not None
 
         def lazy_slices():
diff --git a/include/escgnn_step.h b/include/escgnn_step.h
--- /dev/null
+++ b/include/escgnn_step.h
@@ -0,0 +1,18 @@
+#ifndef ESCGNN_STEP_H
+#define ESCGNN_STEP_H
+#include "escgnn_hip.h"
+
+#ifdef __cplusplus
+extern "C" {
+#endif
+
+int esc_engine_adam_step(float* param, const float* grad, float* exp_avg, float* exp_avg_sq, int64_t n, int64_t n_early,
+                         double lr, double beta1, double beta2, double eps, int64_t step, void* stream);
+int esc_engine_claim_fast_seam(void);
+int esc_engine_drop_fast_seam(void);
+int64_t esc_engine_seam_count(int which);
+
+#ifdef __cplusplus
+}
+#endif
+#endif
```

After: 137,700 graphs/s (median of 6 runs). 1.6% higher.
